# kpham-augment/LongLive

Measured on AMD Instinct MI355X. Metric: generated frames/sec (832x480) LongLive-1.3B, frame-sink + short-window attention, 4 denoise steps + clean-context pass, higher is better.
Workload: dtype bf16

## Files before the change

### include/longlive_hip.h

```cpp
#ifndef LONGLIVE_HIP_H
#define LONGLIVE_HIP_H

#include <stdint.h>

#ifdef __cplusplus
extern "C" {
#endif

typedef uint16_t ll_bf16;
typedef void* ll_stream;

enum ll_status {
  LL_OK = 0,
  LL_ERR_INVALID_ARG = -1,
  LL_ERR_LAUNCH = -2,
  LL_ERR_UNSUPPORTED = -3
};

enum ll_epilogue {
  LL_EPI_BIAS = 0,
  LL_EPI_BIAS_GELU = 1,
  LL_EPI_BIAS_GATE_RES = 2,
  LL_EPI_BIAS_RES = 3
};

#define LL_ABI_VERSION 111
int ll_version(void);
const char* ll_last_error(void);
int ll_set_tuning(const char* key, int value);
int ll_gemm_plan(int M, int N, int K, int int8, char* out, int cap);
int ll_gemm_plan_epi(int M, int N, int K, int int8, int epilogue, int plain, char* out, int cap);
int ll_flash_attn_plan(int Lq, int H, int B, int seg0_len, int seg1_len, int seg_adjacent, char* out, int cap);
int ll_conv_plan(int T, int H, int W, int Cin, int Cout, int KT, int KH, int upsample, int with_res, int rms, char* out, int cap);


int ll_ln_modulate(const ll_bf16* x, ll_bf16* out, const ll_bf16* e, const ll_bf16* mod, int nmod, int shift_idx,
                   int scale_idx, int B, int L, int C, int F, float eps, ll_stream stream);

int ll_modulation_table(const ll_bf16* e, const ll_bf16* mods, ll_bf16* out, int num_layers, int BF, int nmod, int C,
                        ll_stream stream);

int ll_modulation_table_f32(const ll_bf16* e, const ll_bf16* mods, float* out, int num_layers, int BF, int nmod, int C,
                            unsigned one_plus_mask, ll_stream stream);

int ll_ln_modulate_tab(const ll_bf16* x, ll_bf16* out, int8_t* q, float* qscale, const float* tab, int nmod, int shift_idx,
                       int scale_idx, int B, int L, int C, int F, float eps, ll_stream stream);

int ll_layernorm_affine(const ll_bf16* x, const ll_bf16* w, const ll_bf16* b, ll_bf16* out, int rows, int C,
                        float eps, ll_stream stream);

int ll_ln_modulate_q8(const ll_bf16* x, int8_t* q, float* qscale, const ll_bf16* e, const ll_bf16* mod, int nmod,
                      int shift_idx, int scale_idx, int B, int L, int C, int F, float eps, ll_stream stream);
int ll_layernorm_affine_q8(const ll_bf16* x, const ll_bf16* w, const ll_bf16* b, int8_t* q, float* qscale, int rows,
                           int C, float eps, ll_stream stream);

int ll_rmsnorm(const ll_bf16* x, const ll_bf16* w, ll_bf16* out, int rows, int C, int ldx, int ldo, float eps,
               ll_stream stream);

int ll_qk_norm_rope_kv_store(const ll_bf16* qkv, const ll_bf16* wq, const ll_bf16* wk, const float* rope_f,
                             const float* rope_hw, ll_bf16* q_out, ll_bf16* cache_k, ll_bf16* cache_v, int B, int L,
                             int C, int head_dim, int frame_len, int start_frame, int S, int write_start,
                             int roped_offset, int write_len, float eps, ll_stream stream);

int ll_kv_roll(ll_bf16* cache_k, ll_bf16* cache_v, int B, int S, int C, int dst, int src, int n, ll_stream stream);


int ll_gemm_bf16(const ll_bf16* x, const ll_bf16* w, const ll_bf16* bias, ll_bf16* out, int M, int N, int K, int ldx,
                 int ldo, int epilogue, const ll_bf16* res, const ll_bf16* e, const ll_bf16* mod, int nmod,
                 int gate_idx, int rows_per_batch, int frame_len, ll_stream stream);

int ll_gemm_ksplit_plan(int M, int N, int K);
long long ll_gemm_ksplit_workspace_bytes(int M, int N, int K);
int ll_gemm_bf16_ksplit(const ll_bf16* x, const ll_bf16* w, const ll_bf16* bias, ll_bf16* out, int M, int N, int K, int ldx,
                        int ldo, int epilogue, const ll_bf16* res, void* workspace, long long workspace_bytes, ll_stream stream);
int ll_gemm_bf16_ksplit_t5norm(const ll_bf16* x, const ll_bf16* w, const ll_bf16* bias, ll_bf16* out, int M, int N, int K, int ldx,
                               int ldo, const ll_bf16* res, const ll_bf16* norm_w, float eps, ll_bf16* h_out, void* workspace,
                               long long workspace_bytes, ll_stream stream);

int ll_gemm_w8a8(const int8_t* xq, const float* sx, const int8_t* wq, const float* sw, const ll_bf16* bias, ll_bf16* out,
                 int M, int N, int K, int ldo, int epilogue, const ll_bf16* res, const ll_bf16* e, const ll_bf16* mod,
                 int nmod, int gate_idx, int rows_per_batch, int frame_len, ll_stream stream);

int ll_gemm_bf16_qkv(const ll_bf16* x, const ll_bf16* w, const ll_bf16* bias, ll_bf16* out, int M, int N, int K, int ldx, int ldo,
                     ll_bf16* cache_v, int B, int L, int S, int write_start, int roped_offset, int write_len, ll_stream stream);
int ll_gemm_w8a8_qkv(const int8_t* xq, const float* sx, const int8_t* wq, const float* sw, const ll_bf16* bias, ll_bf16* out,
                     int M, int N, int K, int ldo, ll_bf16* cache_v, int B, int L, int S, int write_start, int roped_offset,
                     int write_len, ll_stream stream);

int ll_quantize_rows(const ll_bf16* x, int8_t* q, float* scale, int rows, int K, int ldx, ll_stream stream);

int ll_quantize_mx(const ll_bf16* x, uint8_t* q, uint8_t* qs, int rows, int K, int ldx, ll_stream stream);
int ll_gemm_mx(const uint8_t* xq, const uint8_t* sx, const uint8_t* wq, const uint8_t* sw, const ll_bf16* bias, ll_bf16* out,
               uint8_t* q_out, uint8_t* s_out, int M, int N, int K, int ldo, int epilogue, const ll_bf16* res, const ll_bf16* e,
               const ll_bf16* mod, int nmod, int gate_idx, int rows_per_batch, int frame_len, ll_stream stream);
int ll_gemm_mx_qkv(const uint8_t* xq, const uint8_t* sx, const uint8_t* wq, const uint8_t* sw, const ll_bf16* bias, ll_bf16* out,
                   int M, int N, int K, int ldo, ll_bf16* cache_v, int B, int L, int S, int write_start, int roped_offset,
                   int write_len, ll_stream stream);
int ll_ln_modulate_mx(const ll_bf16* x, uint8_t* q, uint8_t* qs, const ll_bf16* e, const ll_bf16* mod, int nmod, int shift_idx,
                      int scale_idx, int B, int L, int C, int F, float eps, ll_stream stream);
int ll_ln_modulate_tab_mx(const ll_bf16* x, uint8_t* q, uint8_t* qs, const float* tab, int nmod, int shift_idx, int scale_idx,
                          int B, int L, int C, int F, float eps, ll_stream stream);
int ll_layernorm_affine_mx(const ll_bf16* x, const ll_bf16* w, const ll_bf16* b, uint8_t* q, uint8_t* qs, int rows, int C,
                           float eps, ll_stream stream);
int ll_gemm_plan_mx(int M, int N, int K, char* out, int cap);

int ll_quantize_mx6(const ll_bf16* x, uint8_t* q, uint8_t* qs, int rows, int K, int ldx, ll_stream stream);
int ll_gemm_mx6(const uint8_t* xq, const uint8_t* sx, const uint8_t* wq, const uint8_t* sw, const ll_bf16* bias, ll_bf16* out,
                uint8_t* q_out, uint8_t* s_out, int M, int N, int K, int ldo, int epilogue, const ll_bf16* res, const ll_bf16* e,
                const ll_bf16* mod, int nmod, int gate_idx, int rows_per_batch, int frame_len, ll_stream stream);
int ll_gemm_mx6_qkv(const uint8_t* xq, const uint8_t* sx, const uint8_t* wq, const uint8_t* sw, const ll_bf16* bias, ll_bf16* out,
                    int M, int N, int K, int ldo, ll_bf16* cache_v, int B, int L, int S, int write_start, int roped_offset,
                    int write_len, ll_stream stream);
int ll_ln_modulate_mx6(const ll_bf16* x, uint8_t* q, uint8_t* qs, const ll_bf16* e, const ll_bf16* mod, int nmod, int shift_idx,
                       int scale_idx, int B, int L, int C, int F, float eps, ll_stream stream);
int ll_ln_modulate_tab_mx6(const ll_bf16* x, uint8_t* q, uint8_t* qs, const float* tab, int nmod, int shift_idx, int scale_idx,
                           int B, int L, int C, int F, float eps, ll_stream stream);
int ll_layernorm_affine_mx6(const ll_bf16* x, const ll_bf16* w, const ll_bf16* b, uint8_t* q, uint8_t* qs, int rows, int C,
                            float eps, ll_stream stream);
int ll_gemm_plan_mx6(int M, int N, int K, char* out, int cap);

int ll_quantize_mx4(const ll_bf16* x, uint8_t* q, uint8_t* qs, int rows, int K, int ldx, ll_stream stream);
int ll_gemm_mx4w6(const uint8_t* xq, const uint8_t* sx, const uint8_t* wq, const uint8_t* sw, const ll_bf16* bias, ll_bf16* out,
                  uint8_t* q_out, uint8_t* s_out, int M, int N, int K, int ldo, int epilogue, const ll_bf16* res, const ll_bf16* e,
                  const ll_bf16* mod, int nmod, int gate_idx, int rows_per_batch, int frame_len, ll_stream stream);
int ll_gemm_mx4w6_qkv(const uint8_t* xq, const uint8_t* sx, const uint8_t* wq, const uint8_t* sw, const ll_bf16* bias, ll_bf16* out,
                      int M, int N, int K, int ldo, ll_bf16* cache_v, int B, int L, int S, int write_start, int roped_offset,
                      int write_len, ll_stream stream);
int ll_gemm_plan_mx4w6(int M, int N, int K, char* out, int cap);

int ll_gemm_mx4(const uint8_t* xq, const uint8_t* sx, const uint8_t* wq, const uint8_t* sw, const ll_bf16* bias, ll_bf16* out,
                uint8_t* q_out, uint8_t* s_out, int M, int N, int K, int ldo, int epilogue, const ll_bf16* res, const ll_bf16* e,
                const ll_bf16* mod, int nmod, int gate_idx, int rows_per_batch, int frame_len, ll_stream stream);
int ll_gemm_mx4_qkv(const uint8_t* xq, const uint8_t* sx, const uint8_t* wq, const uint8_t* sw, const ll_bf16* bias, ll_bf16* out,
                    int M, int N, int K, int ldo, ll_bf16* cache_v, int B, int L, int S, int write_start, int roped_offset,
                    int write_len, ll_stream stream);
int ll_ln_modulate_mx4(const ll_bf16* x, uint8_t* q, uint8_t* qs, const ll_bf16* e, const ll_bf16* mod, int nmod, int shift_idx,
                       int scale_idx, int B, int L, int C, int F, float eps, ll_stream stream);
int ll_ln_modulate_tab_mx4(const ll_bf16* x, uint8_t* q, uint8_t* qs, const float* tab, int nmod, int shift_idx, int scale_idx,
                           int B, int L, int C, int F, float eps, ll_stream stream);
int ll_layernorm_affine_mx4(const ll_bf16* x, const ll_bf16* w, const ll_bf16* b, uint8_t* q, uint8_t* qs, int rows, int C,
                            float eps, ll_stream stream);
int ll_gemm_plan_mx4(int M, int N, int K, char* out, int cap);

int ll_quantize_rows_f8(const ll_bf16* x, uint8_t* q, float* scale, int rows, int K, int ldx, ll_stream stream);
int ll_gemm_f8(const uint8_t* xq, const float* sx, const uint8_t* wq, const float* sw, const ll_bf16* bias, ll_bf16* out,
               int M, int N, int K, int ldo, int epilogue, const ll_bf16* res, const ll_bf16* e, const ll_bf16* mod,
               int nmod, int gate_idx, int rows_per_batch, int frame_len, ll_stream stream);
int ll_gemm_f8_qkv(const uint8_t* xq, const float* sx, const uint8_t* wq, const float* sw, const ll_bf16* bias, ll_bf16* out,
                   int M, int N, int K, int ldo, ll_bf16* cache_v, int B, int L, int S, int write_start, int roped_offset,
                   int write_len, ll_stream stream);
int ll_ln_modulate_f8(const ll_bf16* x, uint8_t* q, float* qscale, const ll_bf16* e, const ll_bf16* mod, int nmod, int shift_idx,
                      int scale_idx, int B, int L, int C, int F, float eps, ll_stream stream);
int ll_ln_modulate_tab_f8(const ll_bf16* x, uint8_t* q, float* qscale, const float* tab, int nmod, int shift_idx, int scale_idx,
                          int B, int L, int C, int F, float eps, ll_stream stream);
int ll_layernorm_affine_f8(const ll_bf16* x, const ll_bf16* w, const ll_bf16* b, uint8_t* q, float* qscale, int rows, int C,
                           float eps, ll_stream stream);
int ll_gemm_plan_f8(int M, int N, int K, char* out, int cap);

int ll_kv_shadow_mx(const ll_bf16* k, const ll_bf16* v, uint8_t* kq, uint8_t* ks, uint8_t* vq, uint8_t* vs, int B, int S, int S32, int H,
                    int head_dim, int lo, int hi, ll_stream stream);
int ll_flash_attn_mx(const ll_bf16* q, const uint8_t* kq, const uint8_t* ks, const uint8_t* vq, const uint8_t* vs, ll_bf16* out, int B,
                     int Lq, int H, int head_dim, int ldq, int ldo, int S, int S32, int seg0_start, int seg0_len, int seg1_start,
                     int seg1_len, float scale, ll_stream stream);
int ll_flash_attn_mx_plan(int Lq, int H, int B, int seg0_start, int seg0_len, int seg1_start, int seg1_len, char* out, int cap);

int ll_linear_small(const ll_bf16* x, const ll_bf16* w, const ll_bf16* bias, ll_bf16* out, int M, int N, int K,
                    int act_in, int act_out, ll_stream stream);

int ll_flash_attn(const ll_bf16* q, const ll_bf16* k, const ll_bf16* v, ll_bf16* out, int B, int Lq, int H, int ldq,
                  int ldo, int ldk, long long k_batch_stride, int seg0_start, int seg0_len, int seg1_start,
                  int seg1_len, float scale, ll_stream stream);

int ll_gemm_ssq_planes(int M, int N, int K);
int ll_gemm_bf16_ssq(const ll_bf16* x, const ll_bf16* w, const ll_bf16* bias, ll_bf16* out, float* ssq, int M, int N, int K, int ldx,
                     int ldo, ll_stream stream);
int ll_flash_attn_qnorm_ok(int H, int nkeys);
int ll_flash_attn_qnorm(const ll_bf16* q, const float* ssq, const ll_bf16* norm_w, float eps, const ll_bf16* k, const ll_bf16* v,
                        ll_bf16* out, int B, int Lq, int H, int ldq, int ldo, int ldk, long long k_batch_stride, int key_start,
                        int nkeys, float scale, ll_stream stream);

enum ll_qfmt { LL_QFMT_MX = 1, LL_QFMT_MX6 = 2, LL_QFMT_MX4 = 3 };
int ll_flash_attn_q_ok(int fmt, int H, int seg0_start, int seg0_len, int seg1_start, int seg1_len);
int ll_flash_attn_q_plan(int fmt, int Lq, int H, int B, int seg0_start, int seg0_len, int seg1_start, int seg1_len, char* out, int cap);
int ll_flash_attn_q(int fmt, const ll_bf16* q, const ll_bf16* k, const ll_bf16* v, uint8_t* codes, uint8_t* scales, int B, int Lq, int H,
                    int ldq, int ldc, int lds, int ldk, long long k_batch_stride, int seg0_start, int seg0_len, int seg1_start,
                    int seg1_len, float scale, ll_stream stream);
int ll_flash_attn_mx_q(int fmt, const ll_bf16* q, const uint8_t* kq, const uint8_t* ks, const uint8_t* vq, const uint8_t* vs,
                       uint8_t* codes, uint8_t* scales, int B, int Lq, int H, int head_dim, int ldq, int ldc, int lds, int S, int S32,
                       int seg0_start, int seg0_len, int seg1_start, int seg1_len, float scale, ll_stream stream);


int ll_patchify(const ll_bf16* x, ll_bf16* patches, int B, int F, int Cin, int H, int W, ll_stream stream);

int ll_sinusoid(const float* t, ll_bf16* out, int n, int dim, ll_stream stream);

int ll_unpatchify_x0(const ll_bf16* head, const ll_bf16* xt, const float* sigma, ll_bf16* flow, ll_bf16* x0, int B,
                     int F, int Cout, int H, int W, ll_stream stream);

int ll_add_noise(const ll_bf16* x0, const ll_bf16* noise, const float* sigma, ll_bf16* out, int N, long long inner,
                 ll_stream stream);

int ll_sigma_lookup(const float* t, const float* timesteps, const float* sigmas, float* out, int n, int n_table,
                    ll_stream stream);

int ll_synth_hash(float* out, long long lo, long long n, unsigned long long stream_const, int kind, ll_stream stream);


int ll_conv_cl(const ll_bf16* x, const ll_bf16* zero16, const ll_bf16* w, const ll_bf16* bias, const ll_bf16* res,
               ll_bf16* out, int T, int H, int W, int Cin, int Cout, int Kpad, int KT, int KH, int upsample, int ldo,
               ll_stream stream);
int ll_conv_cl_rms_ok(int H, int W, int Cin, int Cout, int KT, int KH, int upsample);
int ll_conv_cl_rms(const ll_bf16* x, const ll_bf16* zero16, const ll_bf16* w, const ll_bf16* bias, const ll_bf16* res, ll_bf16* out,
                   const ll_bf16* rms_gamma, ll_bf16* out_rms, int rms_silu, int T, int H, int W, int Cin, int Cout, int Kpad, int KT,
                   int KH, int upsample, int ldo, ll_stream stream);

int ll_rms_silu_cl(const ll_bf16* x, const ll_bf16* gamma, ll_bf16* out, long long pixels, int C, int do_silu,
                   ll_stream stream);

int ll_softmax_rows(const ll_bf16* s, ll_bf16* p, int rows, int N, int ld, float scale, ll_stream stream);

int ll_vae_unscale_cl(const ll_bf16* z, const ll_bf16* mean, const ll_bf16* inv_std, ll_bf16* out, int T, int C, int h,
                      int w, ll_stream stream);

int ll_cl_to_tchw_clamp(const ll_bf16* x, float* out, int T, int H, int W, int ldc, ll_stream stream);


int ll_cl_to_frames_u8(const ll_bf16* x, uint8_t* out, long long stride_t, int T, int H, int W, int ldc, ll_stream stream);

int ll_jpeg_sizes(int T, int H, int W, long long* out_stride, long long* scratch_bytes);
int ll_jpeg_encode_u8(const uint8_t* frames, long long stride_t, int T, int H, int W, int quality, uint8_t* out, long long out_stride,
                      int32_t* sizes, void* scratch, long long scratch_bytes, ll_stream stream);
int ll_jpeg_coefficients_u8(const uint8_t* frames, long long stride_t, int T, int H, int W, int quality, int16_t* coef, ll_stream stream);

int ll_jpeg_decode_sizes(int T, int H, int W, int ncomp, int hs, int vs, long long* coef_bytes, long long* scratch_bytes);
int ll_jpeg_decode_coefficients(const uint8_t* data, long long nbytes, const int32_t* segs, int nseg, const uint8_t* huff,
                                const uint8_t* sel, int T, int H, int W, int ncomp, int hs, int vs, int16_t* coef, int32_t* status,
                                ll_stream stream);
int ll_jpeg_decode_pixels(const int16_t* coef, const uint16_t* qt, int T, int H, int W, int ncomp, int hs, int vs, uint8_t* out,
                          long long stride_t, void* scratch, long long scratch_bytes, ll_stream stream);
int ll_jpeg_decode_u8(const uint8_t* data, long long nbytes, const int32_t* segs, int nseg, const uint8_t* huff, const uint8_t* sel,
                      const uint16_t* qt, int T, int H, int W, int ncomp, int hs, int vs, int16_t* coef, int32_t* status, uint8_t* out,
                      long long stride_t, void* scratch, long long scratch_bytes, ll_stream stream);
int ll_jpeg_decode_split_sizes(int nseg, int nsub, long long* work_bytes);
int ll_jpeg_decode_coefficients_split(const uint8_t* data, long long nbytes, const int32_t* segs, int nseg, const uint8_t* huff,
                                      const uint8_t* sel, int T, int H, int W, int ncomp, int hs, int vs, int16_t* coef, int32_t* status,
                                      const int32_t* subs, int nsub, int rounds, int32_t* info, void* work, long long work_bytes,
                                      ll_stream stream);
int ll_jpeg_decode_u8_split(const uint8_t* data, long long nbytes, const int32_t* segs, int nseg, const uint8_t* huff, const uint8_t* sel,
                            const uint16_t* qt, int T, int H, int W, int ncomp, int hs, int vs, int16_t* coef, int32_t* status, uint8_t* out,
                            long long stride_t, void* scratch, long long scratch_bytes, const int32_t* subs, int nsub, int rounds,
                            int32_t* info, void* work, long long work_bytes, ll_stream stream);
int ll_resize_u8(const uint8_t* src, long long src_stride_t, int Hs, int Ws, int y0, int x0, int Hc, int Wc, uint8_t* dst,
                 long long dst_stride_t, int Hd, int Wd, int T, const int32_t* ystart, const int32_t* ycount, const float* yweight, int ky,
                 const int32_t* xstart, const int32_t* xcount, const float* xweight, int kx, ll_stream stream);


int ll_conv_cl_down(const ll_bf16* x, const ll_bf16* zero16, const ll_bf16* w, const ll_bf16* bias, ll_bf16* out, int T, int H, int W,
                    int Cin, int Cout, int Kpad, int ldo, ll_stream stream);
int ll_conv_cl_tdown(const ll_bf16* x, const ll_bf16* zero16, const ll_bf16* w, const ll_bf16* bias, ll_bf16* out, int T, int H, int W,
                     int Cin, int Cout, int Kpad, int ldo, ll_stream stream);
int ll_conv_down_plan(int kind, int T, int H, int W, int Cin, int Cout, char* out, int cap);

int ll_pixels_to_cl(const void* px, int is_f32, long long stride_c, long long stride_t, ll_bf16* out, int T, int H, int W, int Cpad,
                    ll_stream stream);

int ll_pixels_u8_to_cl(const uint8_t* px, long long stride_t, ll_bf16* out, int T, int H, int W, int Cpad, ll_stream stream);

int ll_vae_scale_tchw(const ll_bf16* mu, const ll_bf16* mean, const ll_bf16* inv_std, float* out, int T, int z_dim, int h, int w, int ld,
                      ll_stream stream);


int ll_t5_rmsnorm(const ll_bf16* x, const ll_bf16* w, ll_bf16* out, int rows, int C, float eps, ll_stream stream);

int ll_t5_gated_gelu(const ll_bf16* h, ll_bf16* out, long long M, int F, ll_stream stream);

int ll_gather_rows(const ll_bf16* table, const long long* ids, ll_bf16* out, int n, int C, long long vocab, ll_stream stream);

int ll_t5_attention(const ll_bf16* q, const ll_bf16* k, const ll_bf16* vt, const ll_bf16* bias_tab, ll_bf16* out, int L,
                    int H, int ldqk, int ldo, int seq_len, ll_stream stream);

#ifdef __cplusplus
}
#endif
#endif
```

### longlive_amd/_lib.py

```python
from __future__ import annotations

import ctypes as C
import os

_HERE = os.path.dirname(os.path.abspath(__file__))
LIB_PATH = os.path.join(_HERE, "liblonglive_hip.so")

ABI_VERSION = 111

_p, _i, _f, _ll = C.c_void_p, C.c_int, C.c_float, C.c_longlong

SIGNATURES = {
    "ll_version": [],
    "ll_last_error": [],
    "ll_set_tuning": [C.c_char_p, _i],
    "ll_gemm_plan": [_i, _i, _i, _i, C.c_char_p, _i],
    "ll_gemm_plan_epi": [_i, _i, _i, _i, _i, _i, C.c_char_p, _i],
    "ll_flash_attn_plan": [_i, _i, _i, _i, _i, _i, C.c_char_p, _i],
    "ll_ln_modulate": [_p, _p, _p, _p, _i, _i, _i, _i, _i, _i, _i, _f, _p],
    "ll_modulation_table": [_p, _p, _p, _i, _i, _i, _i, _p],
    "ll_modulation_table_f32": [_p, _p, _p, _i, _i, _i, _i, C.c_uint, _p],
    "ll_ln_modulate_tab": [_p, _p, _p, _p, _p, _i, _i, _i, _i, _i, _i, _i, _f, _p],
    "ll_layernorm_affine": [_p, _p, _p, _p, _i, _i, _f, _p],
    "ll_ln_modulate_q8": [_p, _p, _p, _p, _p, _i, _i, _i, _i, _i, _i, _i, _f, _p],
    "ll_layernorm_affine_q8": [_p, _p, _p, _p, _p, _i, _i, _f, _p],
    "ll_rmsnorm": [_p, _p, _p, _i, _i, _i, _i, _f, _p],
    "ll_qk_norm_rope_kv_store": [_p, _p, _p, _p, _p, _p, _p, _p, _i, _i, _i, _i, _i, _i, _i, _i, _i, _i, _f, _p],
    "ll_kv_roll": [_p, _p, _i, _i, _i, _i, _i, _i, _p],
    "ll_gemm_bf16": [_p, _p, _p, _p, _i, _i, _i, _i, _i, _i, _p, _p, _p, _i, _i, _i, _i, _p],
    "ll_gemm_ksplit_plan": [_i, _i, _i],
    "ll_gemm_ksplit_workspace_bytes": [_i, _i, _i],
    "ll_gemm_bf16_ksplit": [_p, _p, _p, _p, _i, _i, _i, _i, _i, _i, _p, _p, _ll, _p],
    "ll_gemm_bf16_ksplit_t5norm": [_p, _p, _p, _p, _i, _i, _i, _i, _i, _p, _p, _f, _p, _p, _ll, _p],
    "ll_gemm_w8a8": [_p, _p, _p, _p, _p, _p, _i, _i, _i, _i, _i, _p, _p, _p, _i, _i, _i, _i, _p],
    "ll_gemm_bf16_qkv": [_p, _p, _p, _p, _i, _i, _i, _i, _i, _p, _i, _i, _i, _i, _i, _i, _p],
    "ll_gemm_w8a8_qkv": [_p, _p, _p, _p, _p, _p, _i, _i, _i, _i, _p, _i, _i, _i, _i, _i, _i, _p],
    "ll_quantize_rows": [_p, _p, _p, _i, _i, _i, _p],
    "ll_linear_small": [_p, _p, _p, _p, _i, _i, _i, _i, _i, _p],
    "ll_flash_attn": [_p, _p, _p, _p, _i, _i, _i, _i, _i, _i, _ll, _i, _i, _i, _i, _f, _p],
    "ll_patchify": [_p, _p, _i, _i, _i, _i, _i, _p],
    "ll_sinusoid": [_p, _p, _i, _i, _p],
    "ll_unpatchify_x0": [_p, _p, _p, _p, _p, _i, _i, _i, _i, _i, _p],
    "ll_add_noise": [_p, _p, _p, _p, _i, _ll, _p],
    "ll_sigma_lookup": [_p, _p, _p, _p, _i, _i, _p],
    "ll_synth_hash": [_p, _ll, _ll, C.c_ulonglong, _i, _p],
    "ll_gemm_ssq_planes": [_i, _i, _i],
    "ll_gemm_bf16_ssq": [_p, _p, _p, _p, _p, _i, _i, _i, _i, _i, _p],
    "ll_flash_attn_qnorm_ok": [_i, _i],
    "ll_flash_attn_qnorm": [_p, _p, _p, _f, _p, _p, _p, _i, _i, _i, _i, _i, _i, _ll, _i, _i, _f, _p],
    "ll_flash_attn_q_ok": [_i] * 6,
    "ll_flash_attn_q_plan": [_i] * 8 + [C.c_char_p, _i],
    "ll_flash_attn_q": [_i] + [_p] * 5 + [_i] * 7 + [_ll] + [_i] * 4 + [_f, _p],
    "ll_flash_attn_mx_q": [_i] + [_p] * 7 + [_i] * 13 + [_f, _p],
    "ll_conv_plan": [_i] * 10 + [C.c_char_p, _i],
    "ll_conv_cl": [_p] * 6 + [_i] * 10 + [_p],
    "ll_conv_cl_rms_ok": [_i] * 7,
    "ll_conv_cl_rms": [_p] * 8 + [_i] * 11 + [_p],
    "ll_rms_silu_cl": [_p, _p, _p, _ll, _i, _i, _p],
    "ll_softmax_rows": [_p, _p, _i, _i, _i, _f, _p],
    "ll_vae_unscale_cl": [_p, _p, _p, _p, _i, _i, _i, _i, _p],
    "ll_cl_to_tchw_clamp": [_p, _p, _i, _i, _i, _i, _p],
    "ll_cl_to_frames_u8": [_p, _p, _ll, _i, _i, _i, _i, _p],
    "ll_jpeg_sizes": [_i, _i, _i, C.POINTER(_ll), C.POINTER(_ll)],
    "ll_jpeg_encode_u8": [_p, _ll, _i, _i, _i, _i, _p, _ll, _p, _p, _ll, _p],
    "ll_jpeg_coefficients_u8": [_p, _ll, _i, _i, _i, _i, _p, _p],
    "ll_jpeg_decode_sizes": [_i] * 6 + [C.POINTER(_ll), C.POINTER(_ll)],
    "ll_jpeg_decode_coefficients": [_p, _ll, _p, _i, _p, _p] + [_i] * 6 + [_p, _p, _p],
    "ll_jpeg_decode_pixels": [_p, _p] + [_i] * 6 + [_p, _ll, _p, _ll, _p],
    "ll_jpeg_decode_u8": [_p, _ll, _p, _i, _p, _p, _p] + [_i] * 6 + [_p, _p, _p, _ll, _p, _ll, _p],
    "ll_jpeg_decode_split_sizes": [_i, _i, C.POINTER(_ll)],
    "ll_jpeg_decode_coefficients_split": [_p, _ll, _p, _i, _p, _p] + [_i] * 6 + [_p, _p] + [_p, _i, _i, _p, _p, _ll, _p],
    "ll_jpeg_decode_u8_split": [_p, _ll, _p, _i, _p, _p, _p] + [_i] * 6 + [_p, _p, _p, _ll, _p, _ll] + [_p, _i, _i, _p, _p, _ll, _p],
    "ll_resize_u8": [_p, _ll] + [_i] * 6 + [_p, _ll, _i, _i, _i, _p, _p, _p, _i, _p, _p, _p, _i, _p],
    "ll_conv_cl_down": [_p] * 5 + [_i] * 7 + [_p],
    "ll_conv_cl_tdown": [_p] * 5 + [_i] * 7 + [_p],
    "ll_conv_down_plan": [_i] * 6 + [C.c_char_p, _i],
    "ll_pixels_to_cl": [_p, _i, _ll, _ll, _p, _i, _i, _i, _i, _p],
    "ll_pixels_u8_to_cl": [_p, _ll, _p, _i, _i, _i, _i, _p],
    "ll_vae_scale_tchw": [_p, _p, _p, _p, _i, _i, _i, _i, _i, _p],
    "ll_t5_rmsnorm": [_p, _p, _p, _i, _i, _f, _p],
    "ll_t5_gated_gelu": [_p, _p, _ll, _i, _p],
    "ll_gather_rows": [_p, _p, _p, _i, _i, _ll, _p],
    "ll_t5_attention": [_p, _p, _p, _p, _p, _i, _i, _i, _i, _i, _p],
    "ll_quantize_mx": [_p, _p, _p, _i, _i, _i, _p],
    "ll_gemm_mx": [_p, _p, _p, _p, _p, _p, _p, _p, _i, _i, _i, _i, _i, _p, _p, _p, _i, _i, _i, _i, _p],
    "ll_gemm_mx_qkv": [_p, _p, _p, _p, _p, _p, _i, _i, _i, _i, _p, _i, _i, _i, _i, _i, _i, _p],
    "ll_ln_modulate_mx": [_p, _p, _p, _p, _p, _i, _i, _i, _i, _i, _i, _i, _f, _p],
    "ll_ln_modulate_tab_mx": [_p, _p, _p, _p, _i, _i, _i, _i, _i, _i, _i, _f, _p],
    "ll_layernorm_affine_mx": [_p, _p, _p, _p, _p, _i, _i, _f, _p],
    "ll_gemm_plan_mx": [_i, _i, _i, C.c_char_p, _i],
    "ll_kv_shadow_mx": [_p] * 6 + [_i] * 7 + [_p],
    "ll_flash_attn_mx": [_p] * 6 + [_i] * 12 + [_f, _p],
    "ll_flash_attn_mx_plan": [_i] * 7 + [C.c_char_p, _i],
    "ll_quantize_rows_f8": [_p, _p, _p, _i, _i, _i, _p],
    "ll_gemm_f8": [_p, _p, _p, _p, _p, _p, _i, _i, _i, _i, _i, _p, _p, _p, _i, _i, _i, _i, _p],
    "ll_gemm_f8_qkv": [_p, _p, _p, _p, _p, _p, _i, _i, _i, _i, _p, _i, _i, _i, _i, _i, _i, _p],
    "ll_ln_modulate_f8": [_p, _p, _p, _p, _p, _i, _i, _i, _i, _i, _i, _i, _f, _p],
    "ll_ln_modulate_tab_f8": [_p, _p, _p, _p, _i, _i, _i, _i, _i, _i, _i, _f, _p],
    "ll_layernorm_affine_f8": [_p, _p, _p, _p, _p, _i, _i, _f, _p],
    "ll_gemm_plan_f8": [_i, _i, _i, C.c_char_p, _i],
    "ll_quantize_mx6": [_p, _p, _p, _i, _i, _i, _p],
    "ll_gemm_mx6": [_p] * 8 + [_i] * 5 + [_p] * 3 + [_i] * 4 + [_p],
    "ll_gemm_mx6_qkv": [_p] * 6 + [_i] * 4 + [_p] + [_i] * 6 + [_p],
    "ll_ln_modulate_mx6": [_p] * 5 + [_i] * 7 + [_f, _p],
    "ll_ln_modulate_tab_mx6": [_p] * 4 + [_i] * 7 + [_f, _p],
    "ll_layernorm_affine_mx6": [_p] * 5 + [_i, _i, _f, _p],
    "ll_gemm_plan_mx6": [_i, _i, _i, C.c_char_p, _i],
    "ll_quantize_mx4": [_p, _p, _p, _i, _i, _i, _p],
    "ll_gemm_mx4w6": [_p] * 8 + [_i] * 5 + [_p] * 3 + [_i] * 4 + [_p],
    "ll_gemm_mx4w6_qkv": [_p] * 6 + [_i] * 4 + [_p] + [_i] * 6 + [_p],
    "ll_gemm_plan_mx4w6": [_i, _i, _i, C.c_char_p, _i],
    "ll_gemm_mx4": [_p] * 8 + [_i] * 5 + [_p] * 3 + [_i] * 4 + [_p],
    "ll_gemm_mx4_qkv": [_p] * 6 + [_i] * 4 + [_p] + [_i] * 6 + [_p],
    "ll_ln_modulate_mx4": [_p] * 5 + [_i] * 7 + [_f, _p],
    "ll_ln_modulate_tab_mx4": [_p] * 4 + [_i] * 7 + [_f, _p],
    "ll_layernorm_affine_mx4": [_p] * 5 + [_i, _i, _f, _p],
    "ll_gemm_plan_mx4": [_i, _i, _i, C.c_char_p, _i],
}
_RESTYPES = {"ll_last_error": C.c_char_p, "ll_gemm_ksplit_workspace_bytes": C.c_longlong}

_lib = None


def load() -> C.CDLL:
    global _lib
    if _lib is not None:
        return _lib
    path = os.environ.get("LONGLIVE_HIP_LIB", LIB_PATH)
    if not os.path.exists(path):
        raise RuntimeError(
            f"{path} not found: the HIP extension is not built (make -C longlive_amd/csrc). "
            "longlive_amd has no CPU fallback by design.")
    lib = C.CDLL(path)
    for name, argtypes in SIGNATURES.items():
        try:
            fn = getattr(lib, name)
        except AttributeError as exc:
            raise RuntimeError(f"{LIB_PATH} does not export {name}") from exc
        fn.argtypes = argtypes
        fn.restype = _RESTYPES.get(name, C.c_int)
    if lib.ll_version() != ABI_VERSION:
        raise RuntimeError(f"{path} has ABI version {lib.ll_version()}, this binding needs {ABI_VERSION}: rebuild it "
                           "(make -C longlive_amd/csrc); a stale library would misread every argument list")
    _lib = lib
    for kv in filter(None, os.environ.get("LL_TUNING", "").split(",")):
        k, v = kv.split("=")
        if lib.ll_set_tuning(k.encode(), int(v)) != 0:
            raise RuntimeError(f"LL_TUNING: {lib.ll_last_error().decode()}")
    return lib


def check(rc: int, what: str = "") -> None:
    if rc != 0:
        msg = load().ll_last_error()
        raise RuntimeError(f"longlive_hip {what} failed (status {rc}): {msg.decode() if msg else ''}")
```

### longlive_amd/csrc/gemm.hip

```cpp
#include <stdio.h>
#include <string.h>
#include <atomic>

#include "attention_common.h"
#include "gemm_asm.h"
#include "gemm_common.h"
#include "mx.h"

#ifdef LL_GEMM_DIAG
constexpr bool GEMM_DIAG = true;
#else
constexpr bool GEMM_DIAG = false;
#endif

#define V2_BM 256
#define V2_STAGE ((V2_BM + BN) * ROWB)

template <int EPI, int Q>
__global__ __launch_bounds__(512, 2) void gemm_kernel_v2(const char* __restrict__ X, const char* __restrict__ Wt,
                                                         bf16* __restrict__ Y, int M, int N, int nk, size_t xrow_bytes,
                                                         size_t wrow_bytes, int ldo, int ntm, int ntn, int gm, int lds_epi, EpiArgs ea) {
  extern __shared__ __attribute__((aligned(16))) char smem[];
  const int tid = threadIdx.x, lane = tid & 63;
  const int wave = __builtin_amdgcn_readfirstlane(tid >> 6);
// ... 346 lines not shown
  else snprintf(walk, sizeof walk, ", N fastest");
  snprintf(out, (size_t)cap, "%s<%s> tile %dx%d, %d workgroups%s", p.name, kind, p.bm, p.bn, p.ntm * p.ntn, walk);
}

extern "C" int ll_gemm_plan(int M, int N, int K, int int8, char* out, int cap) {
  LL_REQUIRE(out != nullptr && cap > 0, "ll_gemm_plan: needs an output buffer");
  gemm_plan_text(M, N, int8 ? "i8" : "bf16", out, cap);
  (void)K;
  return LL_OK;
}

extern "C" int ll_gemm_plan_f8(int M, int N, int K, char* out, int cap) {
  LL_REQUIRE(out != nullptr && cap > 0, "ll_gemm_plan_f8: needs an output buffer");
  gemm_plan_text(M, N, "f8", out, cap);
  (void)K;
  return LL_OK;
}

extern "C" int ll_gemm_plan_epi(int M, int N, int K, int int8, int epilogue, int plain, char* out, int cap);

extern "C" int ll_t5_rmsnorm(const ll_bf16* x, const ll_bf16* w, ll_bf16* out, int rows, int C, float eps, ll_stream stream);

static bool gemm_asm_wanted(int epilogue) {
  return (g_gemm_asm & 1) && !((g_gemm_asm & 4) && epilogue == LL_EPI_BIAS_GELU) && !((g_gemm_asm & 8) && epilogue != LL_EPI_BIAS_GELU);
}

typedef void (*gemm_kernel_t)(const char*, const char*, bf16*, int, int, int, size_t, size_t, int, int, int, int, int, EpiArgs);
template <int E, int Q>
static gemm_kernel_t gemm_instance(int variant) {
  switch (variant) {
    case 3: return gemm_kernel_v5<E, Q, 2, 4, 8, 4, 2, false>;
    case 5: return gemm_kernel_v5<E, Q, 2, 4, 8, 3, 1, true>;
    case 6: return gemm_kernel_v5<E, Q, 4, 2, 4, 7, 1, true>;
    default: return gemm_kernel_v2<E, Q>;
  }
}

template <int Q>
static int launch_gemm(const void* x, const void* w, bf16* out, int M, int N, int K, size_t xrow_bytes, size_t wrow_bytes,
                       int ldo, int epilogue, const EpiArgs& ea, hipStream_t s) {
  if (Q == GQ_BF16 && gemm_asm_wanted(epilogue) && wrow_bytes == (size_t)K * 2) {
    const int r = gemm_asm_launch((const bf16*)x, (const bf16*)w, out, M, N, K, (int)(xrow_bytes / 2), ldo, epilogue, ea, g_gemm_group_m, s);
    if (r) return r < 0 ? r : 0;
  }
  if (Q == GQ_I8 && (g_gemm_asm & 16) && gemm_asm_wanted(epilogue) && xrow_bytes == (size_t)K && wrow_bytes == (size_t)K) {
    const int r = gemm_asm_launch_i8((const int8_t*)x, (const int8_t*)w, out, M, N, K, ldo, epilogue, ea, g_gemm_group_m, s);
    if (r) return r < 0 ? r : 0;
  }
  const int nk = (Q == GQ_BF16 ? 2 * K : K) / ROWB;
  const GemmPlan p = gemm_plan(M, N);
  const int mode = g_gemm_lds_epi & 3;
  const int lds_epi = (mode == 2 || (mode == 1 && epilogue != LL_EPI_BIAS_GELU) ? 1 : 0) | (GEMM_DIAG ? g_gemm_lds_epi & 0x300 : 0);
  const gemm_kernel_t k = epilogue == LL_EPI_BIAS            ? gemm_instance<LL_EPI_BIAS, Q>(p.variant)
                          : epilogue == LL_EPI_BIAS_GELU     ? gemm_instance<LL_EPI_BIAS_GELU, Q>(p.variant)
                          : epilogue == LL_EPI_BIAS_GATE_RES ? gemm_instance<LL_EPI_BIAS_GATE_RES, Q>(p.variant)
                                                             : gemm_instance<LL_EPI_BIAS_RES, Q>(p.variant);
  (void)ll_lds_attr((const void*)k, p.lds);
  hipLaunchKernelGGL(k, dim3(p.ntm * p.ntn), dim3(512), (size_t)p.lds, s, (const char*)x, (const char*)w, out, M, N, nk, xrow_bytes,
                     wrow_bytes, ldo, p.ntm, p.ntn, g_gemm_group_m, lds_epi, ea);
  return LL_OK;
}

struct FamBF16 {
  static constexpr int Q = GQ_BF16;
  static int check(const char* fn, const void*, const void*, const void*, const void*, const void*, int, int K, int ldx, int) {
    LL_REQUIRE(K > 0 && K % 64 == 0, "%s: K=%d must be a positive multiple of 64", fn, K);
    LL_REQUIRE(ldx >= K && ldx % 8 == 0, "%s: ldx=%d must be >= K and a multiple of 8", fn, ldx);
    return LL_OK;
  }
  static size_t xrow(int, int ldx) { return (size_t)ldx * 2; }
  static size_t wrow(int K) { return (size_t)K * 2; }
};
struct FamW8A8 {
  static constexpr int Q = GQ_I8;
  static int check(const char* fn, const void*, const void* sx, const void*, const void* sw, const void*, int, int K, int, int) {
    LL_REQUIRE(K > 0 && K % 128 == 0, "%s: K=%d must be a positive multiple of 128", fn, K);
    LL_REQUIRE(sx && sw, "%s: activation and weight scales are required", fn);
    return LL_OK;
  }
  static size_t xrow(int K, int) { return (size_t)K; }
  static size_t wrow(int K) { return (size_t)K; }
};
struct FamF8 {
  static constexpr int Q = GQ_F8;
  static int check(const char* fn, const void* xq, const void* sx, const void* wq, const void* sw, const void* out, int M, int K, int,
                   int ldo) {
    LL_REQUIRE(xq && sx && wq && sw, "%s: codes and scales of both operands are required", fn);
    LL_REQUIRE(out != nullptr, "%s: out is required", fn);
    LL_REQUIRE(K > 0 && K % 128 == 0, "%s: K=%d must be a positive multiple of 128", fn, K);
    LL_REQUIRE(M >= 0, "%s: M=%d", fn, M);
    LL_REQUIRE(ldo % 8 == 0, "%s: ldo=%d must be a multiple of 8", fn, ldo);
    return LL_OK;
  }
  static size_t xrow(int K, int) { return (size_t)K; }
  static size_t wrow(int K) { return (size_t)K; }
};

template <class F>
static int gemm_call(const char* fn, const void* x, const float* sx, const void* w, const float* sw, const ll_bf16* bias, ll_bf16* out,
                     int M, int N, int K, int ldx, int ldo, int epilogue, const ll_bf16* res, const ll_bf16* e, const ll_bf16* mod,
                     int nmod, int gate_idx, int rows_per_batch, int frame_len, ll_stream stream) {
  if (int rc = F::check(fn, x, sx, w, sw, out, M, K, ldx, ldo)) return rc;
  if (int rc = check_epilogue(fn, M, N, ldo, epilogue, bias, res, e, mod, nmod, gate_idx, rows_per_batch, frame_len)) return rc;
  if (M == 0) return LL_OK;
  EpiArgs ea{(const bf16*)bias, (const bf16*)res, (const bf16*)e, (const bf16*)mod, sx, sw, nmod, gate_idx,
             rows_per_batch, frame_len, frame_len > 0 && rows_per_batch > 0 ? rows_per_batch / frame_len : 0};
  if (int lrc = launch_gemm<F::Q>(x, w, (bf16*)out, M, N, K, F::xrow(K, ldx), F::wrow(K), ldo, epilogue, ea, (hipStream_t)stream)) return lrc;
  return ll_check_launch(fn);
}

template <class F>
static int gemm_call_qkv(const char* fn, const void* x, const float* sx, const void* w, const float* sw, const ll_bf16* bias,
                         ll_bf16* out, int M, int N, int K, int ldx, int ldo, ll_bf16* cache_v, int B, int L, int S, int write_start,
                         int roped_offset, int write_len, ll_stream stream) {
  if (int rc = F::check(fn, x, sx, w, sw, out, M, K, ldx, ldo)) return rc;
  if (int rc = check_epilogue(fn, M, N, ldo, LL_EPI_BIAS, bias, nullptr, nullptr, nullptr, 0, 0, 0, 0)) return rc;
  if (int rc = check_v_insert(fn, M, N, B, L, S, write_start, roped_offset, write_len, cache_v)) return rc;
  if (M == 0) return LL_OK;
  EpiArgs ea{(const bf16*)bias, nullptr, nullptr, nullptr, sx, sw, 0, 0, 0, 0, 0};
  set_v_insert(ea, cache_v, N, L, S, write_start, roped_offset, write_len);
  if (int lrc = launch_gemm<F::Q>(x, w, (bf16*)out, M, N, K, F::xrow(K, ldx), F::wrow(K), ldo, LL_EPI_BIAS, ea, (hipStream_t)stream)) return lrc;
  return ll_check_launch(fn);
}

extern "C" int ll_gemm_bf16(const ll_bf16* x, const ll_bf16* w, const ll_bf16* bias, ll_bf16* out, int M, int N, int K,
                            int ldx, int ldo, int epilogue, const ll_bf16* res, const ll_bf16* e, const ll_bf16* mod,
                            int nmod, int gate_idx, int rows_per_batch, int frame_len, ll_stream stream) {
  return gemm_call<FamBF16>("ll_gemm_bf16", x, nullptr, w, nullptr, bias, out, M, N, K, ldx, ldo, epilogue, res, e, mod, nmod, gate_idx,
                            rows_per_batch, frame_len, stream);
}

extern "C" int ll_gemm_ssq_planes(int M, int N, int K) {
  if (!gemm_asm_wanted(LL_EPI_BIAS)) return 0;
  const GemmAsmPick p = gemm_asm_pick(GQ_BF16, M, N, K, K, LL_EPI_BIAS, true, false, false, 0, 0);
  return p.k && p.k->wn == 128 && N / 128 <= 16 ? N / 128 : 0;
}
extern "C" int ll_gemm_bf16_ssq(const ll_bf16* x, const ll_bf16* w, const ll_bf16* bias, ll_bf16* out, float* ssq, int M, int N, int K,
                                int ldx, int ldo, ll_stream stream) {
  LL_REQUIRE(K > 0 && K % 64 == 0, "ll_gemm_bf16_ssq: K=%d must be a positive multiple of 64", K);
  LL_REQUIRE(ldx >= K && ldx % 8 == 0, "ll_gemm_bf16_ssq: ldx=%d must be >= K and a multiple of 8", ldx);
  int rc = check_epilogue("ll_gemm_bf16_ssq", M, N, ldo, LL_EPI_BIAS, bias, nullptr, nullptr, nullptr, 0, 0, 0, 0);
  if (rc) return rc;
  LL_REQUIRE(ssq != nullptr && ((size_t)ssq & 3) == 0, "ll_gemm_bf16_ssq: ssq is required");
  LL_REQUIRE(ll_gemm_ssq_planes(M, N, K) > 0 && ldx == K, "ll_gemm_bf16_ssq: %d x %d x %d is not covered by the generated kernel under the current "
             "tuning (ask ll_gemm_ssq_planes first and run ll_gemm_bf16 + ll_rmsnorm instead)", M, N, K);
  if (M == 0) return LL_OK;
  const int r = gemm_asm_ssq_launch((const bf16*)x, (const bf16*)w, (const bf16*)bias, (bf16*)out, ssq, M, N, K, ldx, ldo, g_gemm_group_m,
                                    (hipStream_t)stream);
  if (r < 0) return r;
  LL_REQUIRE(r == 1, "ll_gemm_bf16_ssq: the generated kernel refused a shape its plan accepted");
  return ll_check_launch("ll_gemm_bf16_ssq");
}

extern "C" int ll_gemm_ksplit_plan(int M, int N, int K) {
  if (!gemm_asm_wanted(LL_EPI_BIAS)) return 0;
  return gemm_ksplit_splits(M, N, K, device_cus());
}
extern "C" long long ll_gemm_ksplit_workspace_bytes(int M, int N, int K) {
  const int S = ll_gemm_ksplit_plan(M, N, K);
  return S ? (long long)S * M * N * 4 : 0;
}
extern "C" int ll_gemm_bf16_ksplit(const ll_bf16* x, const ll_bf16* w, const ll_bf16* bias, ll_bf16* out, int M, int N, int K,
                                   int ldx, int ldo, int epilogue, const ll_bf16* res, void* workspace,
                                   long long workspace_bytes, ll_stream stream) {
  LL_REQUIRE(K > 0 && K % 64 == 0, "ll_gemm_bf16_ksplit: K=%d must be a positive multiple of 64", K);
  LL_REQUIRE(ldx >= K && ldx % 8 == 0, "ll_gemm_bf16_ksplit: ldx=%d must be >= K and a multiple of 8", ldx);
  LL_REQUIRE(epilogue == LL_EPI_BIAS || epilogue == LL_EPI_BIAS_RES, "ll_gemm_bf16_ksplit: epilogue %d (bias or bias + residual only)", epilogue);
  int rc = check_epilogue("ll_gemm_bf16_ksplit", M, N, ldo, epilogue, bias, res, nullptr, nullptr, 0, 0, 0, 0);
  if (rc) return rc;
  LL_REQUIRE(workspace_bytes >= 0 && (workspace != nullptr || workspace_bytes == 0), "ll_gemm_bf16_ksplit: workspace_bytes without a workspace");
  if (M == 0) return LL_OK;
  const int S = ll_gemm_ksplit_plan(M, N, K);
  if (S >= 2 && workspace != nullptr) {
    LL_REQUIRE(workspace_bytes >= (long long)S * M * N * 4 && ((size_t)workspace & 15) == 0,
               "ll_gemm_bf16_ksplit: workspace of %lld bytes, need %lld (16-byte aligned)", workspace_bytes, (long long)S * M * N * 4);
    const int r = gemm_asm_ksplit_launch((const bf16*)x, (const bf16*)w, (const bf16*)bias, (bf16*)out, M, N, K, ldx, ldo, epilogue,
                                         (const bf16*)res, (float*)workspace, S, g_gemm_group_m, (hipStream_t)stream, nullptr, 0.f, nullptr);
    if (r) return r < 0 ? r : ll_check_launch("ll_gemm_bf16_ksplit");
  }
  EpiArgs ea{(const bf16*)bias, (const bf16*)res, nullptr, nullptr, nullptr, nullptr, 0, 0, 0, 0, 0};
  if (int lrc = launch_gemm<GQ_BF16>(x, w, (bf16*)out, M, N, K, (size_t)ldx * 2, (size_t)K * 2, ldo, epilogue, ea, (hipStream_t)stream)) return lrc;
  return ll_check_launch("ll_gemm_bf16_ksplit");
}

extern "C" int ll_gemm_bf16_ksplit_t5norm(const ll_bf16* x, const ll_bf16* w, const ll_bf16* bias, ll_bf16* out, int M, int N, int K,
                                          int ldx, int ldo, const ll_bf16* res, const ll_bf16* norm_w, float eps, ll_bf16* h_out,
                                          void* workspace, long long workspace_bytes, ll_stream stream) {
  LL_REQUIRE(K > 0 && K % 64 == 0, "ll_gemm_bf16_ksplit_t5norm: K=%d must be a positive multiple of 64", K);
  LL_REQUIRE(ldx >= K && ldx % 8 == 0, "ll_gemm_bf16_ksplit_t5norm: ldx=%d must be >= K and a multiple of 8", ldx);
  LL_REQUIRE(norm_w != nullptr && h_out != nullptr, "ll_gemm_bf16_ksplit_t5norm: needs the norm weight and an output for the normalised rows");
  LL_REQUIRE(ldo == N, "ll_gemm_bf16_ksplit_t5norm: ldo=%d must equal N=%d (the norm runs over whole rows)", ldo, N);
  int rc = check_epilogue("ll_gemm_bf16_ksplit_t5norm", M, N, ldo, LL_EPI_BIAS_RES, bias, res, nullptr, nullptr, 0, 0, 0, 0);
  if (rc) return rc;
  LL_REQUIRE(workspace_bytes >= 0 && (workspace != nullptr || workspace_bytes == 0), "ll_gemm_bf16_ksplit_t5norm: workspace_bytes without a workspace");
  if (M == 0) return LL_OK;
  const int S = ll_gemm_ksplit_plan(M, N, K);
  if (S >= 2 && workspace != nullptr && N <= 4096) {
    LL_REQUIRE(workspace_bytes >= (long long)S * M * N * 4 && ((size_t)workspace & 15) == 0,
               "ll_gemm_bf16_ksplit_t5norm: workspace of %lld bytes, need %lld (16-byte aligned)", workspace_bytes, (long long)S * M * N * 4);
    const int r = gemm_asm_ksplit_launch((const bf16*)x, (const bf16*)w, (const bf16*)bias, (bf16*)out, M, N, K, ldx, ldo, LL_EPI_BIAS_RES,
                                         (const bf16*)res, (float*)workspace, S, g_gemm_group_m, (hipStream_t)stream, (const bf16*)norm_w, eps,
                                         (bf16*)h_out);
    if (r) return r < 0 ? r : ll_check_launch("ll_gemm_bf16_ksplit_t5norm");
  }
  rc = ll_gemm_bf16_ksplit(x, w, bias, out, M, N, K, ldx, ldo, LL_EPI_BIAS_RES, res, workspace, workspace_bytes, stream);
  if (rc) return rc;
  return ll_t5_rmsnorm(out, norm_w, h_out, M, N, eps, stream);
}

extern "C" int ll_gemm_plan_epi(int M, int N, int K, int int8, int epilogue, int plain, char* out, int cap) {
  LL_REQUIRE(out != nullptr && cap > 0, "ll_gemm_plan_epi: needs an output buffer");
  if (gemm_asm_wanted(epilogue) && (!int8 || (g_gemm_asm & 16))) {
    const GemmAsmPick p = gemm_asm_pick(int8 ? GQ_I8 : GQ_BF16, M, N, K, K, epilogue, plain != 0, plain == 2, plain == 2 && (2 * (N / 3)) % 192 == 0,
                                        1, int8 ? 0 : device_cus());
    if (p.k) { gemm_asm_plan(p, out, cap); ll_plan_append_knobs(out, cap); return LL_OK; }
  }
  return ll_gemm_plan(M, N, K, int8, out, cap);
}

extern "C" int ll_gemm_w8a8(const int8_t* xq, const float* sx, const int8_t* wq, const float* sw, const ll_bf16* bias,
                            ll_bf16* out, int M, int N, int K, int ldo, int epilogue, const ll_bf16* res,
                            const ll_bf16* e, const ll_bf16* mod, int nmod, int gate_idx, int rows_per_batch,
                            int frame_len, ll_stream stream) {
  return gemm_call<FamW8A8>("ll_gemm_w8a8", xq, sx, wq, sw, bias, out, M, N, K, K, ldo, epilogue, res, e, mod, nmod, gate_idx,
                            rows_per_batch, frame_len, stream);
}

extern "C" int ll_gemm_f8(const uint8_t* xq, const float* sx, const uint8_t* wq, const float* sw, const ll_bf16* bias, ll_bf16* out,
                          int M, int N, int K, int ldo, int epilogue, const ll_bf16* res, const ll_bf16* e, const ll_bf16* mod,
                          int nmod, int gate_idx, int rows_per_batch, int frame_len, ll_stream stream) {
  return gemm_call<FamF8>("ll_gemm_f8", xq, sx, wq, sw, bias, out, M, N, K, K, ldo, epilogue, res, e, mod, nmod, gate_idx,
                          rows_per_batch, frame_len, stream);
}

extern "C" int ll_gemm_bf16_qkv(const ll_bf16* x, const ll_bf16* w, const ll_bf16* bias, ll_bf16* out, int M, int N, int K, int ldx,
                                int ldo, ll_bf16* cache_v, int B, int L, int S, int write_start, int roped_offset, int write_len,
                                ll_stream stream) {
  return gemm_call_qkv<FamBF16>("ll_gemm_bf16_qkv", x, nullptr, w, nullptr, bias, out, M, N, K, ldx, ldo, cache_v, B, L, S, write_start,
                                roped_offset, write_len, stream);
}

extern "C" int ll_gemm_w8a8_qkv(const int8_t* xq, const float* sx, const int8_t* wq, const float* sw, const ll_bf16* bias,
                                ll_bf16* out, int M, int N, int K, int ldo, ll_bf16* cache_v, int B, int L, int S, int write_start,
                                int roped_offset, int write_len, ll_stream stream) {
  return gemm_call_qkv<FamW8A8>("ll_gemm_w8a8_qkv", xq, sx, wq, sw, bias, out, M, N, K, K, ldo, cache_v, B, L, S, write_start,
                                roped_offset, write_len, stream);
}

extern "C" int ll_gemm_f8_qkv(const uint8_t* xq, const float* sx, const uint8_t* wq, const float* sw, const ll_bf16* bias,
                              ll_bf16* out, int M, int N, int K, int ldo, ll_bf16* cache_v, int B, int L, int S, int write_start,
                              int roped_offset, int write_len, ll_stream stream) {
  return gemm_call_qkv<FamF8>("ll_gemm_f8_qkv", xq, sx, wq, sw, bias, out, M, N, K, K, ldo, cache_v, B, L, S, write_start, roped_offset,
                              write_len, stream);
}

template <bool F8, class TQ>
static int quantize_rows_launch(const char* fn, void (*reg4)(const bf16*, TQ*, float*, int, int, int),
                                void (*reg18)(const bf16*, TQ*, float*, int, int, int), void (*two_pass)(const bf16*, TQ*, float*, int, int, int),
                                const ll_bf16* x, TQ* q, float* scale, int rows, int K, int ldx, ll_stream stream) {
  if (F8) LL_REQUIRE(x != nullptr && q != nullptr && scale != nullptr, "%s: x, codes and scales are required", fn);
  LL_REQUIRE(K > 0 && K % 8 == 0, "%s: K=%d must be a positive multiple of 8", fn, K);
  LL_REQUIRE(ldx >= K && ldx % 8 == 0, "%s: ldx=%d must be >= K and a multiple of 8", fn, ldx);
  if (F8) LL_REQUIRE(rows >= 0, "%s: rows=%d", fn, rows);
  if (rows == 0) return LL_OK;
  hipLaunchKernelGGL(K <= 2048 ? reg4 : K <= 9216 ? reg18 : two_pass, dim3((rows + 3) / 4), dim3(256), 0, (hipStream_t)stream,
                     (const bf16*)x, q, scale, rows, K, ldx);
  return ll_check_launch(fn);
}

extern "C" int ll_quantize_rows(const ll_bf16* x, int8_t* q, float* scale, int rows, int K, int ldx, ll_stream stream) {
  return quantize_rows_launch<false>("ll_quantize_rows", quantize_rows_reg_kernel<4>, quantize_rows_reg_kernel<18>, quantize_rows_kernel,
                                     x, q, scale, rows, K, ldx, stream);
}

extern "C" int ll_quantize_rows_f8(const ll_bf16* x, uint8_t* q, float* scale, int rows, int K, int ldx, ll_stream stream) {
  return quantize_rows_launch<true>("ll_quantize_rows_f8", quantize_rows_f8_reg_kernel<4>, quantize_rows_f8_reg_kernel<18>,
                                    quantize_rows_f8_kernel, x, q, scale, rows, K, ldx, stream);
}

extern "C" int ll_linear_small(const ll_bf16* x, const ll_bf16* w, const ll_bf16* bias, ll_bf16* out, int M, int N,
                               int K, int act_in, int act_out, ll_stream stream) {
  LL_REQUIRE(M >= 0 && M <= 8, "ll_linear_small: M=%d must be <= 8", M);
  LL_REQUIRE(K % 8 == 0, "ll_linear_small: K=%d must be a multiple of 8", K);
  if (M == 0 || N == 0) return LL_OK;
  hipLaunchKernelGGL(linear_small_kernel, dim3((N + 3) / 4), dim3(256), 0, (hipStream_t)stream, (const bf16*)x,
                     (const bf16*)w, (const bf16*)bias, (bf16*)out, M, N, K, act_in, act_out);
  return ll_check_launch("ll_linear_small");
}
```

### longlive_amd/csrc/gemm_asm.h

```cpp
#pragma once
#include "gemm_common.h"

extern int g_gemm_asm_persistent;
extern const int g_gemm_asm_mfma16_default;
extern int g_gemm_asm_mfma16;

struct GemmAsmKernel {
  const void* fn;
  const char* name;
  int wn, epilogue;
  bool persistent, i8, m16;
  int mfma16_bit;
};

struct GemmAsmPick {
  const GemmAsmKernel* k;
  int ntm, ntn, grid, lds;
};
GemmAsmPick gemm_asm_pick(int kind, int M, int N, int K, int ldx, int epilogue, bool plain, bool has_v, bool v_ok, int frame_len, int cus);
const char* gemm_asm_plan(const GemmAsmPick& p, char* out, int cap);

int gemm_asm_launch(const bf16* x, const bf16* w, bf16* out, int M, int N, int K, int ldx, int ldo, int epilogue, const EpiArgs& ea,
                    int gm, hipStream_t s);
int gemm_asm_launch_i8(const int8_t* x, const int8_t* w, bf16* out, int M, int N, int K, int ldo, int epilogue, const EpiArgs& ea,
                       int gm, hipStream_t s);
int gemm_asm_ssq_launch(const bf16* x, const bf16* w, const bf16* bias, bf16* out, float* ssq, int M, int N, int K, int ldx, int ldo, int gm,
                        hipStream_t s);
int gemm_ksplit_splits(int M, int N, int K, int cus);
int gemm_asm_ksplit_launch(const bf16* x, const bf16* w, const bf16* bias, bf16* out, int M, int N, int K, int ldx, int ldo,
                           int epilogue, const bf16* res, float* workspace, int splits, int gm, hipStream_t s, const bf16* norm_w,
                           float eps, bf16* h_out);
```

### longlive_amd/csrc/gemm_asm.hip

```cpp
#include "gemm_asm.h"

#define GA_EACH "gemm_asm_each.inl"
#include "gemm_asm_kernels.def"
static const GemmAsmKernel g_ga_kernels[] = {
#define GA_TABLE
#include "gemm_asm_kernels.def"
#undef GA_TABLE
};
enum { GA_EPI_PARTIAL = 4, GA_EPI_SSQ = 5 };

int g_gemm_asm_persistent = 1;
extern const int g_gemm_asm_mfma16_default = 511;
int g_gemm_asm_mfma16 = g_gemm_asm_mfma16_default;

static const GemmAsmKernel* ga_kernel(bool i8, int wn, int epilogue, bool persistent) {
  const GemmAsmKernel* k32 = nullptr;
  for (const GemmAsmKernel& k : g_ga_kernels)
    if (k.i8 == i8 && k.wn == wn && k.epilogue == epilogue && k.persistent == persistent) {
      if (!k.m16) k32 = &k;
      else if (g_gemm_asm_mfma16 & k.mfma16_bit) return &k;
    }
  return k32;
}

static int ga_lds(int wn) { return 3 * wn * 128 + 4 * 2 * 8192; }

static int ga_width(bool i8, int M, int N, int K, int ldx, int epilogue, bool plain, bool has_v, bool v_ok, int frame_len) {
  const int kstep = i8 ? 128 : 64;
  if (!plain || M <= 0 || K % kstep != 0 || K < 4 * kstep) return 0;
  if (i8 ? (long long)256 * K >= 0x7fffffffLL
         : (ldx % 8) != 0 || (long long)256 * ldx * 2 >= 0x7fffffffLL || (long long)256 * K * 2 >= 0x7fffffffLL) return 0;
  if (epilogue == LL_EPI_BIAS_GATE_RES && frame_len <= 0) return 0;
  if (has_v) return (v_ok && epilogue == LL_EPI_BIAS && N % 192 == 0) ? 192 : 0;
  if (epilogue == LL_EPI_BIAS_GELU) return N % 224 == 0 ? 224 : 0;
  if (epilogue == LL_EPI_BIAS && N > 2048 && N % 192 == 0) return 192;
  if (i8) return N % 128 == 0 && N <= 2048 ? 128 : 0;
  if (epilogue == LL_EPI_BIAS && M <= 1024 && N >= 16384 && N % 256 == 0) return 256;
  if (N % 128 == 0 && (N <= 2048 || M <= 1024) &&
      (epilogue == LL_EPI_BIAS || epilogue == LL_EPI_BIAS_GATE_RES || epilogue == LL_EPI_BIAS_RES)) return 128;
  return 0;
}

GemmAsmPick gemm_asm_pick(int kind, int M, int N, int K, int ldx, int epilogue, bool plain, bool has_v, bool v_ok, int frame_len, int cus) {
  const bool i8 = kind == GQ_I8;
  GemmAsmPick p{};
  const int wn = ga_width(i8, M, N, K, ldx, epilogue, plain, has_v, v_ok, frame_len);
  if (!wn) return p;
  const int epi = wn == 224 ? LL_EPI_BIAS_GELU : wn != 128 || epilogue == LL_EPI_BIAS ? LL_EPI_BIAS
                  : epilogue == LL_EPI_BIAS_GATE_RES ? LL_EPI_BIAS_GATE_RES : LL_EPI_BIAS_RES;
  p.ntm = (M + 255) / 256, p.ntn = N / wn, p.lds = ga_lds(wn);
  const int pcus = cus & ~7;
  if (!i8 && g_gemm_asm_persistent && pcus >= 8 && p.ntm * p.ntn > pcus) p.k = ga_kernel(i8, wn, epi, true);
  p.grid = p.k ? pcus : p.ntm * p.ntn;
  if (!p.k) p.k = ga_kernel(i8, wn, epi, false);
  return p;
}

const char* gemm_asm_plan(const GemmAsmPick& p, char* out, int cap) {
  const int wn = p.k->wn, tiles = p.ntm * p.ntn;
  if (p.k->persistent)
    snprintf(out, (size_t)cap, "%s<bf16> tile 256x%d (4 waves x 64 rows, one wave per SIMD, generated schedule), %d persistent workgroups "
             "walk %d tiles, next tile staged under the epilogue", p.k->name, wn, p.grid, tiles);
  else
    snprintf(out, (size_t)cap, "%s<%s> tile 256x%d (4 waves x 64 rows, one wave per SIMD, generated schedule), %d workgroups", p.k->name,
             p.k->i8 ? "i8" : "bf16", wn, tiles);
  return out;
}

struct GemmAsmArgs {
  const void *x, *w;
  const bf16* bias;
  bf16* out;
  const bf16 *res, *gate;
  int M, N, K, ldx, ldo, frame_len, gate_stride, ntm, ntn, gm;
  bf16* v_out;
  int v_col0, v_C, v_shift, v_lo, v_hi;
  const float *sx, *sw;
  float* ssq;
};

static int ga_launch(const GemmAsmKernel& k, int grid, hipStream_t s, GemmAsmArgs& a, const char* what) {
  const int lds = ga_lds(k.wn);
  if (int rc = ll_lds_attr(k.fn, lds)) return rc;
  void* args[] = {&a.x, &a.w, &a.bias, &a.out, &a.res, &a.gate, &a.M, &a.N, &a.K, &a.ldx, &a.ldo, &a.frame_len, &a.gate_stride, &a.ntm, &a.ntn,
                  &a.gm, &a.v_out, &a.v_col0, &a.v_C, &a.v_shift, &a.v_lo, &a.v_hi, k.i8 ? (void*)&a.sx : (void*)&a.ssq, &a.sw};
  if (hipLaunchKernel(k.fn, dim3(grid), dim3(256), args, (size_t)lds, s) != hipSuccess) return ll_check_launch(what);
  return 1;
}

static int ga_gemm(int kind, const void* x, const void* w, bf16* out, int M, int N, int K, int ldx, int ldo, int epilogue, const EpiArgs& ea,
                   int gm, hipStream_t s) {
  const bool has_v = ea.v_out != nullptr, i8 = kind == GQ_I8;
  const GemmAsmPick p = gemm_asm_pick(kind, M, N, K, ldx, epilogue, ea.mod == nullptr && (i8 || ea.sx == nullptr), has_v,
                                      has_v && ea.v_L == M && ea.v_col0 % 192 == 0 && ea.v_C > 0, ea.frame_len, i8 ? 0 : device_cus());
  if (!p.k) return 0;
  GemmAsmArgs a{x, w, ea.bias, out, ea.res, epilogue == LL_EPI_BIAS_GATE_RES ? ea.e + (size_t)ea.gate_idx * N : nullptr, M, N, K, ldx, ldo,
                ea.frame_len, ea.nmod * N * 2, p.ntm, p.ntn, gm, ea.v_out, ea.v_col0, ea.v_C, ea.v_write_start - ea.v_roped_offset,
                ea.v_roped_offset, ea.v_roped_offset + ea.v_write_len, ea.sx, ea.sw, nullptr};
  return ga_launch(*p.k, p.grid, s, a, "gemm_asm");
}
int gemm_asm_launch(const bf16* x, const bf16* w, bf16* out, int M, int N, int K, int ldx, int ldo, int epilogue, const EpiArgs& ea,
                    int gm, hipStream_t s) {
  return ga_gemm(GQ_BF16, x, w, out, M, N, K, ldx, ldo, epilogue, ea, gm, s);
}
int gemm_asm_launch_i8(const int8_t* x, const int8_t* w, bf16* out, int M, int N, int K, int ldo, int epilogue, const EpiArgs& ea,
                       int gm, hipStream_t s) {
  if (ea.sx == nullptr || ea.sw == nullptr) return 0;
  return ga_gemm(GQ_I8, x, w, out, M, N, K, K, ldo, epilogue, ea, gm, s);
}

int gemm_asm_ssq_launch(const bf16* x, const bf16* w, const bf16* bias, bf16* out, float* ssq, int M, int N, int K, int ldx, int ldo, int gm,
                        hipStream_t s) {
  const GemmAsmPick p = gemm_asm_pick(GQ_BF16, M, N, K, ldx, LL_EPI_BIAS, true, false, false, 0, 0);
  if (!p.k || p.k->wn != 128) return 0;
  const GemmAsmKernel* k = ga_kernel(false, 128, GA_EPI_SSQ, false);
  GemmAsmArgs a{x, w, bias, out, nullptr, nullptr, M, N, K, ldx, ldo, 0, 0, p.ntm, p.ntn, gm, nullptr, 0, 0, 0, 0, 0, nullptr, nullptr, ssq};
  return ga_launch(*k, p.grid, s, a, k->name);
}

template <int EPI>
__global__ __launch_bounds__(256) void gemm_ksplit_reduce_kernel(const float* __restrict__ part, int splits, int M, int N,
                                                                 const bf16* __restrict__ bias, const bf16* __restrict__ res,
                                                                 bf16* __restrict__ out, int ldo) {
  const int n8 = N / 8;
  const long long idx = (long long)blockIdx.x * 256 + threadIdx.x;
  if (idx >= (long long)M * n8) return;
  const int m = (int)(idx / n8), n = (int)(idx - (long long)m * n8) * 8;
  float acc[8];
#pragma unroll
  for (int j = 0; j < 8; ++j) acc[j] = 0.f;
  for (int s = 0; s < splits; ++s) {
    const float4* p = reinterpret_cast<const float4*>(part + ((size_t)s * M + m) * N + n);
    float4 a = p[0], b = p[1];
    acc[0] += a.x; acc[1] += a.y; acc[2] += a.z; acc[3] += a.w; acc[4] += b.x; acc[5] += b.y; acc[6] += b.z; acc[7] += b.w;
  }
  bf16x8 bv = *reinterpret_cast<const bf16x8*>(bias + n), o;
  bf16x8 rv;
  if (EPI == LL_EPI_BIAS_RES) rv = *reinterpret_cast<const bf16x8*>(res + (size_t)m * ldo + n);
#pragma unroll
  for (int j = 0; j < 8; ++j) {
    bf16 v = (bf16)(acc[j] + (float)bv[j]);
    o[j] = EPI == LL_EPI_BIAS_RES ? (bf16)((float)rv[j] + (float)v) : v;
  }
  *reinterpret_cast<bf16x8*>(out + (size_t)m * ldo + n) = o;
}

__global__ __launch_bounds__(256) void gemm_ksplit_reduce_norm_kernel(const float* __restrict__ part, int splits, int M, int N,
                                                                      const bf16* __restrict__ bias, const bf16* __restrict__ res,
                                                                      bf16* __restrict__ out, int ldo, const bf16* __restrict__ nw,
                                                                      float eps, bf16* __restrict__ h_out) {
  __shared__ float sh[4];
  const int m = blockIdx.x;
  bf16x8 xn[2];
  float ss = 0.f;
#pragma unroll
  for (int i = 0; i < 2; ++i) {
    const int n = threadIdx.x * 8 + 2048 * i;
    if (n < N) {
      float acc[8];
#pragma unroll
      for (int j = 0; j < 8; ++j) acc[j] = 0.f;
      for (int s = 0; s < splits; ++s) {
        const float4* p = reinterpret_cast<const float4*>(part + ((size_t)s * M + m) * N + n);
        float4 a = p[0], b = p[1];
        acc[0] += a.x; acc[1] += a.y; acc[2] += a.z; acc[3] += a.w; acc[4] += b.x; acc[5] += b.y; acc[6] += b.z; acc[7] += b.w;
      }
      bf16x8 bv = *reinterpret_cast<const bf16x8*>(bias + n), rv = *reinterpret_cast<const bf16x8*>(res + (size_t)m * ldo + n), o;
#pragma unroll
      for (int j = 0; j < 8; ++j) {
        bf16 v = (bf16)(acc[j] + (float)bv[j]);
        o[j] = (bf16)((float)rv[j] + (float)v);
        ss += (float)o[j] * (float)o[j];
      }
      xn[i] = o;
      *reinterpret_cast<bf16x8*>(out + (size_t)m * ldo + n) = o;
    }
  }
  ss = t5_block_sum(ss, sh);
  const float r = rsqrtf(ss / (float)N + eps);
#pragma unroll
  for (int i = 0; i < 2; ++i) {
    const int n = threadIdx.x * 8 + 2048 * i;
    if (n < N) {
      bf16x8 g = *reinterpret_cast<const bf16x8*>(nw + n), o;
#pragma unroll
      for (int j = 0; j < 8; ++j) o[j] = (bf16)((float)g[j] * rbf((float)xn[i][j] * r));
      *reinterpret_cast<bf16x8*>(h_out + (size_t)m * N + n) = o;
    }
  }
}

int gemm_ksplit_splits(int M, int N, int K, int cus) {
  if (M <= 0 || N <= 0 || N % 128 != 0 || K % 64 != 0 || K < 1024 || cus <= 0) return 0;
  const long long tiles = (long long)((M + 255) / 256) * (N / 128);
  if (tiles * 2 > cus) return 0;
  const int nk = K / 64;
  int S = (int)((long long)cus * 64 / N);
  if (S > 4) S = 4;
  if (S > nk / 8) S = nk / 8;
  while (S >= 2 && (S - 1) * ((nk + S - 1) / S) >= nk) --S;
  if (S < 2 || tiles * S > 2 * cus) return 0;
  return S;
}
int gemm_asm_ksplit_launch(const bf16* x, const bf16* w, const bf16* bias, bf16* out, int M, int N, int K, int ldx, int ldo,
                           int epilogue, const bf16* res, float* workspace, int splits, int gm, hipStream_t s, const bf16* norm_w,
                           float eps, bf16* h_out) {
  if (splits < 2 || (epilogue != LL_EPI_BIAS && epilogue != LL_EPI_BIAS_RES) || (ldx % 8) != 0) return 0;
  if ((long long)256 * ldx * 2 >= 0x7fffffffLL || (long long)256 * K * 2 >= 0x7fffffffLL) return 0;
  const GemmAsmKernel* k = ga_kernel(false, 128, GA_EPI_PARTIAL, false);
  const int ntm = (M + 255) / 256, ntn = N / 128, per = (K / 64 + splits - 1) / splits;
  GemmAsmArgs a{x, w, nullptr, (bf16*)workspace, nullptr, nullptr, M, N, K, ldx,  N, 0, 0, ntm, ntn, gm, nullptr,  per, 0, 0, 0, 0,
                nullptr, nullptr, nullptr};
  if (int rc = ga_launch(*k, ntm * ntn * splits, s, a, k->name); rc != 1) return rc;
  const long long threads = (long long)M * (N / 8);
  dim3 grid((unsigned)((threads + 255) / 256)), block(256);
  if (norm_w != nullptr)
    hipLaunchKernelGGL(gemm_ksplit_reduce_norm_kernel, dim3(M), block, 0, s, (const float*)workspace, splits, M, N, bias, res,
                       out, ldo, norm_w, eps, h_out);
  else if (epilogue == LL_EPI_BIAS_RES)
    hipLaunchKernelGGL((gemm_ksplit_reduce_kernel<LL_EPI_BIAS_RES>), grid, block, 0, s, (const float*)workspace, splits, M, N, bias, res, out, ldo);
  else
    hipLaunchKernelGGL((gemm_ksplit_reduce_kernel<LL_EPI_BIAS>), grid, block, 0, s, (const float*)workspace, splits, M, N, bias, res, out, ldo);
  return 1;
}
```

### longlive_amd/csrc/gen/gemm_asm_gen.py

```python
#!/usr/bin/env python3
from __future__ import annotations

import os
import sys

sys.path.insert(0, os.path.dirname(os.path.abspath(__file__)))
import attn_asm_gen as _A
from attn_asm_gen import Gen, finalize, lint, sreg, vreg, areg, to_inc, f32bits, spread

EPI_BIAS, EPI_GELU, EPI_GATE_RES, EPI_RES = 0, 1, 2, 3
EPI_PARTIAL = 4
EPI_BIAS_SSQ = 5

S_X, S_W, S_Y, S_BIAS, S_RES, S_GATE = 8, 10, 12, 14, 16, 18
S_LDX, S_LDW, S_LDO = 20, 21, 22
S_ROWS, S_COLS, S_NK = 23, 24, 25
S_FLEN, S_GSTRIDE, S_M0 = 26, 27, 28
S_ROWLO = 29
S_SX, S_SW = 64, 66
S_SSQ = 64
S_XRS, S_WRS = 32, 36
S_WAVE, S_I, S_T0, S_T1, S_T2 = 40, 41, 44, 45, 46
S_WM0, S_XK, S_WK, S_XKMAX, S_WKMAX = 47, 48, 49, 43, 62
S_MSK = 50
V_TID = 0

NSLOT, XU = 3, 2
S_XM0 = 30

S_XB, S_WB, S_YB, S_BIASB, S_RESB, S_GATEB = 84, 86, 88, 90, 92, 94
S_LDO0, S_MM, S_NN = 68, 69, 70
S_TILE, S_GRID, S_NTILES, S_NTM, S_NTN, S_GM = 71, 72, 73, 74, 75, 76
S_VHI, S_VOUT, S_VCOL0, S_VC2, S_VSHIFT, S_VLO = 77, 78, 80, 81, 82, 83
S_XN, S_WN, S_PF, S_ROWSN = 64, 66, 31, 42
S_MT, S_NT = 54, 55


def KN(k):
    return _A.knob_env("ASM_G_", k, 0)


class Cfg:
    def __init__(self, WN, epi, i8=False, mfma=32):
        assert WN % 32 == 0 and 64 <= WN <= 256
        assert not (i8 and epi in (EPI_PARTIAL, EPI_BIAS_SSQ))
        assert mfma in (32, 16) and not (mfma == 16 and (i8 or epi == EPI_PARTIAL))
        self.WN, self.NB, self.MB, self.epi, self.i8 = WN, WN // 32, 2, epi, i8
        self.mfma = mfma
        self.m16 = mfma == 16
        self.sc = 2 if self.m16 else 1
        self.bl = 2 if self.m16 else 4
        self.nacc = self.MB * self.NB * 16
        self.slotb = WN * 128
        self.npw = WN // 32
        self.xbase = NSLOT * self.slotb
        self.xunit = 64 * 128
        self.lds_bytes = self.xbase + 4 * XU * self.xunit
        assert self.lds_bytes <= 160 * 1024
        self.FW = 0
        self.FX = 2 * self.NB * 2 * 4
        nxt = max(self.FX + 2 * self.MB * 4 * 4, 144)
        self.V_WOFF = nxt
        self.V_XROFF = nxt + 12
        self.V_DW = nxt + 16
        self.V_DX = nxt + 24
        self.V_LANE, self.V_R, self.V_H, self.V_ROW = nxt + 32, nxt + 33, nxt + 34, nxt + 35
        self.V_T = 0
        assert nxt + 37 <= 256, nxt
        self.V_EA = nxt + 37
        top = self.V_EA + (7 if self.m16 else 5)
        if i8:
            self.V_SX = top + 2
            top += 6
        assert top % 2 == 0, top
        self.nl = {EPI_GATE_RES: 6, EPI_RES: 2}.get(epi, 0)
        self.V_E0 = top
        top += 16 if self.nl else 0
        self.V_SS = top
        top += (8 if self.m16 else 4) if epi == EPI_BIAS_SSQ else 0
        self.V_EB = top
        self.early_nb = 0 if epi == EPI_PARTIAL else max(0, min(self.NB, (256 - top) // 8))

    def acc(self, mb, nb):
        return (mb * self.NB + nb) * 16

    def fw(self, p, nb, ks):
        return self.FW + ((p * self.NB + nb) * 2 + ks) * 4

    def fx(self, b, mb, ks4):
        return self.FX + ((b * self.MB + mb) * 4 + ks4) * 4

    def acc16(self, mb16, nb16):
        return (mb16 * 2 * self.NB + nb16) * 4

    def fw16(self, p, nb16):
        return self.FW + (p * 2 * self.NB + nb16) * 4

    def fx16(self, b, mb16, hs):
        return self.FX + ((b * 4 + mb16) * 2 + hs) * 4


def mfmas(c: Cfg, h):
    p, b, hf = h & 1, (h >> 1) & 1, h & 1
    out = []
    if c.m16:
        for nb16 in range(2 * c.NB):
            for mb16 in range(4):
                a = areg(c.acc16(mb16, nb16), 4)
                out.append(f"v_mfma_f32_16x16x32_bf16 {a}, {vreg(c.fw16(p, nb16), 4)}, {vreg(c.fx16(b, mb16, hf), 4)}, {a}")
        return out
    for ks in range(2):
        for nb in range(c.NB):
            for mb in range(c.MB):
                a = areg(c.acc(mb, nb), 16)
                op = "v_mfma_i32_32x32x32_i8" if c.i8 else "v_mfma_f32_32x32x16_bf16"
                out.append(f"{op} {a}, {vreg(c.fw(p, nb, ks), 4)}, {vreg(c.fx(b, mb, 2 * hf + ks), 4)}, {a}")
    return out


def w_frag_reads(c: Cfg, h):
    slot, hs = (h >> 1) % NSLOT, h & 1
    out = []
    if c.m16:
        for nb16 in range(2 * c.NB):
            off = slot * c.slotb + nb16 * 2048
            b64, imm = off >> 16, off & 0xFFFF
            out.append(f"ds_read_b128 {vreg(c.fw16(h & 1, nb16), 4)}, {vreg(c.V_WOFF + 4 * b64 + 2 * hs)} offset:{imm}")
        return out
    for ks in range(2):
        for nb in range(c.NB):
            off = slot * c.slotb + nb * 4096
            b64, imm = off >> 16, off & 0xFFFF
            out.append(f"ds_read_b128 {vreg(c.fw(h & 1, nb, ks), 4)}, {vreg(c.V_WOFF + 4 * b64 + 2 * hs + ks)} offset:{imm}")
    return out


def x_frag_reads(c: Cfg, s):
    out = []
    if c.m16:
        for hs in range(2):
            for mb16 in range(4):
                out.append(f"ds_read_b128 {vreg(c.fx16(s & 1, mb16, hs), 4)}, {vreg(c.V_XROFF + 2 * hs)} offset:{(s % XU) * c.xunit + mb16 * 2048}")
        return out
    for ks4 in range(4):
        for mb in range(c.MB):
            out.append(f"ds_read_b128 {vreg(c.fx(s & 1, mb, ks4), 4)}, {vreg(c.V_XROFF + ks4)} offset:{(s % XU) * c.xunit + mb * 4096}")
    return out


def x_dma(c: Cfg, s):
    out = []
    for i in range(8):
        out.append(f"s_add_u32 m0, {sreg(S_XM0)}, {(s % XU) * c.xunit + 1024 * i}")
        out.append(f"buffer_load_dwordx4 {vreg(c.V_DX + i)}, {sreg(S_XRS, 4)}, {sreg(S_XK)} offen lds")
    out.append(f"s_add_u32 {sreg(S_XK)}, {sreg(S_XK)}, 128")
    out.append(f"s_min_u32 {sreg(S_XK)}, {sreg(S_XK)}, {sreg(S_XKMAX)}")
    return out


def w_dma(c: Cfg, s):
    out = []
    for i in range(c.npw):
        out.append(f"s_add_u32 m0, {sreg(S_WM0)}, {(s % NSLOT) * c.slotb + 1024 * i}")
        out.append(f"buffer_load_dwordx4 {vreg(c.V_DW + i)}, {sreg(S_WRS, 4)}, {sreg(S_WK)} offen lds")
    out.append(f"s_add_u32 {sreg(S_WK)}, {sreg(S_WK)}, 128")
    out.append(f"s_min_u32 {sreg(S_WK)}, {sreg(S_WK)}, {sreg(S_WKMAX)}")
    return out


def drop_loads(ops):
    return [o for o in ops if not o.startswith("buffer_load")]


def udiv(g: Gen, q, num, den, T):
    I = g.I
    I(f"v_cvt_f32_u32 {vreg(T)}, {sreg(num)}")
    I(f"v_cvt_f32_u32 {vreg(T + 1)}, {sreg(den)}")
    I(f"v_rcp_f32 {vreg(T + 1)}, {vreg(T + 1)}")
    I("s_nop 0")
    I(f"v_mul_f32 {vreg(T)}, {vreg(T)}, {vreg(T + 1)}")
    I(f"v_cvt_u32_f32 {vreg(T)}, {vreg(T)}")
    I("s_nop 0")
    I(f"v_readfirstlane_b32 {sreg(q)}, {vreg(T)}")
    I("s_nop 0")
    I(f"s_mul_i32 {sreg(S_T2)}, {sreg(q)}, {sreg(den)}")
    I(f"s_cmp_gt_u32 {sreg(S_T2)}, {sreg(num)}")
    I(f"s_cselect_b32 {sreg(S_T2)}, 1, 0")
    I(f"s_sub_u32 {sreg(q)}, {sreg(q)}, {sreg(S_T2)}")
    I(f"s_mul_i32 {sreg(S_T2)}, {sreg(q)}, {sreg(den)}")
    I(f"s_sub_u32 {sreg(S_T2)}, {sreg(num)}, {sreg(S_T2)}")
    I(f"s_cmp_ge_u32 {sreg(S_T2)}, {sreg(den)}")
    I(f"s_cselect_b32 {sreg(S_T2)}, 1, 0")
    I(f"s_add_u32 {sreg(q)}, {sreg(q)}, {sreg(S_T2)}")


def gen_tile_map(g: Gen, tile, T):
    I = g.I
    q, r, x, hi, q1, a, b, c_ = 54, 55, 56, 57, 58, 59, 60, 61
    I(f"s_lshr_b32 {sreg(q)}, {sreg(S_NTILES)}, 3")
    I(f"s_and_b32 {sreg(r)}, {sreg(S_NTILES)}, 7")
    I(f"s_and_b32 {sreg(x)}, {sreg(tile)}, 7")
    I(f"s_lshr_b32 {sreg(hi)}, {sreg(tile)}, 3")
    I(f"s_add_u32 {sreg(q1)}, {sreg(q)}, 1")
    I(f"s_mul_i32 {sreg(a)}, {sreg(x)}, {sreg(q1)}")
    I(f"s_mul_i32 {sreg(b)}, {sreg(r)}, {sreg(q1)}")
    I(f"s_sub_u32 {sreg(c_)}, {sreg(x)}, {sreg(r)}")
    I(f"s_mul_i32 {sreg(c_)}, {sreg(c_)}, {sreg(q)}")
    I(f"s_add_u32 {sreg(b)}, {sreg(b)}, {sreg(c_)}")
    I(f"s_cmp_lt_u32 {sreg(x)}, {sreg(r)}")
    I(f"s_cselect_b32 {sreg(a)}, {sreg(a)}, {sreg(b)}")
    I(f"s_add_u32 {sreg(S_T0)}, {sreg(a)}, {sreg(hi)}")
    I(f"s_mul_i32 {sreg(S_T1)}, {sreg(S_GM)}, {sreg(S_NTN)}")
    udiv(g, 56, S_T0, S_T1, T)
    I(f"s_mul_i32 {sreg(57)}, {sreg(56)}, {sreg(S_T1)}")
    I(f"s_sub_u32 {sreg(S_T0)}, {sreg(S_T0)}, {sreg(57)}")
    I(f"s_mul_i32 {sreg(58)}, {sreg(56)}, {sreg(S_GM)}")
    I(f"s_sub_u32 {sreg(S_T1)}, {sreg(S_NTM)}, {sreg(58)}")
    I(f"s_min_u32 {sreg(S_T1)}, {sreg(S_T1)}, {sreg(S_GM)}")
    udiv(g, S_NT, S_T0, S_T1, T)
    I(f"s_mul_i32 {sreg(57)}, {sreg(S_NT)}, {sreg(S_T1)}")
    I(f"s_sub_u32 {sreg(57)}, {sreg(S_T0)}, {sreg(57)}")
    I(f"s_add_u32 {sreg(S_MT)}, {sreg(58)}, {sreg(57)}")


def add64(g: Gen, dst, base, lo, hi=None):
    g.I(f"s_add_u32 {sreg(dst)}, {sreg(base)}, {sreg(lo)}")
    g.I(f"s_addc_u32 {sreg(dst + 1)}, {sreg(base + 1)}, {sreg(hi) if hi is not None else 0}")


def gen_tile_bases(g: Gen, c, xdst, wdst, rows_dst, skip_label, full: bool, prefix: str):
    I = g.I
    m0r, n0 = 56, 57
    I(f"s_lshl_b32 {sreg(m0r)}, {sreg(S_MT)}, 8")
    I(f"s_mul_i32 {sreg(n0)}, {sreg(S_NT)}, {c.WN}")
    I(f"s_mul_i32 {sreg(S_T0)}, {sreg(m0r)}, {sreg(S_LDX)}")
    I(f"s_mul_hi_u32 {sreg(S_T1)}, {sreg(m0r)}, {sreg(S_LDX)}")
    add64(g, xdst, S_XB, S_T0, S_T1)
    I(f"s_mul_i32 {sreg(S_T0)}, {sreg(n0)}, {sreg(S_LDW)}")
    I(f"s_mul_hi_u32 {sreg(S_T1)}, {sreg(n0)}, {sreg(S_LDW)}")
    add64(g, wdst, S_WB, S_T0, S_T1)
    I(f"s_sub_u32 {sreg(rows_dst)}, {sreg(S_MM)}, {sreg(m0r)}")
    if full:
        I(f"s_sub_u32 {sreg(S_COLS)}, {sreg(S_NN)}, {sreg(n0)}")
        I(f"s_mov_b32 {sreg(S_M0)}, {sreg(m0r)}")
        I(f"s_mov_b32 {sreg(S_ROWLO)}, 0")
        I(f"s_mov_b32 {sreg(S_LDO)}, {sreg(S_LDO0)}")
        I(f"s_lshl_b32 {sreg(58)}, {sreg(n0)}, 1")
        add64(g, S_BIAS, S_BIASB, 58)
        add64(g, S_GATE, S_GATEB, 58)
        I(f"s_mul_i32 {sreg(S_T0)}, {sreg(m0r)}, {sreg(S_LDO0)}")
        I(f"s_mul_hi_u32 {sreg(S_T1)}, {sreg(m0r)}, {sreg(S_LDO0)}")
        I(f"s_add_u32 {sreg(S_T0)}, {sreg(S_T0)}, {sreg(58)}")
        I(f"s_addc_u32 {sreg(S_T1)}, {sreg(S_T1)}, 0")
        add64(g, S_Y, S_YB, S_T0, S_T1)
        add64(g, S_RES, S_RESB, S_T0, S_T1)
    g.uid += 1
    lab = f"{prefix}_NOTV_{g.uid}"
    I(f"s_cmp_eq_u64 {sreg(S_VOUT, 2)}, 0")
    I(f"s_cbranch_scc1 {lab}")
    I(f"s_cmp_lt_u32 {sreg(n0)}, {sreg(S_VCOL0)}")
    I(f"s_cbranch_scc1 {lab}")
    I(f"s_min_i32 {sreg(59)}, {sreg(S_MM)}, {sreg(S_VHI)}")
    I(f"s_sub_i32 {sreg(59)}, {sreg(59)}, {sreg(m0r)}")
    I(f"s_sub_i32 {sreg(60)}, {sreg(S_VLO)}, {sreg(m0r)}")
    I(f"s_max_i32 {sreg(60)}, {sreg(60)}, 0")
    I(f"s_cmp_le_i32 {sreg(59)}, {sreg(60)}")
    I(f"s_cbranch_scc1 {skip_label}")
    I(f"s_mov_b32 {sreg(rows_dst)}, {sreg(59)}")
    if full:
        I(f"s_mov_b32 {sreg(S_ROWLO)}, {sreg(60)}")
        I(f"s_mov_b32 {sreg(S_LDO)}, {sreg(S_VC2)}")
        I(f"s_add_i32 {sreg(S_T2)}, {sreg(m0r)}, {sreg(S_VSHIFT)}")
        I(f"s_mul_i32 {sreg(S_T0)}, {sreg(S_T2)}, {sreg(S_VC2)}")
        I(f"s_mul_hi_i32 {sreg(S_T1)}, {sreg(S_T2)}, {sreg(S_VC2)}")
        I(f"s_sub_u32 {sreg(58)}, {sreg(n0)}, {sreg(S_VCOL0)}")
        I(f"s_lshl_b32 {sreg(58)}, {sreg(58)}, 1")
        I(f"s_add_u32 {sreg(S_T0)}, {sreg(S_T0)}, {sreg(58)}")
        I(f"s_addc_u32 {sreg(S_T1)}, {sreg(S_T1)}, 0")
        add64(g, S_Y, S_VOUT, S_T0, S_T1)
    g.L(lab)


def generate(WN: int, epi: int, prefix: str, i8: bool = False, persistent: bool = False, mfma: int = 32) -> str:
    c = Cfg(WN, epi, i8, mfma)
    assert not (persistent and (i8 or epi in (EPI_PARTIAL, EPI_BIAS_SSQ)))
    g = Gen()
    I = g.I
    T = 128
    npw = c.npw
    def ident():
        I(f"v_and_b32 {vreg(c.V_LANE)}, 63, {vreg(V_TID)}")
        I(f"v_lshrrev_b32 {vreg(T)}, 6, {vreg(V_TID)}")
        I("s_nop 0")
        I(f"v_readfirstlane_b32 {sreg(S_WAVE)}, {vreg(T)}")
        I(f"v_and_b32 {vreg(c.V_R)}, 31, {vreg(c.V_LANE)}")
        I(f"v_lshrrev_b32 {vreg(c.V_H)}, 5, {vreg(c.V_LANE)}")
    if persistent:
        ident()
        I(f"s_mov_b32 {sreg(S_PF)}, 0")
        g.L(f"{prefix}_TILE")
        gen_tile_map(g, S_TILE, T)
        gen_tile_bases(g, c, S_X, S_W, S_ROWS, f"{prefix}_NEXT", True, prefix)
    if not persistent:
        ident()
    for rs, base, rows, ld in ((S_XRS, S_X, S_ROWS, S_LDX), (S_WRS, S_W, S_COLS, S_LDW)):
        I(f"s_mov_b32 {sreg(rs)}, {sreg(base)}")
        I(f"s_and_b32 {sreg(rs + 1)}, {sreg(base + 1)}, 0xffff")
        I(f"s_min_u32 {sreg(S_T0)}, {sreg(rows)}, 256")
        I(f"s_mul_i32 {sreg(rs + 2)}, {sreg(S_T0)}, {sreg(ld)}")
        I(f"s_mov_b32 {sreg(rs + 3)}, 0x00020000")
    I(f"s_mov_b32 {sreg(S_XK)}, 0")
    I(f"s_mov_b32 {sreg(S_WK)}, 0")
    I(f"s_lshl_b32 {sreg(S_WKMAX)}, {sreg(S_NK)}, 7")
    I(f"s_sub_u32 {sreg(S_WKMAX)}, {sreg(S_WKMAX)}, 128")
    I(f"s_mov_b32 {sreg(S_XKMAX)}, {sreg(S_WKMAX)}")
    I(f"s_mul_i32 {sreg(S_WM0)}, {sreg(S_WAVE)}, {1024 * npw}")
    I(f"s_mul_i32 {sreg(S_XM0)}, {sreg(S_WAVE)}, {XU * c.xunit}")
    I(f"s_add_u32 {sreg(S_XM0)}, {sreg(S_XM0)}, {c.xbase}")
    I(f"v_lshrrev_b32 {vreg(T)}, 3, {vreg(c.V_LANE)}")
    I(f"v_and_b32 {vreg(T + 1)}, 7, {vreg(c.V_LANE)}")
    for dst, cnt, ld in ((c.V_DW, npw, S_LDW), (c.V_DX, 8, S_LDX)):
        I(f"s_mul_i32 {sreg(S_T0)}, {sreg(S_WAVE)}, {8 * cnt}")
        for i in range(cnt):
            I(f"v_add_u32 {vreg(T + 2)}, {sreg(S_T0)}, {vreg(T)}")
            I(f"v_add_u32 {vreg(T + 2)}, {8 * i}, {vreg(T + 2)}")
            I(f"v_lshrrev_b32 {vreg(T + 3)}, 1, {vreg(T + 2)}")
            I(f"v_and_b32 {vreg(T + 3)}, 7, {vreg(T + 3)}")
            I(f"v_xor_b32 {vreg(T + 3)}, {vreg(T + 3)}, {vreg(T + 1)}")
            I(f"v_lshlrev_b32 {vreg(T + 3)}, 4, {vreg(T + 3)}")
            I(f"v_mul_lo_u32 {vreg(dst + i)}, {vreg(T + 2)}, {sreg(ld)}")
            I(f"v_add_u32 {vreg(dst + i)}, {vreg(dst + i)}, {vreg(T + 3)}")
    I(f"s_lshl_b32 {sreg(S_T0)}, {sreg(S_WAVE)}, 6")
    for mb in range(c.MB):
        I(f"v_add_u32 {vreg(c.V_ROW + mb)}, {sreg(S_T0)}, {vreg(c.V_R)}")
        if mb:
            I(f"v_add_u32 {vreg(c.V_ROW + mb)}, {32 * mb}, {vreg(c.V_ROW + mb)}")
    if c.m16:
        I(f"v_and_b32 {vreg(T + 1)}, 15, {vreg(c.V_LANE)}")
        I(f"v_lshrrev_b32 {vreg(T + 3)}, 4, {vreg(c.V_LANE)}")
        I(f"v_lshrrev_b32 {vreg(T)}, 1, {vreg(T + 1)}")
        I(f"v_lshlrev_b32 {vreg(T + 1)}, 7, {vreg(T + 1)}")
    else:
        I(f"v_lshrrev_b32 {vreg(T)}, 1, {vreg(c.V_R)}")
        I(f"v_and_b32 {vreg(T)}, 7, {vreg(T)}")
        I(f"v_lshlrev_b32 {vreg(T + 1)}, 7, {vreg(c.V_R)}")
    for hs in range(2):
        if c.m16:
            I(f"v_add_u32 {vreg(T + 2)}, {4 * hs}, {vreg(T + 3)}")
            I(f"v_xor_b32 {vreg(T + 2)}, {vreg(T + 2)}, {vreg(T)}")
            I(f"v_lshl_add_u32 {vreg(c.V_WOFF + 2 * hs)}, {vreg(T + 2)}, 4, {vreg(T + 1)}")
            I(f"v_add_u32 {vreg(c.V_WOFF + 4 + 2 * hs)}, 0x10000, {vreg(c.V_WOFF + 2 * hs)}")
            I(f"v_add_u32 {vreg(c.V_WOFF + 8 + 2 * hs)}, 0x20000, {vreg(c.V_WOFF + 2 * hs)}")
            I(f"v_add_u32 {vreg(c.V_XROFF + 2 * hs)}, {sreg(S_XM0)}, {vreg(c.V_WOFF + 2 * hs)}")
            continue
        for ks in range(2):
            I(f"v_add_u32 {vreg(T + 2)}, {4 * hs + 2 * ks}, {vreg(c.V_H)}")
            I(f"v_xor_b32 {vreg(T + 2)}, {vreg(T + 2)}, {vreg(T)}")
            I(f"v_lshl_add_u32 {vreg(c.V_WOFF + 2 * hs + ks)}, {vreg(T + 2)}, 4, {vreg(T + 1)}")
            I(f"v_add_u32 {vreg(c.V_WOFF + 4 + 2 * hs + ks)}, 0x10000, {vreg(c.V_WOFF + 2 * hs + ks)}")
            I(f"v_add_u32 {vreg(c.V_WOFF + 8 + 2 * hs + ks)}, 0x20000, {vreg(c.V_WOFF + 2 * hs + ks)}")
            I(f"v_add_u32 {vreg(c.V_XROFF + 2 * hs + ks)}, {sreg(S_XM0)}, {vreg(c.V_WOFF + 2 * hs + ks)}")
    I(f"s_cmp_ge_u32 {sreg(S_T0)}, {sreg(S_ROWS)}")
    I(f"s_cbranch_scc1 {prefix}_IDLE")
    n_early = gen_epilogue_setup(g, c)
    if persistent:
        I(f"s_cmp_eq_u32 {sreg(S_PF)}, 1")
        I(f"s_cbranch_scc1 {prefix}_STAGED")
    for j in range(NSLOT):
        for op in w_dma(c, j):
            I(op)
        if j < XU:
            for op in x_dma(c, j):
                I(op)
    for r in range(c.nacc):
        I(f"v_accvgpr_write_b32 {areg(r)}, 0")
    I(f"s_waitcnt vmcnt({2 * npw + 8})")
    if persistent:
        I(f"s_branch {prefix}_READY")
        g.L(f"{prefix}_STAGED")
        I(f"s_mov_b32 {sreg(S_WK)}, {128 * NSLOT}")
        I(f"s_min_u32 {sreg(S_WK)}, {sreg(S_WK)}, {sreg(S_WKMAX)}")
        I(f"s_mov_b32 {sreg(S_XK)}, {128 * XU}")
        I(f"s_min_u32 {sreg(S_XK)}, {sreg(S_XK)}, {sreg(S_XKMAX)}")
        for r in range(c.nacc):
            I(f"v_accvgpr_write_b32 {areg(r)}, 0")
        I(f"s_waitcnt vmcnt({n_early})")
        g.L(f"{prefix}_READY")
    I("s_barrier")
    for op in x_frag_reads(c, 0) + w_frag_reads(c, 0):
        I(op)
    I("s_waitcnt lgkmcnt(0)")
    I(f"s_mov_b32 {sreg(S_I)}, 0")
    period = 2 * NSLOT * XU // (2 if NSLOT % 2 == 0 else 1)
    sc = c.sc
    assert (period // 2) % NSLOT == 0 and (period // 2) % XU == 0
    g.L(f"{prefix}_LOOP")
    for h in range(period):
        s = h >> 1
        mm = mfmas(c, h)
        n = len(mm)
        wr = [] if KN("NO_WREAD") else w_frag_reads(c, h + 1)
        if h & 1 == 0:
            fillers = [(0.6 * sc + k * (n - 6 * sc) / len(wr), op) for k, op in enumerate(wr)] if wr else []
            xd = x_dma(c, s + 2)
            fillers += spread(drop_loads(xd) if KN("NO_X") else xd, 1.3 * sc, n - 1.5 * sc)
            g.phase([] if KN("NO_MFMA") else mm, fillers)
            I(f"s_waitcnt vmcnt({npw + 8})")
            I("s_barrier")
        else:
            xr = [] if KN("NO_WREAD") else x_frag_reads(c, s + 1)
            fillers = [((0.3 + k * 0.5) * sc, op) for k, op in enumerate(xr)]
            fillers += [(4.6 * sc + k * (n - 10 * sc) / len(wr), op) for k, op in enumerate(wr)] if wr else []
            wd = w_dma(c, s + 3)
            fillers += spread(drop_loads(wd) if KN("NO_W") else wd, 1.3 * sc, n - 1.5 * sc)
            g.phase([] if KN("NO_MFMA") else mm, fillers)
            I(f"s_add_u32 {sreg(S_I)}, {sreg(S_I)}, 1")
            I(f"s_cmp_ge_u32 {sreg(S_I)}, {sreg(S_NK)}")
            I(f"s_cbranch_scc1 {prefix}_EPI")
    I(f"s_branch {prefix}_LOOP")
    g.L(f"{prefix}_EPI")
    I("s_nop 15")
    I("s_nop 15")
    if KN("NO_EPI") and not persistent:
        I("s_waitcnt vmcnt(0)")
        I("s_endpgm")
    if persistent:
        gen_prefetch(g, c, prefix, "A")
    tail_stores = 0 if KN("NO_EPI") else gen_epilogue(g, c)
    if persistent:
        g.L(f"{prefix}_NEXT")
        I(f"s_add_u32 {sreg(S_TILE)}, {sreg(S_TILE)}, {sreg(S_GRID)}")
        I(f"s_cmp_lt_u32 {sreg(S_TILE)}, {sreg(S_NTILES)}")
        I(f"s_cbranch_scc1 {prefix}_TILE")
    I(f"s_waitcnt vmcnt({0 if persistent else min(63, tail_stores)})")
    I("s_endpgm")
    g.L(f"{prefix}_IDLE")
    if persistent:
        I(f"s_cmp_eq_u32 {sreg(S_PF)}, 1")
        I(f"s_cbranch_scc1 {prefix}_IDLE_STAGED")
    for j in range(NSLOT):
        for op in w_dma(c, j):
            I(op)
    I(f"s_waitcnt vmcnt({2 * npw})")
    if persistent:
        I(f"s_branch {prefix}_IDLE_READY")
        g.L(f"{prefix}_IDLE_STAGED")
        I(f"s_mov_b32 {sreg(S_WK)}, {128 * NSLOT}")
        I(f"s_min_u32 {sreg(S_WK)}, {sreg(S_WK)}, {sreg(S_WKMAX)}")
        I("s_waitcnt vmcnt(0)")
        g.L(f"{prefix}_IDLE_READY")
    I("s_barrier")
    I(f"s_mov_b32 {sreg(S_I)}, 0")
    g.L(f"{prefix}_IDLE_LOOP")
    for st in range(NSLOT):
        I(f"s_waitcnt vmcnt({npw})")
        I("s_barrier")
        for op in w_dma(c, st + 3):
            I(op)
        I(f"s_add_u32 {sreg(S_I)}, {sreg(S_I)}, 1")
        I(f"s_cmp_ge_u32 {sreg(S_I)}, {sreg(S_NK)}")
        I(f"s_cbranch_scc1 {prefix}_IDLE_END")
    I(f"s_branch {prefix}_IDLE_LOOP")
    g.L(f"{prefix}_IDLE_END")
    if persistent:
        gen_prefetch(g, c, prefix, "I")
        I(f"s_branch {prefix}_NEXT")
    else:
        I("s_waitcnt vmcnt(0)")
        I("s_endpgm")
    return finalize(g.out)


def gen_prefetch(g: Gen, c: Cfg, prefix: str, tag: str):
    I = g.I
    T = 128
    npw = c.npw
    I("s_barrier")
    I(f"s_mov_b32 {sreg(S_PF)}, 0")
    I(f"s_add_u32 {sreg(S_I)}, {sreg(S_TILE)}, {sreg(S_GRID)}")
    I(f"s_cmp_ge_u32 {sreg(S_I)}, {sreg(S_NTILES)}")
    I(f"s_cbranch_scc1 {prefix}_PF_DONE_{tag}")
    gen_tile_map(g, S_I, T)
    gen_tile_bases(g, c, S_XN, S_WN, S_ROWSN, f"{prefix}_PF_DONE_{tag}", False, prefix)
    I(f"s_mov_b32 {sreg(S_PF)}, 1")
    for rs, base, rows, ld in ((S_WRS, S_WN, None, S_LDW), (S_XRS, S_XN, S_ROWSN, S_LDX)):
        I(f"s_mov_b32 {sreg(rs)}, {sreg(base)}")
        I(f"s_and_b32 {sreg(rs + 1)}, {sreg(base + 1)}, 0xffff")
        if rows is None:
            I(f"s_mul_i32 {sreg(rs + 2)}, {sreg(ld)}, {c.WN}")
        else:
            I(f"s_min_u32 {sreg(S_T0)}, {sreg(rows)}, 256")
            I(f"s_mul_i32 {sreg(rs + 2)}, {sreg(S_T0)}, {sreg(ld)}")
        I(f"s_mov_b32 {sreg(rs + 3)}, 0x00020000")
    I(f"s_mov_b32 {sreg(S_XK)}, 0")
    I(f"s_mov_b32 {sreg(S_WK)}, 0")
    I(f"s_lshl_b32 {sreg(S_T0)}, {sreg(S_WAVE)}, 6")
    I(f"s_cmp_ge_u32 {sreg(S_T0)}, {sreg(S_ROWSN)}")
    I(f"s_cbranch_scc1 {prefix}_PF_WONLY_{tag}")
    for j in range(NSLOT):
        for op in w_dma(c, j):
            I(op)
        if j < XU:
            for op in x_dma(c, j):
                I(op)
    I(f"s_branch {prefix}_PF_DONE_{tag}")
    g.L(f"{prefix}_PF_WONLY_{tag}")
    for j in range(NSLOT):
        for op in w_dma(c, j):
            I(op)
    g.L(f"{prefix}_PF_DONE_{tag}")



def gen_epilogue_setup(g: Gen, c: Cfg):
    I = g.I
    T = c.V_T
    epi = c.epi
    EA = c.V_EA
    for mb in range(c.MB):
        I(f"v_mul_lo_u32 {vreg(EA + mb)}, {vreg(c.V_ROW + mb)}, {sreg(S_LDO)}")
        I(f"v_lshl_add_u32 {vreg(EA + mb)}, {vreg(c.V_H)}, 4, {vreg(EA + mb)}")
    R16, Q16 = T + 60, T + 61
    if c.m16:
        I(f"v_and_b32 {vreg(R16)}, 0xffffffef, {vreg(c.V_ROW)}")
        I(f"v_lshrrev_b32 {vreg(Q16)}, 4, {vreg(c.V_LANE)}")
        I(f"v_lshlrev_b32 {vreg(EA + 2)}, 3, {vreg(Q16)}")
    else:
        I(f"v_lshlrev_b32 {vreg(EA + 2)}, 3, {vreg(c.V_H)}")
    if epi == EPI_GATE_RES:
        I(f"s_sub_u32 {sreg(S_T1)}, {sreg(S_ROWS)}, 1")
        for mb in range(4 if c.m16 else c.MB):
            m, q, t = T + 66, EA + 3 + mb, T + 48
            if c.m16:
                I(f"v_add_u32 {vreg(m)}, {16 * mb}, {vreg(R16)}")
                I(f"v_min_u32 {vreg(m)}, {sreg(S_T1)}, {vreg(m)}")
            else:
                I(f"v_min_u32 {vreg(m)}, {sreg(S_T1)}, {vreg(c.V_ROW + mb)}")
            I(f"v_add_u32 {vreg(m)}, {sreg(S_M0)}, {vreg(m)}")
            I(f"v_cvt_f32_u32 {vreg(t)}, {vreg(m)}")
            I(f"v_cvt_f32_u32 {vreg(t + 1)}, {sreg(S_FLEN)}")
            I(f"v_rcp_f32 {vreg(t + 1)}, {vreg(t + 1)}")
            I("s_nop 0")
            I(f"v_mul_f32 {vreg(t)}, {vreg(t)}, {vreg(t + 1)}")
            I(f"v_cvt_u32_f32 {vreg(q)}, {vreg(t)}")
            I(f"v_mul_lo_u32 {vreg(t)}, {vreg(q)}, {sreg(S_FLEN)}")
            I(f"v_cmp_gt_u32_e64 {sreg(S_MSK, 2)}, {vreg(t)}, {vreg(m)}")
            I(f"v_cndmask_b32_e64 {vreg(t + 2)}, 0, 1, {sreg(S_MSK, 2)}")
            I(f"v_sub_u32 {vreg(q)}, {vreg(q)}, {vreg(t + 2)}")
            I(f"v_mul_lo_u32 {vreg(t)}, {vreg(q)}, {sreg(S_FLEN)}")
            I(f"v_add_u32 {vreg(t)}, {sreg(S_FLEN)}, {vreg(t)}")
            I(f"v_cmp_le_u32_e64 {sreg(S_MSK, 2)}, {vreg(t)}, {vreg(m)}")
            I(f"v_cndmask_b32_e64 {vreg(t + 2)}, 0, 1, {sreg(S_MSK, 2)}")
            I(f"v_add_u32 {vreg(q)}, {vreg(q)}, {vreg(t + 2)}")
            I(f"v_mul_lo_u32 {vreg(q)}, {vreg(q)}, {sreg(S_GSTRIDE)}")
            I(f"v_lshl_add_u32 {vreg(q)}, {vreg(Q16 if c.m16 else c.V_H)}, 3, {vreg(q)}")
    for mb in range(c.MB):
        I(f"v_cmp_lt_u32_e64 {sreg(S_MSK + 2 * mb, 2)}, {vreg(c.V_ROW + mb)}, {sreg(S_ROWS)}")
        I(f"v_cmp_ge_u32_e64 vcc, {vreg(c.V_ROW + mb)}, {sreg(S_ROWLO)}")
        I(f"s_and_b64 {sreg(S_MSK + 2 * mb, 2)}, {sreg(S_MSK + 2 * mb, 2)}, vcc")
    if c.i8:
        I(f"v_lshlrev_b32 {vreg(EA + 5)}, 4, {vreg(c.V_H)}")
        I(f"s_sub_u32 {sreg(S_T1)}, {sreg(S_ROWS)}, 1")
        for mb in range(c.MB):
            I(f"v_min_u32 {vreg(T + 48)}, {sreg(S_T1)}, {vreg(c.V_ROW + mb)}")
            I(f"v_lshlrev_b32 {vreg(T + 48)}, 2, {vreg(T + 48)}")
            I(f"global_load_dword {vreg(c.V_SX + 2 * mb)}, {vreg(T + 48)}, {sreg(S_SX, 2)}")
    n0 = sum(1 for l in g.out if l.startswith("global_load"))
    for nb in range(c.early_nb):
        for g4 in range(c.bl):
            I(f"global_load_dwordx2 {vreg(c.V_EB + 8 * nb + 2 * g4, 2)}, {vreg(EA + 2)}, {sreg(S_BIAS, 2)} offset:{64 * nb + (64 // c.bl) * g4}")
    if c.nl:
        epi_block_loads(g, c, 0, c.V_E0)
    return sum(1 for l in g.out if l.startswith("global_load")) - n0 + (c.MB if c.i8 else 0)


def epi_block_loads(g: Gen, c: Cfg, j: int, P: int):
    I = g.I
    nb, mb = j // c.MB, j % c.MB
    EA = c.V_EA
    if c.epi == EPI_GATE_RES:
        for g4 in range(4):
            if c.m16:
                I(f"global_load_dwordx2 {vreg(P + 2 * g4, 2)}, {vreg(EA + 3 + 2 * mb + (g4 & 1))}, {sreg(S_GATE, 2)} offset:{64 * nb + 32 * (g4 >> 1)}")
                continue
            I(f"global_load_dwordx2 {vreg(P + 2 * g4, 2)}, {vreg(EA + 3 + mb)}, {sreg(S_GATE, 2)} offset:{64 * nb + 16 * g4}")
    if c.epi in (EPI_GATE_RES, EPI_RES):
        I(f"s_mov_b64 exec, {sreg(S_MSK + 2 * mb, 2)}")
        for k in (0, 2):
            I(f"global_load_dwordx4 {vreg(P + 8 + 2 * k, 4)}, {vreg(EA + mb)}, {sreg(S_RES, 2)} offset:{64 * nb + 16 * k}")
        I("s_mov_b64 exec, -1")


def gen_epilogue(g: Gen, c: Cfg):
    I = g.I
    T = c.V_T
    epi = c.epi
    EA = c.V_EA
    K0, K1, CEXP = 0.7978845608028654, 0.044715, -2.0 * 1.4426950408889634
    cons = {}
    def const_pair(name, val, s0):
        I(f"s_mov_b32 {sreg(s0)}, {hex(f32bits(val))}")
        I(f"s_mov_b32 {sreg(s0 + 1)}, {hex(f32bits(val))}")
        cons[name] = s0
    if epi == EPI_GELU:
        const_pair("k1", K1, 54); const_pair("k0", K0, 56); const_pair("ce", CEXP, 58); const_pair("one", 1.0, 60)
    if epi == EPI_BIAS_SSQ:
        for k in range((4 if c.m16 else 2) * c.MB):
            I(f"v_mov_b32 {vreg(c.V_SS + k)}, 0")
    if epi == EPI_PARTIAL:
        for nb in range(c.NB):
            for mb in range(c.MB):
                a0 = c.acc(mb, nb)
                for r in range(16):
                    I(f"v_accvgpr_read_b32 {vreg(T + r)}, {areg(a0 + r)}")
                I(f"s_mov_b64 exec, {sreg(S_MSK + 2 * mb, 2)}")
                for g4 in range(4):
                    I(f"global_store_dwordx4 {vreg(EA + mb)}, {vreg(T + 4 * g4, 4)}, {sreg(S_Y, 2)} offset:{128 * nb + 32 * g4}")
                I("s_mov_b64 exec, -1")
        return 4 * c.NB * c.MB
    BB, PB = T + 72, T + 72 + 8 * c.NB
    assert PB + 32 <= min(c.V_WOFF + 32, 256), (PB, c.V_WOFF)
    n_late = c.bl * (c.NB - c.early_nb)
    q = []
    SWB = PB + 32
    assert not c.i8 or SWB + 32 <= c.V_LANE, (SWB, c.V_LANE)

    def wait_for(tags):
        idx = [i for i, t in enumerate(q) if t in tags]
        return None if not idx else min(63, len(q) - 1 - idx[-1])

    def sw_loads(nb):
        for g4 in range(4):
            I(f"global_load_dwordx4 {vreg(SWB + 16 * (nb & 1) + 4 * g4, 4)}, {vreg(EA + 5)}, {sreg(S_SW, 2)} offset:{128 * nb + 32 * g4}")
        q.extend([("sw", nb)] * 4)

    for nb in range(c.early_nb, c.NB):
        for g4 in range(c.bl):
            I(f"global_load_dwordx2 {vreg(BB + 8 * nb + 2 * g4, 2)}, {vreg(EA + 2)}, {sreg(S_BIAS, 2)} offset:{64 * nb + (64 // c.bl) * g4}")
        q.extend([("bias", nb)] * c.bl)
    if c.i8:
        sw_loads(0)
        for mb in range(c.MB):
            I(f"v_mov_b32 {vreg(c.V_SX + 2 * mb + 1)}, {vreg(c.V_SX + 2 * mb)}")
    blocks = [(nb, mb) for nb in range(c.NB) for mb in range(c.MB)]
    nl = c.nl

    for j, (nb, mb) in enumerate(blocks):
        P = c.V_E0 if j == 0 else PB + 16 * (j & 1)
        if c.i8 and mb == 0 and nb + 1 < c.NB:
            sw_loads(nb + 1)
        if nl and j + 1 < len(blocks):
            epi_block_loads(g, c, j + 1, PB + 16 * ((j + 1) & 1))
            q.extend([("blk", j + 1)] * nl)
        nxt_loads = nl if (nl and j + 1 < len(blocks)) else 0
        if c.i8:
            need = [("blk", j)] + ([("bias", nb), ("sw", nb)] if mb == 0 else [])
            n = wait_for(need)
            if n is not None:
                I(f"s_waitcnt vmcnt({n})")
        elif nl and j == 0:
            I(f"s_waitcnt vmcnt({(n_late if c.early_nb else 0) + nxt_loads})")
        elif nl:
            I(f"s_waitcnt vmcnt({2 + nxt_loads})")
        elif c.early_nb == 0 and j == 0:
            I("s_waitcnt vmcnt(0)")
        if not nl and mb == 0 and nb == c.early_nb and 0 < c.early_nb < c.NB:
            I(f"s_waitcnt vmcnt({min(63, 2 * j)})")
        if mb == 0:
            for g4 in range(4):
                for d in range(2):
                    src = (c.V_EB if nb < c.early_nb else BB) + 8 * nb + 2 * (g4 >> 1 if c.m16 else g4) + d
                    I(f"v_lshlrev_b32 {vreg(T + 24 + 4 * g4 + 2 * d)}, 16, {vreg(src)}")
                    I(f"v_and_b32 {vreg(T + 24 + 4 * g4 + 2 * d + 1)}, 0xffff0000, {vreg(src)}")
        a0 = c.acc(mb, nb)
        for r in range(16):
            src = c.acc16(2 * mb + ((r >> 2) & 1), 2 * nb + (r >> 3)) + (r & 3) if c.m16 else a0 + r
            I(f"v_accvgpr_read_b32 {vreg(T + r)}, {areg(src)}")
        if c.i8:
            for r in range(16):
                I(f"v_cvt_f32_i32 {vreg(T + r)}, {vreg(T + r)}")
            for r in range(0, 16, 2):
                I(f"v_pk_mul_f32 {vreg(T + 56, 2)}, {vreg(SWB + 16 * (nb & 1) + r, 2)}, {vreg(c.V_SX + 2 * mb, 2)}")
                I(f"v_pk_mul_f32 {vreg(T + r, 2)}, {vreg(T + r, 2)}, {vreg(T + 56, 2)}")
        for r in range(0, 16, 2):
            I(f"v_pk_add_f32 {vreg(T + r, 2)}, {vreg(T + r, 2)}, {vreg(T + 24 + r, 2)}")
        for r in range(0, 16, 2):
            I(f"v_cvt_pk_bf16_f32 {vreg(T + 16 + r // 2)}, {vreg(T + r)}, {vreg(T + r + 1)}")
        if epi in (EPI_GELU, EPI_GATE_RES, EPI_BIAS_SSQ):
            for r in range(0, 16, 2):
                I(f"v_lshlrev_b32 {vreg(T + r)}, 16, {vreg(T + 16 + r // 2)}")
                I(f"v_and_b32 {vreg(T + r + 1)}, 0xffff0000, {vreg(T + 16 + r // 2)}")
        if epi == EPI_BIAS_SSQ:
            for r in range(0, 16, 2):
                ss = c.V_SS + 2 * (2 * mb + ((r >> 2) & 1) if c.m16 else mb)
                I(f"v_pk_fma_f32 {vreg(ss, 2)}, {vreg(T + r, 2)}, {vreg(T + r, 2)}, {vreg(ss, 2)}")
        if epi == EPI_GATE_RES:
            for r in range(0, 16, 2):
                src = P + r // 2
                I(f"v_lshlrev_b32 {vreg(T + 56)}, 16, {vreg(src)}")
                I(f"v_and_b32 {vreg(T + 57)}, 0xffff0000, {vreg(src)}")
                I(f"v_pk_mul_f32 {vreg(T + r, 2)}, {vreg(T + r, 2)}, {vreg(T + 56, 2)}")
            for r in range(0, 16, 2):
                I(f"v_cvt_pk_bf16_f32 {vreg(T + 16 + r // 2)}, {vreg(T + r)}, {vreg(T + r + 1)}")
        if epi == EPI_GELU:
            for r in range(0, 16, 2):
                x, t = vreg(T + r, 2), vreg(T + 44 + (r % 4), 2)
                I(f"v_pk_mul_f32 {t}, {sreg(cons['k1'], 2)}, {x}")
                I(f"v_pk_mul_f32 {t}, {t}, {x}")
                I(f"v_pk_mul_f32 {t}, {t}, {x}")
                I(f"v_pk_add_f32 {t}, {x}, {t}")
                I(f"v_pk_mul_f32 {t}, {sreg(cons['k0'], 2)}, {t}")
                I(f"v_pk_mul_f32 {t}, {sreg(cons['ce'], 2)}, {t}")
                I(f"v_exp_f32 {vreg(T + 44 + (r % 4))}, {vreg(T + 44 + (r % 4))}")
                I(f"v_exp_f32 {vreg(T + 45 + (r % 4))}, {vreg(T + 45 + (r % 4))}")
                I("s_nop 0")
                I(f"v_pk_add_f32 {t}, {sreg(cons['one'], 2)}, {t}")
                I(f"v_rcp_f32 {vreg(T + 44 + (r % 4))}, {vreg(T + 44 + (r % 4))}")
                I(f"v_rcp_f32 {vreg(T + 45 + (r % 4))}, {vreg(T + 45 + (r % 4))}")
                I("s_nop 0")
                I(f"v_pk_mul_f32 {x}, {x}, {t}")
            for r in range(0, 16, 2):
                I(f"v_cvt_pk_bf16_f32 {vreg(T + 16 + r // 2)}, {vreg(T + r)}, {vreg(T + r + 1)}")
        for k in (0, 2):
            ax, ay, bx, by = T + 16 + 2 * k, T + 17 + 2 * k, T + 18 + 2 * k, T + 19 + 2 * k
            I("s_nop 1")
            swap = "v_permlane16_swap_b32" if c.m16 else "v_permlane32_swap_b32"
            I(f"{swap} {vreg(ax)}, {vreg(bx)}")
            I(f"{swap} {vreg(ay)}, {vreg(by)}")
        off_y = 64 * nb
        if epi in (EPI_GATE_RES, EPI_RES):
            for k in (0, 2):
                for d in range(4):
                    vsrc, rsrc = T + 16 + 2 * k + d, P + 8 + 2 * k + d
                    I(f"v_lshlrev_b32 {vreg(T)}, 16, {vreg(vsrc)}")
                    I(f"v_and_b32 {vreg(T + 1)}, 0xffff0000, {vreg(vsrc)}")
                    I(f"v_lshlrev_b32 {vreg(T + 2)}, 16, {vreg(rsrc)}")
                    I(f"v_and_b32 {vreg(T + 3)}, 0xffff0000, {vreg(rsrc)}")
                    I(f"v_pk_add_f32 {vreg(T, 2)}, {vreg(T + 2, 2)}, {vreg(T, 2)}")
                    I(f"v_cvt_pk_bf16_f32 {vreg(vsrc)}, {vreg(T)}, {vreg(T + 1)}")
        I(f"s_mov_b64 exec, {sreg(S_MSK + 2 * mb, 2)}")
        for k in (0, 2):
            I(f"global_store_dwordx4 {vreg(EA + mb)}, {vreg(T + 16 + 2 * k, 4)}, {sreg(S_Y, 2)} offset:{off_y + 16 * k}")
        I("s_mov_b64 exec, -1")
        q.extend([("st", j)] * 2)
    if epi == EPI_BIAS_SSQ and c.m16:
        R16, Q16 = T + 8, T + 9
        I(f"v_and_b32 {vreg(R16)}, 0xffffffef, {vreg(c.V_ROW)}")
        I(f"v_lshrrev_b32 {vreg(Q16)}, 4, {vreg(c.V_LANE)}")
        for step in ("v_permlane32_swap_b32", "v_permlane16_swap_b32"):
            for mb in range(4):
                ss = c.V_SS + 2 * mb
                I(f"v_add_f32 {vreg(ss)}, {vreg(ss)}, {vreg(ss + 1)}")
                I(f"v_mov_b32 {vreg(ss + 1)}, {vreg(ss)}")
            I("s_nop 1")
            for mb in range(4):
                ss = c.V_SS + 2 * mb
                I(f"{step} {vreg(ss)}, {vreg(ss + 1)}")
        for mb in range(4):
            ss = c.V_SS + 2 * mb
            I(f"v_add_f32 {vreg(ss)}, {vreg(ss)}, {vreg(ss + 1)}")
            I(f"v_add_u32 {vreg(T + mb)}, {16 * mb}, {vreg(R16)}")
            I(f"v_cmp_lt_u32_e64 vcc, {vreg(T + mb)}, {sreg(S_ROWS)}")
            I(f"v_cmp_eq_u32_e64 {sreg(S_MT, 2)}, {vreg(Q16)}, 0")
            I(f"s_and_b64 vcc, vcc, {sreg(S_MT, 2)}")
            I(f"v_lshlrev_b32 {vreg(T + mb)}, 2, {vreg(T + mb)}")
            I("s_mov_b64 exec, vcc")
            I(f"global_store_dword {vreg(T + mb)}, {vreg(ss)}, {sreg(S_SSQ, 2)}")
            I("s_mov_b64 exec, -1")
            q.append(("st", "ssq"))
    elif epi == EPI_BIAS_SSQ:
        for mb in range(c.MB):
            ss = c.V_SS + 2 * mb
            I(f"v_add_f32 {vreg(ss)}, {vreg(ss)}, {vreg(ss + 1)}")
            I(f"v_mov_b32 {vreg(ss + 1)}, {vreg(ss)}")
        I("s_nop 1")
        for mb in range(c.MB):
            ss = c.V_SS + 2 * mb
            I(f"v_permlane32_swap_b32 {vreg(ss)}, {vreg(ss + 1)}")
        for mb in range(c.MB):
            ss = c.V_SS + 2 * mb
            I(f"v_add_f32 {vreg(ss)}, {vreg(ss)}, {vreg(ss + 1)}")
            I(f"v_lshlrev_b32 {vreg(T + mb)}, 2, {vreg(c.V_ROW + mb)}")
            I(f"v_cmp_eq_u32_e64 vcc, {vreg(c.V_H)}, 0")
            I(f"s_and_b64 vcc, vcc, {sreg(S_MSK + 2 * mb, 2)}")
            I("s_mov_b64 exec, vcc")
            I(f"global_store_dword {vreg(T + mb)}, {vreg(ss)}, {sreg(S_SSQ, 2)}")
            I("s_mov_b64 exec, -1")
            q.append(("st", "ssq"))
    n = 0
    while n < len(q) and q[len(q) - 1 - n][0] == "st":
        n += 1
    return n


if __name__ == "__main__":
    if "--diag" in sys.argv:
        sys.argv.remove("--diag")
    WN, epi = int(sys.argv[1]), int(sys.argv[2])
    form = sys.argv[5] if len(sys.argv) > 5 else ""
    i8, pers, mfma = form == "i8", form in ("p", "pm16"), 16 if form in ("m16", "pm16") else 32
    txt = generate(WN, epi, f"GA{WN}E{epi}" + ("I8" if i8 else "") + ("P" if pers else "") + ("M16" if mfma == 16 else ""), i8, pers, mfma)
    probs = lint(txt)
    for p in probs[:20]:
        print("LINT:", p, file=sys.stderr)
    if len(sys.argv) > 3:
        open(sys.argv[3], "w").write(to_inc(txt))
    if len(sys.argv) > 4:
        open(sys.argv[4], "w").write(txt)
    n = sum(1 for l in txt.splitlines() if l and not l.endswith(":"))
    print(f"gemm WN={WN} epi={epi}: {n} instructions, {len(probs)} lint findings", file=sys.stderr)
    sys.exit(1 if probs else 0)
```

### longlive_amd/model.py

```python
from __future__ import annotations

import math
from typing import Callable, Dict, List, NamedTuple, Optional, Tuple

import torch
import torch.nn as nn

from . import ops
from .kv_cache import KVPlan, plan_update, shadow_refresh_ranges
from .synth import WanConfig

bf16 = torch.bfloat16


class _Lin(nn.Module):
    def __init__(self, out_f: int, in_f: int, device, dtype):
        super().__init__()
        self.weight = nn.Parameter(torch.zeros(out_f, in_f, device=device, dtype=dtype), requires_grad=False)
        self.bias = nn.Parameter(torch.zeros(out_f, device=device, dtype=dtype), requires_grad=False)


class _Norm(nn.Module):
    def __init__(self, dim: int, device, dtype, bias: bool = False):
        super().__init__()
        self.weight = nn.Parameter(torch.ones(dim, device=device, dtype=dtype), requires_grad=False)
        if bias:
            self.bias = nn.Parameter(torch.zeros(dim, device=device, dtype=dtype), requires_grad=False)


class _Attn(nn.Module):
    def __init__(self, dim, device, dtype):
        super().__init__()
        self.q, self.k, self.v, self.o = (_Lin(dim, dim, device, dtype) for _ in range(4))
        self.norm_q, self.norm_k = _Norm(dim, device, dtype), _Norm(dim, device, dtype)
        self.max_attention_size = 32760


class _Block(nn.Module):
    def __init__(self, cfg: WanConfig, device, dtype):
        super().__init__()
        d = cfg.dim
        self.self_attn = _Attn(d, device, dtype)
        self.cross_attn = _Attn(d, device, dtype)
        del self.cross_attn.max_attention_size
        self.norm3 = _Norm(d, device, dtype, bias=True)
        self.ffn = nn.ModuleList([_Lin(cfg.ffn_dim, d, device, dtype), nn.Identity(), _Lin(d, cfg.ffn_dim, device, dtype)])
        self.modulation = nn.Parameter(torch.zeros(1, 6, d, device=device, dtype=dtype), requires_grad=False)


class _Head(nn.Module):
    def __init__(self, cfg: WanConfig, device, dtype):
        super().__init__()
        self.head = _Lin(math.prod(cfg.patch_size) * cfg.out_dim, cfg.dim, device, dtype)
        self.modulation = nn.Parameter(torch.zeros(1, 2, cfg.dim, device=device, dtype=dtype), requires_grad=False)


class _Conv(nn.Module):
    def __init__(self, cfg: WanConfig, device, dtype):
        super().__init__()
        self.weight = nn.Parameter(torch.zeros(cfg.dim, cfg.in_dim, *cfg.patch_size, device=device, dtype=dtype),
                                   requires_grad=False)
        self.bias = nn.Parameter(torch.zeros(cfg.dim, device=device, dtype=dtype), requires_grad=False)


class _QuantMode(NamedTuple):
    quantize_w: Optional[Callable]
    quantize_x: Optional[Callable]
    ln_modulate: Callable
    ln_modulate_tab: Callable
    layernorm_affine: Callable
    gemm: Callable
    gemm_qkv: Callable
    mx_out: bool
    granule: int
    afmt: Optional[ops.QFormat] = None


def _op(name: str) -> Callable:
    return lambda *a, **kw: getattr(ops, name)(*a, **kw)


def _quant_mode(wq: str, xq: str, act: str, gemm: str, mx_out: bool, granule: int) -> _QuantMode:
    return _QuantMode(_op(wq), _op(xq), _op("ln_modulate_" + act), _op("ln_modulate_tab_" + act), _op("layernorm_affine_" + act),
                      _op("gemm_" + gemm), _op(f"gemm_{gemm}_qkv_v_insert"), mx_out, granule, getattr(ops, act.upper()) if act.startswith("mx") else None)


def _rowwise(gemm: str) -> Callable:
    return lambda x, w, *a, **kw: getattr(ops, gemm)(*x, *w, *a, **kw)


_QUANT_MODES = {
    None: _QuantMode(None, None, _op("ln_modulate"), _op("ln_modulate_tab"), _op("layernorm_affine"), _op("gemm"),
                     lambda x, w, b, cache_v, ws, ro, wl, B, L: ops.gemm_qkv_v_insert(x, w, b, cache_v, ws, ro, wl), False, 1),
    "int8": _quant_mode("quantize_rows", "quantize_rows", "q8", "w8a8", False, 128)._replace(
        ln_modulate_tab=lambda *a: ops.ln_modulate_tab(*a, q8=True), gemm=_rowwise("gemm_w8a8"),
        gemm_qkv=lambda x, w, b, cache_v, ws, ro, wl, B, L: ops.gemm_qkv_v_insert(None, w, b, cache_v, ws, ro, wl, xq=x)),
    "mxfp8": _quant_mode("quantize_mx", "quantize_mx", "mx", "mx", True, 128),
    "fp8_rowwise": _quant_mode("quantize_rows_f8", "quantize_rows_f8", "f8", "f8", False, 128)._replace(gemm=_rowwise("gemm_f8")),
    "mxfp6": _quant_mode("quantize_mx6", "quantize_mx6", "mx6", "mx6", True, 256),
    "mxfp4_a6": _quant_mode("quantize_mx4", "quantize_mx6", "mx6", "mx4w6", True, 256),
    "mxfp4_a4": _quant_mode("quantize_mx4", "quantize_mx4", "mx4", "mx4", True, 256),
}


_MX_SHADOW = "_ll_mx"


def mx_shadow_key(k: torch.Tensor, v: torch.Tensor) -> tuple:
    return (k.data_ptr(), v.data_ptr(), tuple(k.shape), k._version, v._version)


def _idx_versions(cache: dict):
    g, e = cache.get("global_end_index"), cache.get("local_end_index")
    return (g._version if torch.is_tensor(g) else ("int", g), e._version if torch.is_tensor(e) else ("int", e))


def _kv_state(cache: dict) -> Tuple[int, int]:
    st = cache.get("_ll_idx")
    if st is not None and len(st) == 4 and st[2:] != list(_idx_versions(cache)):
        st = None
    if st is None:
        g, e = cache["global_end_index"], cache["local_end_index"]
        st = [int(g.item()) if torch.is_tensor(g) else int(g), int(e.item()) if torch.is_tensor(e) else int(e),
              *_idx_versions(cache)]
        cache["_ll_idx"] = st
    return st[0], st[1]


def _kv_commit(cache: dict, G: int, E: int) -> None:
    for key, val in (("global_end_index", G), ("local_end_index", E)):
        cur = cache.get(key)
        if torch.is_tensor(cur):
            cur.fill_(val)
        else:
            cache[key] = val
    cache["_ll_idx"] = [G, E, *_idx_versions(cache)]


class CausalWanModelHIP(nn.Module):

    rope_frames = 1024

    def __init__(self, cfg: WanConfig, device="cuda", dtype=bf16):
        super().__init__()
        assert dtype == bf16, "the HIP path computes in bf16 (inference.py:134)"
        assert cfg.head_dim == 128, "kernels are specialised for head_dim 128 (Wan2.1-T2V-1.3B: 1536 / 12)"
        assert cfg.patch_size == (1, 2, 2)
        self.cfg = cfg
        d = cfg.dim
        self.patch_embedding = _Conv(cfg, device, dtype)
        self.text_embedding = nn.ModuleList([_Lin(d, cfg.text_dim, device, dtype), nn.Identity(), _Lin(d, d, device, dtype)])
        self.time_embedding = nn.ModuleList([_Lin(d, cfg.freq_dim, device, dtype), nn.Identity(), _Lin(d, d, device, dtype)])
        self.time_projection = nn.ModuleList([nn.Identity(), _Lin(6 * d, d, device, dtype)])
        self.blocks = nn.ModuleList([_Block(cfg, device, dtype) for _ in range(cfg.num_layers)])
        self.head = _Head(cfg, device, dtype)
        self.local_attn_size = cfg.local_attn_size
        self.sink_size = cfg.sink_size
        self.max_attention_size = 32760 if cfg.local_attn_size == -1 else cfg.local_attn_size * 1560
        for b in self.blocks:
            b.self_attn.max_attention_size = self.max_attention_size
        self.num_frame_per_block = 1
        self.block_mask = None
        self.quant: Optional[str] = None
        self.attn_quant: Optional[str] = None
        self.use_modulation_table = True
        self.fuse_v_insert = True
        self.use_modulation_f32 = True
        self.fuse_attn_quant = False
        self.fuse_cross_qnorm = True
        self._packed = None
        self._rope_f = None
        self._rope_hw: Dict[Tuple[int, int], torch.Tensor] = {}
        self._ctx_cache = None
        self._time_memo: Dict[tuple, tuple] = {}
        self._register_load_state_dict_pre_hook(self._invalidate_derived)

    def _apply(self, fn, *a, **k):
        self._packed = None
        self._rope_f = None
        self._rope_hw = {}
        self._ctx_cache = None
        self._time_memo = {}
        return super()._apply(fn, *a, **k)

    def _invalidate_derived(self, *unused_hook_args):
        self._packed = None
        self._ctx_cache = None
        self._time_memo = {}

    def invalidate_packed(self):
        self._invalidate_derived()

    def load_state_dict(self, state_dict, strict: bool = True, **kw):
        self._invalidate_derived()
        return super().load_state_dict(state_dict, strict=strict, **kw)

    @staticmethod
    def _prepare_blockwise_causal_attn_mask(*args, **kwargs):
        return None

    def _param_key(self):
        key = []
        for blk in self.blocks:
            sa = blk.self_attn
            ts = [sa.q.weight, sa.k.weight, sa.v.weight, sa.q.bias, sa.k.bias, sa.v.bias, blk.modulation]
            if self.quant is not None:
                ts += [sa.o.weight, blk.cross_attn.q.weight, blk.cross_attn.o.weight, blk.ffn[0].weight, blk.ffn[2].weight]
            key.extend((t.data_ptr(), t._version) for t in ts)
        return tuple(key)

    def _pack(self):
        if self._packed is not None:
            if self._packed_key == self._param_key():
                return self._packed
            self._invalidate_derived()
        P = []
        for blk in self.blocks:
            sa, ca = blk.self_attn, blk.cross_attn
            d = dict(
                wqkv=torch.cat([sa.q.weight, sa.k.weight, sa.v.weight], 0).contiguous(),
                bqkv=torch.cat([sa.q.bias, sa.k.bias, sa.v.bias], 0).contiguous(),
                mod=blk.modulation.detach().reshape(6, -1).contiguous(),
            )
            quantize = _QUANT_MODES[self.quant].quantize_w
            if quantize is not None:
                for name, w in (("qkv", d["wqkv"]), ("o", sa.o.weight), ("cq", ca.q.weight), ("co", ca.o.weight),
                                ("f1", blk.ffn[0].weight), ("f2", blk.ffn[2].weight)):
                    d["q_" + name], d["s_" + name] = quantize(w.detach().contiguous())
            P.append(d)
        self._packed = P
        self._mods = torch.stack([d["mod"] for d in P], 0).contiguous()
        self._packed_key = self._param_key()
        return P

    def set_quant(self, mode: Optional[str]):
        if mode not in _QUANT_MODES:
            raise ValueError(f"unknown quantisation mode {mode!r}")
        granule = _QUANT_MODES[mode].granule
        if granule >= 128 and (self.cfg.dim % 128 or self.cfg.ffn_dim % 128):
            raise ValueError(f"{mode} linears need dim and ffn_dim to be multiples of 128")
        if granule == 256 and (self.cfg.dim % 256 or self.cfg.ffn_dim % 256):
            raise ValueError(f"{mode} linears need dim and ffn_dim to be multiples of 256 (packed 256-k super-blocks)")
        self.quant = mode
        self._packed = None
        return self

    def set_attn_quant(self, mode: Optional[str]):
        if mode not in (None, "mxfp8"):
            raise ValueError(f"unknown attention quantisation mode {mode!r}")
        if mode is not None and self.cfg.head_dim != 128:
            raise ValueError("MX attention needs head_dim 128")
        self.attn_quant = mode
        return self

    @staticmethod
    def _mx_shadow(kvc: dict):
        k = kvc["k"]
        sh = kvc.get(_MX_SHADOW)
        if sh is None or sh["kq"].shape[0] != k.shape[0] or sh["S"] != k.shape[1] or sh["kq"].shape[2] != k.shape[2]:
            sh = ops.kv_shadow_mx_alloc(k)
            sh["key"] = None
            kvc[_MX_SHADOW] = sh
        return sh, sh["key"] != mx_shadow_key(k, kvc["v"])

    def _lin(self, x, pk, key, w, b, epilogue=0, **kw):
        m = _QUANT_MODES[self.quant]
        if m.quantize_w is not None:
            w = (pk["q_" + key], pk["s_" + key])
            if not isinstance(x, tuple):
                x = m.quantize_x(x)
        return m.gemm(x, w, b, epilogue, tag="gemm_" + key, **kw)

    def _rope_tables(self, hp: int, wp: int, device):
        d = self.cfg.head_dim
        half = d // 2
        c3 = half // 3
        nf = half - 2 * c3

        def angles(n, dim):
            return torch.outer(torch.arange(n, dtype=torch.float64),
                               1.0 / torch.pow(10000.0, torch.arange(0, dim, 2, dtype=torch.float64).div(dim)))

        if self._rope_f is None:
            a = angles(self.rope_frames, d - 4 * (d // 6))
            assert a.shape[1] == nf
            self._rope_f = torch.stack([a.cos(), a.sin()], -1).float().contiguous().to(device)
        key = (hp, wp)
        if key not in self._rope_hw:
            ah = angles(1024, 2 * (d // 6))[:hp]
            aw = angles(1024, 2 * (d // 6))[:wp]
            a = torch.cat([ah.view(hp, 1, c3).expand(hp, wp, c3), aw.view(1, wp, c3).expand(hp, wp, c3)], -1)
            a = a.reshape(hp * wp, 2 * c3)
            self._rope_hw[key] = torch.stack([a.cos(), a.sin()], -1).float().contiguous().to(device)
        return self._rope_f, self._rope_hw[key]

    def time_embed(self, t: torch.Tensor):
        c = self.cfg
        tf = t.reshape(-1).to(torch.float32).contiguous()
        emb = ops.sinusoid(tf, c.freq_dim)
        h = ops.linear_small(emb, self.time_embedding[0].weight, self.time_embedding[0].bias, act_out=1)
        e = ops.linear_small(h, self.time_embedding[2].weight, self.time_embedding[2].bias)
        e0 = ops.linear_small(e, self.time_projection[1].weight, self.time_projection[1].bias, act_in=1)
        return e, e0.view(*t.shape, 6, c.dim)

    def _time_param_key(self):
        ps = (self.time_embedding[0].weight, self.time_embedding[0].bias, self.time_embedding[2].weight, self.time_embedding[2].bias,
              self.time_projection[1].weight, self.time_projection[1].bias)
        return tuple((p.data_ptr(), p._version) for p in ps)

    def text_embed(self, context: torch.Tensor):
        key = (context.data_ptr(), (context._version, torch.cuda.current_stream(context.device).cuda_stream if context.is_cuda else 0))
        if self._ctx_cache is not None and self._ctx_cache[:2] == key:
            return self._ctx_cache[2]
        c = self.cfg
        ctx = context.to(bf16)
        if ctx.shape[1] < c.text_len:
            ctx = torch.cat([ctx, ctx.new_zeros(ctx.shape[0], c.text_len - ctx.shape[1], ctx.shape[2])], 1)
        ctx = ctx.contiguous()
        h = ops.gemm(ctx, self.text_embedding[0].weight, self.text_embedding[0].bias, ops.EPI_BIAS_GELU)
        out = ops.gemm(h, self.text_embedding[2].weight, self.text_embedding[2].bias)
        self._ctx_cache = (key[0], key[1], out, context)
        return out

    @torch.no_grad()
    def block_forward(self, i: int, xs: torch.Tensor, e0: torch.Tensor, ctx: Optional[torch.Tensor], kvc: dict,
                      cac: dict, F: int, grid_hw: Tuple[int, int], current_start: int,
                      sink_recache_after_switch: bool = False, q_buf: Optional[torch.Tensor] = None,
                      kv_insert_only: bool = False, pk: Optional[dict] = None, premod: bool = False,
                      cache_done_event=None, co_running: bool = False, tab32: Optional[torch.Tensor] = None) -> KVPlan:
        c = self.cfg
        B, L, C = xs.shape
        Hh, D = c.num_heads, c.head_dim
        hp, wp = grid_hw
        fs = hp * wp
        if L != F * fs:
            raise ValueError(f"block_forward: {L} tokens are not {F} frames of {hp}x{wp}")
        rope_f, rope_hw = self._rope_tables(hp, wp, xs.device)
        if q_buf is None:
            q_buf = torch.empty(B, L, Hh, D, dtype=bf16, device=xs.device)
        blk = self.blocks[i]
        if pk is None:
            pk = self._pack()[i]
        mod = None if premod else pk["mod"]
        sa, ca = blk.self_attn, blk.cross_attn
        m = _QUANT_MODES[self.quant]
        G, E = _kv_state(kvc)
        S = kvc["k"].shape[1]
        plan = plan_update(current_start, L, G, E, S, self.sink_size * fs, self.local_attn_size,
                           sa.max_attention_size, sink_recache_after_switch)
        amx = self.attn_quant == "mxfp8"
        ofmt = m.afmt if self.fuse_attn_quant else None
        if amx:
            shadow, stale = self._mx_shadow(kvc)
        else:
            kvc.pop(_MX_SHADOW, None)
        if plan.roll is not None:
            ops.kv_roll(kvc["k"], kvc["v"], *plan.roll)
        h1 = m.ln_modulate_tab(xs, tab32, 0, 1, F, c.eps) if tab32 is not None else m.ln_modulate(xs, e0, mod, 0, 1, F, c.eps)
        if self.fuse_v_insert:
            qkv = m.gemm_qkv(h1, pk["wqkv"] if m.quantize_w is None else (pk["q_qkv"], pk["s_qkv"]), pk["bqkv"], kvc["v"],
                             plan.write_start, plan.roped_offset, plan.write_len, B, L)
            v_dst = None
        else:
            qkv = self._lin(h1, pk, "qkv", pk["wqkv"], pk["bqkv"])
            v_dst = kvc["v"]
        ops.qk_norm_rope_kv_store(qkv, sa.norm_q.weight, sa.norm_k.weight, rope_f, rope_hw, q_buf.view(B, L, C),
                                  kvc["k"], v_dst, D, fs, current_start // fs, plan.write_start,
                                  plan.roped_offset, plan.write_len, c.eps)
        if amx:
            for lo, hi in shadow_refresh_ranges(plan, stale, S):
                ops.kv_shadow_mx(kvc["k"], kvc["v"], shadow, lo, hi, tag="kv_shadow_mx_co" if co_running else "kv_shadow_mx")
            shadow["key"] = mx_shadow_key(kvc["k"], kvc["v"])
        if kv_insert_only:
            if cache_done_event is not None:
                cache_done_event.record(torch.cuda.current_stream())
            return plan
        if amx:
            att = ops.flash_attn_mx(q_buf, shadow, plan.segments, tag="flash_attn_self_mx_co" if co_running else "flash_attn_self_mx",
                                    out_fmt=ofmt)
        else:
            att = ops.flash_attn(q_buf, kvc["k"], kvc["v"], plan.segments, tag="flash_attn_self_co" if co_running else "flash_attn_self",
                                 out_fmt=ofmt)
        if cache_done_event is not None:
            cache_done_event.record(torch.cuda.current_stream())
        self._lin(att if ofmt is not None else att.view(B, L, C), pk, "o", sa.o.weight, sa.o.bias, ops.EPI_BIAS_GATE_RES, out=xs, res=xs, e=e0,
                  mod=mod, gate_idx=2, rows_per_batch=L, frame_len=fs)
        xn = m.layernorm_affine(xs, blk.norm3.weight, blk.norm3.bias, c.eps)
        fuse_qn = (self.fuse_cross_qnorm and self.quant is None and ops.gemm_ssq_planes(B * L, C, C) == Hh and ops.flash_attn_qnorm_ok(Hh, c.text_len))
        if fuse_qn:
            qraw, ssq = ops.gemm_ssq(xn, ca.q.weight, ca.q.bias, tag="gemm_cq_ssq")
        else:
            qc = ops.rmsnorm(self._lin(xn, pk, "cq", ca.q.weight, ca.q.bias), ca.norm_q.weight, c.eps)
        if not cac["is_init"]:
            kc = ops.gemm(ctx, ca.k.weight, ca.k.bias)
            if cac["k"].shape != (B, c.text_len, Hh, D) or not cac["k"].is_contiguous():
                cac["k"] = torch.empty(B, c.text_len, Hh, D, dtype=bf16, device=xs.device)
                cac["v"] = torch.empty(B, c.text_len, Hh, D, dtype=bf16, device=xs.device)
            ops.rmsnorm(kc, ca.norm_k.weight, c.eps, out=cac["k"].view(B, c.text_len, C))
            ops.gemm(ctx, ca.v.weight, ca.v.bias, out=cac["v"].view(B, c.text_len, C))
            cac["is_init"] = True
        if fuse_qn:
            atc = ops.flash_attn_qnorm(qraw.view(B, L, Hh, D), ssq, ca.norm_q.weight, c.eps, cac["k"], cac["v"], c.text_len, tag="flash_attn_cross_qn")
        else:
            atc = ops.flash_attn(qc.view(B, L, Hh, D), cac["k"], cac["v"], [(0, c.text_len)], tag="flash_attn_cross", out_fmt=ofmt)
        self._lin(atc if isinstance(atc, tuple) else atc.view(B, L, C), pk, "co", ca.o.weight, ca.o.bias, ops.EPI_BIAS_RES, out=xs, res=xs)
        h2 = m.ln_modulate_tab(xs, tab32, 3, 4, F, c.eps) if tab32 is not None else m.ln_modulate(xs, e0, mod, 3, 4, F, c.eps)
        ff = self._lin(h2, pk, "f1", blk.ffn[0].weight, blk.ffn[0].bias, ops.EPI_BIAS_GELU,
                       **(dict(mx_out=True) if m.mx_out else {}))
        self._lin(ff, pk, "f2", blk.ffn[2].weight, blk.ffn[2].bias, ops.EPI_BIAS_GATE_RES, out=xs, res=xs, e=e0,
                  mod=mod, gate_idx=5, rows_per_batch=L, frame_len=fs)
        return plan

    @torch.no_grad()
    def forward_frames(self, x: torch.Tensor, t: torch.Tensor, context: torch.Tensor, kv_cache: List[dict],
                       crossattn_cache: List[dict], current_start: int = 0,
                       sink_recache_after_switch: bool = False, sigma: Optional[torch.Tensor] = None,
                       kv_only: bool = False, layer_wait=None, layer_record=None, t_uniform: Optional[float] = None):
        c = self.cfg
        B, F, Cin, H, W = x.shape
        hp, wp = H // 2, W // 2
        fs = hp * wp
        L = F * fs
        Hh, D, C = c.num_heads, c.head_dim, c.dim
        assert current_start % fs == 0, "current_start must sit on a frame boundary"
        x = x.to(bf16).contiguous()
        pe = self.patch_embedding
        xs = ops.gemm(ops.patchify(x), pe.weight.view(C, -1), pe.bias)
        need_ctx = any(not cc["is_init"] for cc in crossattn_cache)
        ctx = self.text_embed(context) if need_ctx else None

        q_buf = torch.empty(B, L, Hh, D, dtype=bf16, device=x.device)
        plans: List[KVPlan] = []
        last = len(self.blocks) - 1
        P = self._pack()
        premod = self.use_modulation_table
        tab_f32 = premod and self.use_modulation_f32 and x.is_cuda
        memo_key = None
        if t_uniform is not None and x.is_cuda and tuple(t.shape) == (B, F):
            memo_key = (float(t_uniform), B, F, premod, tab_f32, torch.cuda.current_stream(x.device).cuda_stream)
            hit = self._time_memo.get(memo_key)
            if hit is not None and hit[0] == self._time_param_key() and hit[1] is self._packed_key:
                e, e0, etab, etab32 = hit[2:]
            else:
                hit = None
        if memo_key is None or hit is None:
            e, e0 = self.time_embed(t)
            etab = ops.modulation_table(e0, self._mods) if premod else None
            etab32 = ops.modulation_table_f32(e0, self._mods, 0b010010) if tab_f32 else None
            if memo_key is not None:
                if len(self._time_memo) >= 64:
                    self._time_memo = {}
                self._time_memo[memo_key] = (self._time_param_key(), self._packed_key, e, e0, etab, etab32)
        cur_stream = torch.cuda.current_stream() if (layer_wait is not None or layer_record is not None) else None
        for i in range(len(self.blocks)):
            if layer_wait is not None:
                cur_stream.wait_event(layer_wait[i])
            plans.append(self.block_forward(i, xs, etab[i] if premod else e0, ctx, kv_cache[i], crossattn_cache[i], F, (hp, wp),
                                            current_start, sink_recache_after_switch, q_buf,
                                            kv_insert_only=kv_only and i == last, pk=P[i], premod=premod,
                                            cache_done_event=layer_record[i] if layer_record is not None else None,
                                            co_running=cur_stream is not None, tab32=etab32[i] if tab_f32 else None))
        for kvc, plan in zip(kv_cache, plans):
            _kv_commit(kvc, plan.G_new, plan.E_new)
        if kv_only:
            return (None, None) if sigma is not None else None
        eh = e.view(B, F, 1, C).expand(B, F, 2, C).contiguous()
        hd = ops.ln_modulate(xs, eh, self.head.modulation.view(2, C), 0, 1, F, c.eps)
        ho = ops.gemm(hd, self.head.head.weight, self.head.head.bias)
        if sigma is None:
            return ho
        return ops.unpatchify_x0(ho, x, sigma)

    def forward(self, x, t=None, context=None, seq_len=None, kv_cache=None, crossattn_cache=None,
                current_start: int = 0, cache_start=None, sink_recache_after_switch: bool = False, **unused):
        if kv_cache is None:
            raise NotImplementedError("only the KV-cache inference branch exists (the reference's training branch "
                                      "is itself a stub: causal_model.py:1102-1103)")
        xf = x.permute(0, 2, 1, 3, 4).contiguous()
        B, F = xf.shape[:2]
        zero = torch.zeros(B * F, dtype=torch.float32, device=xf.device)
        flow, _ = self.forward_frames(xf, t, context, kv_cache, crossattn_cache, current_start,
                                      sink_recache_after_switch, sigma=zero)
        return flow.permute(0, 2, 1, 3, 4)
```

### longlive_amd/ops.py

```python
from __future__ import annotations

import functools
import math
from dataclasses import dataclass
from typing import Optional, Tuple

import torch

from . import _lib

bf16 = torch.bfloat16

EPI_BIAS, EPI_BIAS_GELU, EPI_BIAS_GATE_RES, EPI_BIAS_RES = 0, 1, 2, 3


def _stream() -> int:
    return torch.cuda.current_stream().cuda_stream


class KernelTimer:

    def __init__(self, tags=None):
        self.tags = None if tags is None else set(tags)
        self.records = {}
# ... 105 lines not shown
    else:
        out = torch.empty_like(x)
        q = sc = None
    t0 = _t0(tag)
    _lib.check(lib.ll_ln_modulate_tab(x.data_ptr(), _ptr(out), _ptr(q), _ptr(sc), tab.data_ptr(), nmod, shift_idx, scale_idx,
                                      B, L, Cc, num_frames, eps, _stream()), "ll_ln_modulate_tab")
    _t1(tag, t0, (3.0 if q8 else 4.0) * B * L * Cc)
    return (q, sc) if q8 else out


def modulation_table(e, mods):
    _chk(e, "e"); _chk(mods, "mods")
    B, F, nmod, Cc = e.shape
    NL = mods.shape[0]
    assert mods.shape == (NL, nmod, Cc), (mods.shape, e.shape)
    out = torch.empty(NL, B, F, nmod, Cc, dtype=bf16, device=e.device)
    lib = _lib.load()
    _lib.check(lib.ll_modulation_table(e.data_ptr(), mods.data_ptr(), out.data_ptr(), NL, B * F, nmod, Cc, _stream()),
               "ll_modulation_table")
    return out


def layernorm_affine(x, w, b, eps: float, out=None):
    _chk(x, "x"); _chk(w, "w"); _chk(b, "b")
    Cc = x.shape[-1]
    assert w.numel() == Cc and b.numel() == Cc
    out = torch.empty_like(x) if out is None else _chk(out, "out")
    assert out.shape == x.shape
    lib = _lib.load()
    t0 = _t0("layernorm_affine")
    _lib.check(lib.ll_layernorm_affine(x.data_ptr(), w.data_ptr(), b.data_ptr(), out.data_ptr(), x.numel() // Cc, Cc,
                                       eps, _stream()), "ll_layernorm_affine")
    _t1("layernorm_affine", t0, 4.0 * x.numel())
    return out


def rmsnorm(x, w, eps: float, out=None, C: Optional[int] = None):
    assert x.dtype == bf16 and x.is_cuda and x.stride(-1) == 1
    Cc = x.shape[-1] if C is None else C
    x2 = x.flatten(0, -2) if x.dim() > 2 else x
    assert x2.dim() == 2 and x2.data_ptr() == x.data_ptr(), "rows of x must be evenly strided"
    rows, ldx = x2.shape[0], x2.stride(0)
    _chk(w, "w")
    assert w.numel() == Cc
    if out is None:
        out = torch.empty(rows, Cc, dtype=bf16, device=x.device)
    assert out.dtype == bf16 and out.is_cuda and out.stride(-1) == 1
    o2 = out.flatten(0, -2) if out.dim() > 2 else out
    assert o2.dim() == 2 and o2.data_ptr() == out.data_ptr() and o2.shape[0] == rows and o2.shape[1] >= Cc
    lib = _lib.load()
    t0 = _t0("rmsnorm")
    _lib.check(lib.ll_rmsnorm(x2.data_ptr(), w.data_ptr(), o2.data_ptr(), rows, Cc, ldx, o2.stride(0), eps, _stream()),
               "ll_rmsnorm")
    _t1("rmsnorm", t0, 4.0 * rows * Cc)
    return out


def qk_norm_rope_kv_store(qkv, wq, wk, rope_f, rope_hw, q_out, cache_k, cache_v, head_dim: int, frame_len: int,
                          start_frame: int, write_start: int, roped_offset: int, write_len: int, eps: float):
    _chk(qkv, "qkv"); _chk(wq, "wq"); _chk(wk, "wk"); _chk(q_out, "q_out"); _chk(cache_k, "cache_k")
    if cache_v is not None:
        _chk(cache_v, "cache_v")
    _chk(rope_f, "rope_f", torch.float32); _chk(rope_hw, "rope_hw", torch.float32)
    B, L, C3 = qkv.shape
    Cc = C3 // 3
    assert C3 == 3 * Cc and q_out.shape == (B, L, Cc)
    S = cache_k.shape[1]
    assert cache_k.shape[0] == B and cache_k.numel() == B * S * Cc and (cache_v is None or cache_v.shape == cache_k.shape)
    half = head_dim // 2
    nf = half - 2 * (half // 3)
    assert rope_f.shape == (1024, nf, 2), rope_f.shape
    assert rope_hw.shape == (frame_len, half - nf, 2), rope_hw.shape
    lib = _lib.load()
    t0 = _t0("qk_norm_rope_kv_store")
    _lib.check(lib.ll_qk_norm_rope_kv_store(qkv.data_ptr(), wq.data_ptr(), wk.data_ptr(), rope_f.data_ptr(),
                                            rope_hw.data_ptr(), q_out.data_ptr(), cache_k.data_ptr(),
                                            _ptr(cache_v), B, L, Cc, head_dim, frame_len, start_frame, S,
                                            write_start, roped_offset, write_len, eps, _stream()),
               "ll_qk_norm_rope_kv_store")
    nv = 1 if cache_v is not None else 0
    _t1("qk_norm_rope_kv_store", t0, 2.0 * ((2 + nv) * B * L * Cc + B * L * Cc + (1 + nv) * B * write_len * Cc))
    return q_out


def kv_roll(cache_k, cache_v, dst: int, src: int, n: int):
    _chk(cache_k, "cache_k"); _chk(cache_v, "cache_v")
    B, S = cache_k.shape[:2]
    Cc = cache_k.numel() // (B * S)
    assert cache_v.shape == cache_k.shape
    lib = _lib.load()
    t0 = _t0("kv_roll")
    _lib.check(lib.ll_kv_roll(cache_k.data_ptr(), cache_v.data_ptr(), B, S, Cc, dst, src, n, _stream()), "ll_kv_roll")
    _t1("kv_roll", t0, 2.0 * 2 * 2 * B * n * Cc)


def gemm(x, w, bias, epilogue: int = EPI_BIAS, out=None, res=None, e=None, mod=None, gate_idx: int = 0,
         rows_per_batch: int = 0, frame_len: int = 0, tag: str = "gemm"):
    _chk(x, "x"); _chk(w, "w"); _chk(bias, "bias")
    K = x.shape[-1]
    M = x.numel() // K
    N = w.shape[0]
    assert w.shape == (N, K) and bias.numel() == N, (w.shape, bias.shape, K)
    if out is None:
        out = torch.empty(*x.shape[:-1], N, dtype=bf16, device=x.device)
    _chk(out, "out")
    assert out.numel() == M * N
    nmod = 0
    if epilogue in (EPI_BIAS_GATE_RES, EPI_BIAS_RES):
        _chk(res, "res")
        assert res.numel() == M * N
    if epilogue == EPI_BIAS_GATE_RES:
        _chk(e, "e")
        nmod = e.shape[-2]
        assert e.shape[-1] == N and e.numel() == (M // frame_len) * nmod * N, (e.shape, M, frame_len)
        if mod is not None:
            _chk(mod, "mod")
            assert mod.numel() == nmod * N
    lib = _lib.load()
    t0 = _t0(tag)
    if M <= 1024 and M * N <= (1 << 22) and epilogue in (EPI_BIAS, EPI_BIAS_RES) and _ksplit_plan(lib, M, N, K):
        ws = ksplit_workspace(x.device, M, N, K)
        _lib.check(lib.ll_gemm_bf16_ksplit(x.data_ptr(), w.data_ptr(), bias.data_ptr(), out.data_ptr(), M, N, K, K, N, epilogue,
                                           _ptr(res), ws.data_ptr(), ws.numel(), _stream()), "ll_gemm_bf16_ksplit")
    else:
        _lib.check(lib.ll_gemm_bf16(x.data_ptr(), w.data_ptr(), bias.data_ptr(), out.data_ptr(), M, N, K, K, N, epilogue,
                                    _ptr(res), _ptr(e), _ptr(mod), nmod, gate_idx, rows_per_batch, frame_len, _stream()),
                   "ll_gemm_bf16")
    _t1(tag, t0, 2.0 * M * N * K)
    return out


def gemm_ssq_planes(M: int, N: int, K: int) -> int:
    return int(_lib.load().ll_gemm_ssq_planes(M, N, K))


def gemm_ssq(x, w, bias, out=None, tag: str = "gemm"):
    _chk(x, "x"); _chk(w, "w"); _chk(bias, "bias")
    K = x.shape[-1]
    M = x.numel() // K
    N = w.shape[0]
    assert w.shape == (N, K) and bias.numel() == N
    if out is None:
        out = torch.empty(*x.shape[:-1], N, dtype=bf16, device=x.device)
    _chk(out, "out")
    assert out.numel() == M * N
    planes = gemm_ssq_planes(M, N, K)
    if planes == 0:
        raise RuntimeError(f"gemm_ssq: {M} x {N} x {K} is not covered by the generated kernel (use gemm + rmsnorm)")
    ssq = torch.empty(planes, M, dtype=torch.float32, device=x.device)
    lib = _lib.load()
    t0 = _t0(tag)
    _lib.check(lib.ll_gemm_bf16_ssq(x.data_ptr(), w.data_ptr(), bias.data_ptr(), out.data_ptr(), ssq.data_ptr(), M, N, K, K, N, _stream()),
               "ll_gemm_bf16_ssq")
    _t1(tag, t0, 2.0 * M * N * K)
    return out, ssq


_ksplit_ws = {}


def _ksplit_plan(lib, M: int, N: int, K: int) -> int:
    return int(lib.ll_gemm_ksplit_plan(M, N, K))


def _dev_index(device) -> int:
    return torch.cuda.current_device() if device.index is None else device.index


def ksplit_workspace(device, M: int, N: int, K: int) -> torch.Tensor:
    need = int(_lib.load().ll_gemm_ksplit_workspace_bytes(M, N, K))
    key = (device.type, _dev_index(device), int(_stream() or 0))
    buf = _ksplit_ws.get(key)
    if buf is None or buf.numel() < need:
        buf = torch.empty(max(need, 16), dtype=torch.uint8, device=device)
        _ksplit_ws[key] = buf
    return buf


def gemm_qkv_v_insert(x, w, bias, cache_v, write_start: int, roped_offset: int, write_len: int, xq=None, tag: str = "gemm_qkv"):
    _chk(bias, "bias"); _chk(cache_v, "cache_v")
    int8 = xq is not None
    if int8:
        xi, sx = xq
        wq, sw = w
        _chk(xi, "xq", torch.int8); _chk(sx, "sx", torch.float32); _chk(wq, "wq", torch.int8); _chk(sw, "sw", torch.float32)
        B, L, K = xi.shape
        N = wq.shape[0]
        assert wq.shape == (N, K) and sx.numel() == B * L and sw.numel() == N
        dev = xi.device
    else:
        _chk(x, "x"); _chk(w, "w")
        B, L, K = x.shape
        N = w.shape[0]
        assert w.shape == (N, K)
        dev = x.device
    assert bias.numel() == N and N % 3 == 0
    S = cache_v.shape[1]
    assert cache_v.shape[0] == B and cache_v.numel() == B * S * (N // 3), (cache_v.shape, B, S, N)
    out = torch.empty(B, L, N, dtype=bf16, device=dev)
    lib = _lib.load()
    t0 = _t0(tag)
    if int8:
        _lib.check(lib.ll_gemm_w8a8_qkv(xi.data_ptr(), sx.data_ptr(), wq.data_ptr(), sw.data_ptr(), bias.data_ptr(), out.data_ptr(),
                                        B * L, N, K, N, cache_v.data_ptr(), B, L, S, write_start, roped_offset, write_len, _stream()),
                   "ll_gemm_w8a8_qkv")
    else:
        _lib.check(lib.ll_gemm_bf16_qkv(x.data_ptr(), w.data_ptr(), bias.data_ptr(), out.data_ptr(), B * L, N, K, K, N,
                                        cache_v.data_ptr(), B, L, S, write_start, roped_offset, write_len, _stream()),
                   "ll_gemm_bf16_qkv")
    _t1(tag, t0, 2.0 * B * L * N * K)
    return out


def quantize_rows(x, q=None, scale=None):
    _chk(x, "x")
    K = x.shape[-1]
    rows = x.numel() // K
    if q is None:
        q = torch.empty(x.shape, dtype=torch.int8, device=x.device)
    if scale is None:
        scale = torch.empty(rows, dtype=torch.float32, device=x.device)
    _chk(q, "q", torch.int8); _chk(scale, "scale", torch.float32)
    assert q.numel() == x.numel() and scale.numel() == rows
    lib = _lib.load()
    t0 = _t0("quantize_rows")
    _lib.check(lib.ll_quantize_rows(x.data_ptr(), q.data_ptr(), scale.data_ptr(), rows, K, K, _stream()), "ll_quantize_rows")
    _t1("quantize_rows", t0, 3.0 * x.numel())
    return q, scale


def linear_small(x, w, bias, act_in: int = 0, act_out: int = 0):
    _chk(x, "x"); _chk(w, "w"); _chk(bias, "bias")
    K = x.shape[-1]
    M = x.numel() // K
    N = w.shape[0]
    assert w.shape == (N, K) and bias.numel() == N
    out = torch.empty(*x.shape[:-1], N, dtype=bf16, device=x.device)
    lib = _lib.load()
    x2, o2 = x.view(M, K), out.view(M, N)
    for m0 in range(0, M, 8):
        m = min(8, M - m0)
        _lib.check(lib.ll_linear_small(x2[m0:].data_ptr(), w.data_ptr(), bias.data_ptr(), o2[m0:].data_ptr(), m, N, K,
                                       act_in, act_out, _stream()), "ll_linear_small")
    return out


def flash_attn(q, k, v, segments, out=None, scale: Optional[float] = None, tag: Optional[str] = None, out_fmt: Optional["QFormat"] = None):
    if out_fmt is not None:
        return _flash_attn_q(out_fmt, q, k, v, segments, scale, tag)
    _chk(q, "q"); _chk(k, "k"); _chk(v, "v")
    B, Lq, H, D = q.shape
    assert D == 128, "kernel is specialised for head_dim 128"
    Sk = k.shape[1]
    assert k.shape == (B, Sk, H, D) and v.shape == k.shape
    segs = [(int(a), int(b)) for a, b in segments if b > a]
    assert 1 <= len(segs) <= 2, segments
    for a, b_ in segs:
        assert 0 <= a < b_ <= Sk, (segments, Sk)
    (s0, e0) = segs[0]
    (s1, e1) = segs[1] if len(segs) == 2 else (0, 0)
    out = torch.empty_like(q) if out is None else _chk(out, "out")
    assert out.shape == q.shape
    if scale is None:
        scale = 1.0 / math.sqrt(D)
    lib = _lib.load()
    t0 = None
    if timer is not None:
        nkeys = (e0 - s0) + (e1 - s1)
        tag = tag or "flash_attn"
        t0 = timer.begin(tag)
    _lib.check(lib.ll_flash_attn(q.data_ptr(), k.data_ptr(), v.data_ptr(), out.data_ptr(), B, Lq, H, H * D, H * D,
                                 H * D, Sk * H * D, s0, e0 - s0, s1, e1 - s1, scale, _stream()),
               "ll_flash_attn")
    if timer is not None:
        timer.end(tag, t0, 4.0 * B * H * Lq * nkeys * D)
    return out


def flash_attn_qnorm_ok(H: int, nkeys: int) -> bool:
    return bool(_lib.load().ll_flash_attn_qnorm_ok(H, nkeys))


_QFMT_ID = {"mx": 1, "mx6": 2, "mx4": 3}


def _qfmt_id(fmt) -> int:
    assert fmt.name in _QFMT_ID, f"attention emits the block-scaled formats only (MX, MX6, MX4), not {fmt.name}"
    return _QFMT_ID[fmt.name]


def flash_attn_q_ok(fmt, H: int, segments) -> bool:
    s0, e0, s1, e1 = _segs2(segments, 1 << 30)
    return bool(_lib.load().ll_flash_attn_q_ok(_qfmt_id(fmt), H, s0, e0 - s0, s1, e1 - s1))


def flash_attn_q_plan(fmt, Lq: int, H: int, B: int, segments) -> str:
    import ctypes
    s0, e0, s1, e1 = _segs2(segments, 1 << 30)
    buf = ctypes.create_string_buffer(512)
    _lib.check(_lib.load().ll_flash_attn_q_plan(_qfmt_id(fmt), Lq, H, B, s0, e0 - s0, s1, e1 - s1, buf, 512), "ll_flash_attn_q_plan")
    return buf.value.decode()


def _flash_attn_q(fmt, q, k, v, segments, scale, tag):
    B, Lq, H, D = q.shape
    if not flash_attn_q_ok(fmt, H, segments):
# ... 926 lines not shown
```

Baseline: 92.94.

## Fold norm3 layernorm into cross-attn q GEMM via epilogue row statistics

```diff
diff --git a/include/longlive_hip.h b/include/longlive_hip.h
--- a/include/longlive_hip.h
+++ b/include/longlive_hip.h
@@ -175,6 +175,14 @@
 int ll_gemm_bf16_ssq(const ll_bf16* x, const ll_bf16* w, const ll_bf16* bias, ll_bf16* out, float* ssq, int M, int N, int K, int ldx,
                      int ldo, ll_stream stream);
 int ll_flash_attn_qnorm_ok(int H, int nkeys);
+
+int ll_gemm_fold_planes(int M, int C, int K, int frame_len);
+int ll_gemm_fold_plan(int M, int C, int K, int frame_len, char* out, int cap);
+int ll_gemm_bf16_gate_res_stats(const ll_bf16* x, const ll_bf16* w, const ll_bf16* bias, ll_bf16* out, float* sum, float* ssq, int M, int N, int K,
+                                int ldx, int ldo, const ll_bf16* res, const ll_bf16* e, int nmod, int gate_idx, int rows_per_batch,
+                                int frame_len, ll_stream stream);
+int ll_gemm_bf16_fold_ssq(const ll_bf16* x, const ll_bf16* w, const float* csum, const float* bfold, const float* psum, const float* pssq,
+                          float eps, ll_bf16* out, float* ssq, int M, int N, int K, int ldx, int ldo, ll_stream stream);
 int ll_flash_attn_qnorm(const ll_bf16* q, const float* ssq, const ll_bf16* norm_w, float eps, const ll_bf16* k, const ll_bf16* v,
                         ll_bf16* out, int B, int Lq, int H, int ldq, int ldo, int ldk, long long k_batch_stride, int key_start,
                         int nkeys, float scale, ll_stream stream);
diff --git a/longlive_amd/_lib.py b/longlive_amd/_lib.py
--- a/longlive_amd/_lib.py
+++ b/longlive_amd/_lib.py
@@ -46,6 +46,10 @@
     "ll_synth_hash": [_p, _ll, _ll, C.c_ulonglong, _i, _p],
     "ll_gemm_ssq_planes": [_i, _i, _i],
     "ll_gemm_bf16_ssq": [_p, _p, _p, _p, _p, _i, _i, _i, _i, _i, _p],
+    "ll_gemm_fold_planes": [_i, _i, _i, _i],
+    "ll_gemm_fold_plan": [_i, _i, _i, _i, C.c_char_p, _i],
+    "ll_gemm_bf16_gate_res_stats": [_p, _p, _p, _p, _p, _p, _i, _i, _i, _i, _i, _p, _p, _i, _i, _i, _i, _p],
+    "ll_gemm_bf16_fold_ssq": [_p, _p, _p, _p, _p, _p, _f, _p, _p, _i, _i, _i, _i, _i, _p],
     "ll_flash_attn_qnorm_ok": [_i, _i],
     "ll_flash_attn_qnorm": [_p, _p, _p, _f, _p, _p, _p, _i, _i, _i, _i, _i, _i, _ll, _i, _i, _f, _p],
     "ll_flash_attn_q_ok": [_i] * 6,
diff --git a/longlive_amd/csrc/gemm.hip b/longlive_amd/csrc/gemm.hip
--- a/longlive_amd/csrc/gemm.hip
+++ b/longlive_amd/csrc/gemm.hip
@@ -522,6 +522,50 @@
   return ll_check_launch("ll_gemm_bf16_ssq");
 }
 
+extern "C" int ll_gemm_fold_planes(int M, int C, int K, int frame_len) {
+  if (!gemm_asm_wanted(LL_EPI_BIAS) || M <= 0) return 0;
+  return gemm_asm_fold_planes(M, C, K, frame_len);
+}
+extern "C" int ll_gemm_fold_plan(int M, int C, int K, int frame_len, char* out, int cap) {
+  LL_REQUIRE(out != nullptr && cap > 0, "ll_gemm_fold_plan: needs an output buffer");
+  LL_REQUIRE(gemm_asm_wanted(LL_EPI_BIAS) && M > 0 && gemm_asm_fold_plan(M, C, K, frame_len, out, cap) != nullptr,
+             "ll_gemm_fold_plan: %d x %d x %d is not covered (ll_gemm_fold_planes)", M, C, K);
+  ll_plan_append_knobs(out, cap);
+  return LL_OK;
+}
+extern "C" int ll_gemm_bf16_gate_res_stats(const ll_bf16* x, const ll_bf16* w, const ll_bf16* bias, ll_bf16* out, float* sum, float* ssq, int M,
+                                           int N, int K, int ldx, int ldo, const ll_bf16* res, const ll_bf16* e, int nmod, int gate_idx,
+                                           int rows_per_batch, int frame_len, ll_stream stream) {
+  const char* fn = "ll_gemm_bf16_gate_res_stats";
+  if (int rc = FamBF16::check(fn, x, nullptr, w, nullptr, out, M, K, ldx, ldo)) return rc;
+  if (int rc = check_epilogue(fn, M, N, ldo, LL_EPI_BIAS_GATE_RES, bias, res, e, nullptr, nmod, gate_idx, rows_per_batch, frame_len)) return rc;
+  LL_REQUIRE(sum != nullptr && ssq != nullptr && (((size_t)sum | (size_t)ssq) & 3) == 0, "%s: sum and ssq are required", fn);
+  LL_REQUIRE(ll_gemm_fold_planes(M, N, K, frame_len) > 0 && ldx == K, "%s: %d x %d x %d is not covered by the generated kernel under the current "
+             "tuning (ask ll_gemm_fold_planes first and run ll_gemm_bf16 + ll_layernorm_affine instead)", fn, M, N, K);
+  EpiArgs ea{(const bf16*)bias, (const bf16*)res, (const bf16*)e, nullptr, nullptr, nullptr, nmod, gate_idx, rows_per_batch, frame_len,
+             frame_len > 0 && rows_per_batch > 0 ? rows_per_batch / frame_len : 0};
+  const int r = gemm_asm_stats_launch((const bf16*)x, (const bf16*)w, (bf16*)out, sum, ssq, M, N, K, ldx, ldo, ea, g_gemm_group_m, (hipStream_t)stream);
+  if (r < 0) return r;
+  LL_REQUIRE(r == 1, "%s: the generated kernel refused a shape its plan accepted", fn);
+  return ll_check_launch(fn);
+}
+extern "C" int ll_gemm_bf16_fold_ssq(const ll_bf16* x, const ll_bf16* w, const float* csum, const float* bfold, const float* psum, const float* pssq,
+                                     float eps, ll_bf16* out, float* ssq, int M, int N, int K, int ldx, int ldo, ll_stream stream) {
+  const char* fn = "ll_gemm_bf16_fold_ssq";
+  if (int rc = FamBF16::check(fn, x, nullptr, w, nullptr, out, M, K, ldx, ldo)) return rc;
+  LL_REQUIRE(x && w && out && N > 0 && ldo >= N && ldo % 8 == 0, "%s: x, w, out are required, ldo=%d must be >= N=%d and a multiple of 8", fn, ldo, N);
+  LL_REQUIRE(csum && bfold && psum && pssq && ssq && (((size_t)csum | (size_t)bfold) & 15) == 0 && (((size_t)psum | (size_t)pssq | (size_t)ssq) & 3) == 0,
+             "%s: csum and bfold (16-byte aligned), psum, pssq and ssq are required", fn);
+  LL_REQUIRE(N == K && ll_gemm_fold_planes(M, N, K, 1) > 0 && ll_gemm_ssq_planes(M, N, K) > 0 && ldx == K,
+             "%s: %d x %d x %d is not covered by the generated kernel under the current tuning (ask ll_gemm_fold_planes and "
+             "ll_gemm_ssq_planes first and run ll_layernorm_affine + ll_gemm_bf16_ssq instead)", fn, M, N, K);
+  const int r = gemm_asm_fold_launch((const bf16*)x, (const bf16*)w, csum, bfold, psum, pssq, eps, (bf16*)out, ssq, M, N, K, ldx, ldo,
+                                     g_gemm_group_m, (hipStream_t)stream);
+  if (r < 0) return r;
+  LL_REQUIRE(r == 1, "%s: the generated kernel refused a shape its plan accepted", fn);
+  return ll_check_launch(fn);
+}
+
 extern "C" int ll_gemm_ksplit_plan(int M, int N, int K) {
   if (!gemm_asm_wanted(LL_EPI_BIAS)) return 0;
   return gemm_ksplit_splits(M, N, K, device_cus());
diff --git a/longlive_amd/csrc/gemm_asm.h b/longlive_amd/csrc/gemm_asm.h
--- a/longlive_amd/csrc/gemm_asm.h
+++ b/longlive_amd/csrc/gemm_asm.h
@@ -26,6 +26,12 @@
                        int gm, hipStream_t s);
 int gemm_asm_ssq_launch(const bf16* x, const bf16* w, const bf16* bias, bf16* out, float* ssq, int M, int N, int K, int ldx, int ldo, int gm,
                         hipStream_t s);
+int gemm_asm_fold_planes(int M, int C, int K, int frame_len);
+const char* gemm_asm_fold_plan(int M, int C, int K, int frame_len, char* out, int cap);
+int gemm_asm_stats_launch(const bf16* x, const bf16* w, bf16* out, float* sum, float* ssq, int M, int N, int K, int ldx, int ldo, const EpiArgs& ea,
+                          int gm, hipStream_t s);
+int gemm_asm_fold_launch(const bf16* x, const bf16* w, const float* csum, const float* bfold, const float* psum, const float* pssq, float eps,
+                         bf16* out, float* ssq, int M, int N, int K, int ldx, int ldo, int gm, hipStream_t s);
 int gemm_ksplit_splits(int M, int N, int K, int cus);
 int gemm_asm_ksplit_launch(const bf16* x, const bf16* w, const bf16* bias, bf16* out, int M, int N, int K, int ldx, int ldo,
                            int epilogue, const bf16* res, float* workspace, int splits, int gm, hipStream_t s, const bf16* norm_w,
diff --git a/longlive_amd/csrc/gemm_asm.hip b/longlive_amd/csrc/gemm_asm.hip
--- a/longlive_amd/csrc/gemm_asm.hip
+++ b/longlive_amd/csrc/gemm_asm.hip
@@ -1,4 +1,6 @@
 #include "gemm_asm.h"
+
+#include <cstring>
 
 #define GA_EACH "gemm_asm_each.inl"
 #include "gemm_asm_kernels.def"
@@ -7,7 +9,7 @@
 #include "gemm_asm_kernels.def"
 #undef GA_TABLE
 };
-enum { GA_EPI_PARTIAL = 4, GA_EPI_SSQ = 5 };
+enum { GA_EPI_PARTIAL = 4, GA_EPI_SSQ = 5, GA_EPI_GATE_RES_STATS = 6, GA_EPI_FOLD_SSQ = 7 };
 
 int g_gemm_asm_persistent = 1;
 extern const int g_gemm_asm_mfma16_default = 511;
@@ -77,13 +79,16 @@
   int v_col0, v_C, v_shift, v_lo, v_hi;
   const float *sx, *sw;
   float* ssq;
+  const float *sum = nullptr, *pssq = nullptr, *csum = nullptr, *bfold = nullptr;
+  float invk = 0.f, eps = 0.f;
 };
 
 static int ga_launch(const GemmAsmKernel& k, int grid, hipStream_t s, GemmAsmArgs& a, const char* what) {
   const int lds = ga_lds(k.wn);
   if (int rc = ll_lds_attr(k.fn, lds)) return rc;
   void* args[] = {&a.x, &a.w, &a.bias, &a.out, &a.res, &a.gate, &a.M, &a.N, &a.K, &a.ldx, &a.ldo, &a.frame_len, &a.gate_stride, &a.ntm, &a.ntn,
-                  &a.gm, &a.v_out, &a.v_col0, &a.v_C, &a.v_shift, &a.v_lo, &a.v_hi, k.i8 ? (void*)&a.sx : (void*)&a.ssq, &a.sw};
+                  &a.gm, &a.v_out, &a.v_col0, &a.v_C, &a.v_shift, &a.v_lo, &a.v_hi, k.i8 ? (void*)&a.sx : (void*)&a.ssq, k.i8 ? (void*)&a.sw : (void*)&a.sum,
+                  &a.pssq, &a.csum, &a.bfold, &a.invk, &a.eps};
   if (hipLaunchKernel(k.fn, dim3(grid), dim3(256), args, (size_t)lds, s) != hipSuccess) return ll_check_launch(what);
   return 1;
 }
@@ -115,6 +120,47 @@
   if (!p.k || p.k->wn != 128) return 0;
   const GemmAsmKernel* k = ga_kernel(false, 128, GA_EPI_SSQ, false);
   GemmAsmArgs a{x, w, bias, out, nullptr, nullptr, M, N, K, ldx, ldo, 0, 0, p.ntm, p.ntn, gm, nullptr, 0, 0, 0, 0, 0, nullptr, nullptr, ssq};
+  return ga_launch(*k, p.grid, s, a, k->name);
+}
+
+int gemm_asm_fold_planes(int M, int C, int K, int frame_len) {
+  if (C % 128 != 0 || C / 128 > 12 || (long long)M * 4 * 12 >= 0x7fffffffLL) return 0;
+  const GemmAsmPick o = gemm_asm_pick(GQ_BF16, M, C, K, K, LL_EPI_BIAS_GATE_RES, true, false, false, frame_len, 0);
+  const GemmAsmPick q = gemm_asm_pick(GQ_BF16, M, C, C, C, LL_EPI_BIAS, true, false, false, 0, 0);
+  if (!o.k || !q.k || o.k->wn != 128 || q.k->wn != 128) return 0;
+  return C / 128;
+}
+const char* gemm_asm_fold_plan(int M, int C, int K, int frame_len, char* out, int cap) {
+  if (!gemm_asm_fold_planes(M, C, K, frame_len)) return nullptr;
+  GemmAsmPick o = gemm_asm_pick(GQ_BF16, M, C, K, K, LL_EPI_BIAS_GATE_RES, true, false, false, frame_len, 0);
+  GemmAsmPick q = gemm_asm_pick(GQ_BF16, M, C, C, C, LL_EPI_BIAS, true, false, false, 0, 0);
+  o.k = ga_kernel(false, 128, GA_EPI_GATE_RES_STATS, false), q.k = ga_kernel(false, 128, GA_EPI_FOLD_SSQ, false);
+  gemm_asm_plan(o, out, cap);
+  const size_t n = strlen(out);
+  if ((size_t)cap > n + 3) {
+    snprintf(out + n, (size_t)cap - n, "; ");
+    gemm_asm_plan(q, out + n + 2, cap - (int)n - 2);
+  }
+  return out;
+}
+int gemm_asm_stats_launch(const bf16* x, const bf16* w, bf16* out, float* sum, float* ssq, int M, int N, int K, int ldx, int ldo, const EpiArgs& ea,
+                          int gm, hipStream_t s) {
+  if (ea.mod != nullptr || ea.sx != nullptr || ea.v_out != nullptr || !gemm_asm_fold_planes(M, N, K, ea.frame_len)) return 0;
+  const GemmAsmPick p = gemm_asm_pick(GQ_BF16, M, N, K, ldx, LL_EPI_BIAS_GATE_RES, true, false, false, ea.frame_len, 0);
+  const GemmAsmKernel* k = ga_kernel(false, 128, GA_EPI_GATE_RES_STATS, false);
+  if (!p.k || !k) return 0;
+  GemmAsmArgs a{x, w, ea.bias, out, ea.res, ea.e + (size_t)ea.gate_idx * N, M, N, K, ldx, ldo, ea.frame_len, ea.nmod * N * 2, p.ntm, p.ntn, gm,
+                nullptr, 0, 0, 0, 0, 0, nullptr, nullptr, ssq};
+  a.sum = sum;
+  return ga_launch(*k, p.grid, s, a, k->name);
+}
+int gemm_asm_fold_launch(const bf16* x, const bf16* w, const float* csum, const float* bfold, const float* psum, const float* pssq, float eps,
+                         bf16* out, float* ssq, int M, int N, int K, int ldx, int ldo, int gm, hipStream_t s) {
+  const GemmAsmPick p = gemm_asm_pick(GQ_BF16, M, N, K, ldx, LL_EPI_BIAS, true, false, false, 0, 0);
+  const GemmAsmKernel* k = ga_kernel(false, 128, GA_EPI_FOLD_SSQ, false);
+  if (!p.k || p.k->wn != 128 || !k || K % 128 != 0 || K / 128 > 12 || (long long)M * 4 * 12 >= 0x7fffffffLL) return 0;
+  GemmAsmArgs a{x, w, nullptr, out, nullptr, nullptr, M, N, K, ldx, ldo, 0, 0, p.ntm, p.ntn, gm, nullptr, 0, 0, 0, 0, 0, nullptr, nullptr, ssq};
+  a.sum = psum, a.pssq = pssq, a.csum = csum, a.bfold = bfold, a.invk = 1.0f / (float)K, a.eps = eps;
   return ga_launch(*k, p.grid, s, a, k->name);
 }
 
diff --git a/longlive_amd/csrc/gen/gemm_asm_gen.py b/longlive_amd/csrc/gen/gemm_asm_gen.py
--- a/longlive_amd/csrc/gen/gemm_asm_gen.py
+++ b/longlive_amd/csrc/gen/gemm_asm_gen.py
@@ -11,6 +11,8 @@
 EPI_BIAS, EPI_GELU, EPI_GATE_RES, EPI_RES = 0, 1, 2, 3
 EPI_PARTIAL = 4
 EPI_BIAS_SSQ = 5
+EPI_GATE_RES_STATS = 6
+EPI_FOLD_SSQ = 7
 
 S_X, S_W, S_Y, S_BIAS, S_RES, S_GATE = 8, 10, 12, 14, 16, 18
 S_LDX, S_LDW, S_LDO = 20, 21, 22
@@ -19,6 +21,9 @@
 S_ROWLO = 29
 S_SX, S_SW = 64, 66
 S_SSQ = 64
+S_SUM = 66
+S_PSUM, S_PSSQ, S_CSUM, S_BF, S_PSTRIDE, S_NPL, S_INVC, S_EPS, S_PW = 66, 68, 70, 72, 74, 75, 76, 77, 78
+FOLD_MAXPL = 12
 S_XRS, S_WRS = 32, 36
 S_WAVE, S_I, S_T0, S_T1, S_T2 = 40, 41, 44, 45, 46
 S_WM0, S_XK, S_WK, S_XKMAX, S_WKMAX = 47, 48, 49, 43, 62
@@ -43,7 +48,10 @@
 class Cfg:
     def __init__(self, WN, epi, i8=False, mfma=32):
         assert WN % 32 == 0 and 64 <= WN <= 256
-        assert not (i8 and epi in (EPI_PARTIAL, EPI_BIAS_SSQ))
+        assert not (i8 and epi in (EPI_PARTIAL, EPI_BIAS_SSQ, EPI_GATE_RES_STATS, EPI_FOLD_SSQ))
+        assert WN == 128 or epi not in (EPI_GATE_RES_STATS, EPI_FOLD_SSQ)
+        self.gate, self.stats = epi in (EPI_GATE_RES, EPI_GATE_RES_STATS), epi == EPI_GATE_RES_STATS
+        self.ssq, self.fold = epi in (EPI_BIAS_SSQ, EPI_FOLD_SSQ), epi == EPI_FOLD_SSQ
         assert mfma in (32, 16) and not (mfma == 16 and (i8 or epi == EPI_PARTIAL))
         self.WN, self.NB, self.MB, self.epi, self.i8 = WN, WN // 32, 2, epi, i8
         self.mfma = mfma
@@ -73,13 +81,20 @@
             self.V_SX = top + 2
             top += 6
         assert top % 2 == 0, top
-        self.nl = {EPI_GATE_RES: 6, EPI_RES: 2}.get(epi, 0)
+        self.nl = {EPI_GATE_RES: 6, EPI_GATE_RES_STATS: 6, EPI_RES: 2}.get(epi, 0)
         self.V_E0 = top
         top += 16 if self.nl else 0
         self.V_SS = top
-        top += (8 if self.m16 else 4) if epi == EPI_BIAS_SSQ else 0
+        top += (8 if self.m16 else 4) if self.ssq else 0
+        self.V_RS = top
+        top += 4 * self.MB if self.stats else 0
+        self.nrb = 4 if self.m16 else 2
+        self.V_ST = top
+        top += 4 * self.nrb if self.fold else 0
+        self.nbv = 8 if self.m16 else 16
         self.V_EB = top
-        self.early_nb = 0 if epi == EPI_PARTIAL else max(0, min(self.NB, (256 - top) // 8))
+        assert not self.fold or top + 2 * self.nbv <= 256, top
+        self.early_nb = 0 if epi == EPI_PARTIAL or self.fold else max(0, min(self.NB, (256 - top) // 8))
 
     def acc(self, mb, nb):
         return (mb * self.NB + nb) * 16
@@ -283,7 +298,7 @@
 
 def generate(WN: int, epi: int, prefix: str, i8: bool = False, persistent: bool = False, mfma: int = 32) -> str:
     c = Cfg(WN, epi, i8, mfma)
-    assert not (persistent and (i8 or epi in (EPI_PARTIAL, EPI_BIAS_SSQ)))
+    assert not (persistent and (i8 or epi in (EPI_PARTIAL, EPI_BIAS_SSQ, EPI_GATE_RES_STATS, EPI_FOLD_SSQ)))
     g = Gen()
     I = g.I
     T = 128
@@ -362,7 +377,7 @@
             I(f"v_add_u32 {vreg(c.V_XROFF + 2 * hs + ks)}, {sreg(S_XM0)}, {vreg(c.V_WOFF + 2 * hs + ks)}")
     I(f"s_cmp_ge_u32 {sreg(S_T0)}, {sreg(S_ROWS)}")
     I(f"s_cbranch_scc1 {prefix}_IDLE")
-    n_early = gen_epilogue_setup(g, c)
+    n_early = gen_epilogue_setup(g, c, prefix)
     if persistent:
         I(f"s_cmp_eq_u32 {sreg(S_PF)}, 1")
         I(f"s_cbranch_scc1 {prefix}_STAGED")
@@ -375,6 +390,8 @@
     for r in range(c.nacc):
         I(f"v_accvgpr_write_b32 {areg(r)}, 0")
     I(f"s_waitcnt vmcnt({2 * npw + 8})")
+    if c.fold:
+        gen_fold_stats(g, c)
     if persistent:
         I(f"s_branch {prefix}_READY")
         g.L(f"{prefix}_STAGED")
@@ -512,7 +529,7 @@
 
 
 
-def gen_epilogue_setup(g: Gen, c: Cfg):
+def gen_epilogue_setup(g: Gen, c: Cfg, prefix: str = "GA"):
     I = g.I
     T = c.V_T
     epi = c.epi
@@ -527,7 +544,7 @@
         I(f"v_lshlrev_b32 {vreg(EA + 2)}, 3, {vreg(Q16)}")
     else:
         I(f"v_lshlrev_b32 {vreg(EA + 2)}, 3, {vreg(c.V_H)}")
-    if epi == EPI_GATE_RES:
+    if c.gate:
         I(f"s_sub_u32 {sreg(S_T1)}, {sreg(S_ROWS)}, 1")
         for mb in range(4 if c.m16 else c.MB):
             m, q, t = T + 66, EA + 3 + mb, T + 48
@@ -571,6 +588,10 @@
             I(f"global_load_dwordx2 {vreg(c.V_EB + 8 * nb + 2 * g4, 2)}, {vreg(EA + 2)}, {sreg(S_BIAS, 2)} offset:{64 * nb + (64 // c.bl) * g4}")
     if c.nl:
         epi_block_loads(g, c, 0, c.V_E0)
+    if c.fold:
+        I(f"v_lshlrev_b32 {vreg(EA + 3)}, 1, {vreg(EA + 2)}")
+        fold_vec_loads(g, c, 0, c.V_EB)
+        fold_plane_loads(g, c, prefix)
     return sum(1 for l in g.out if l.startswith("global_load")) - n0 + (c.MB if c.i8 else 0)
 
 
@@ -578,17 +599,75 @@
     I = g.I
     nb, mb = j // c.MB, j % c.MB
     EA = c.V_EA
-    if c.epi == EPI_GATE_RES:
+    if c.gate:
         for g4 in range(4):
             if c.m16:
                 I(f"global_load_dwordx2 {vreg(P + 2 * g4, 2)}, {vreg(EA + 3 + 2 * mb + (g4 & 1))}, {sreg(S_GATE, 2)} offset:{64 * nb + 32 * (g4 >> 1)}")
                 continue
             I(f"global_load_dwordx2 {vreg(P + 2 * g4, 2)}, {vreg(EA + 3 + mb)}, {sreg(S_GATE, 2)} offset:{64 * nb + 16 * g4}")
-    if c.epi in (EPI_GATE_RES, EPI_RES):
+    if c.nl:
         I(f"s_mov_b64 exec, {sreg(S_MSK + 2 * mb, 2)}")
         for k in (0, 2):
             I(f"global_load_dwordx4 {vreg(P + 8 + 2 * k, 4)}, {vreg(EA + mb)}, {sreg(S_RES, 2)} offset:{64 * nb + 16 * k}")
         I("s_mov_b64 exec, -1")
+
+
+def fold_vec_loads(g: Gen, c: Cfg, nb: int, base: int):
+    for k in range(c.nbv // 4):
+        off = 4 * (32 * nb + (16 if c.m16 else 8) * k)
+        g.I(f"global_load_dwordx4 {vreg(base + 4 * k, 4)}, {vreg(c.V_EA + 3)}, {sreg(S_BF, 2)} offset:{off}")
+        g.I(f"global_load_dwordx4 {vreg(base + c.nbv + 4 * k, 4)}, {vreg(c.V_EA + 3)}, {sreg(S_CSUM, 2)} offset:{off}")
+
+
+FOLD_PL, FOLD_ROW = 2, 100
+
+
+def fold_plane_loads(g: Gen, c: Cfg, prefix: str):
+    I = g.I
+    I(f"s_sub_u32 {sreg(S_T1)}, {sreg(S_ROWS)}, 1")
+    if c.m16:
+        I(f"v_and_b32 {vreg(FOLD_ROW + 4)}, 0xffffffef, {vreg(c.V_ROW)}")
+    for rb in range(c.nrb):
+        if c.m16:
+            I(f"v_add_u32 {vreg(FOLD_ROW + rb)}, {16 * rb}, {vreg(FOLD_ROW + 4)}")
+            I(f"v_min_u32 {vreg(FOLD_ROW + rb)}, {sreg(S_T1)}, {vreg(FOLD_ROW + rb)}")
+        else:
+            I(f"v_min_u32 {vreg(FOLD_ROW + rb)}, {sreg(S_T1)}, {vreg(c.V_ROW + rb)}")
+        I(f"v_lshlrev_b32 {vreg(FOLD_ROW + rb)}, 2, {vreg(FOLD_ROW + rb)}")
+    for k in range(2 * c.nrb * FOLD_MAXPL):
+        I(f"v_mov_b32 {vreg(FOLD_PL + k)}, 0")
+    for k in range(2):
+        I(f"s_mov_b32 {sreg(S_PW + k)}, {sreg(S_PSUM + k)}")
+        I(f"s_mov_b32 {sreg(S_PW + 2 + k)}, {sreg(S_PSSQ + k)}")
+    for p in range(FOLD_MAXPL):
+        if p:
+            I(f"s_cmp_le_u32 {sreg(S_NPL)}, {p}")
+            I(f"s_cbranch_scc1 {prefix}_PLANES")
+        for rb in range(c.nrb):
+            for k in range(2):
+                I(f"global_load_dword {vreg(FOLD_PL + 2 * (p * c.nrb + rb) + k)}, {vreg(FOLD_ROW + rb)}, {sreg(S_PW + 2 * k, 2)}")
+        for k in range(2):
+            add64(g, S_PW + 2 * k, S_PW + 2 * k, S_PSTRIDE)
+    g.L(f"{prefix}_PLANES")
+
+
+def gen_fold_stats(g: Gen, c: Cfg):
+    I = g.I
+    for rb in range(c.nrb):
+        s, qq, st = FOLD_PL + 2 * rb, FOLD_PL + 2 * rb + 1, c.V_ST + 4 * rb
+        for p in range(1, FOLD_MAXPL):
+            I(f"v_add_f32 {vreg(s)}, {vreg(s)}, {vreg(FOLD_PL + 2 * (p * c.nrb + rb))}")
+            I(f"v_add_f32 {vreg(qq)}, {vreg(qq)}, {vreg(FOLD_PL + 2 * (p * c.nrb + rb) + 1)}")
+        I(f"v_mul_f32 {vreg(s)}, {sreg(S_INVC)}, {vreg(s)}")
+        I(f"v_mul_f32 {vreg(qq)}, {sreg(S_INVC)}, {vreg(qq)}")
+        I(f"v_xor_b32 {vreg(st)}, 0x80000000, {vreg(s)}")
+        I(f"v_fma_f32 {vreg(qq)}, {vreg(st)}, {vreg(s)}, {vreg(qq)}")
+        I(f"v_max_f32 {vreg(qq)}, 0, {vreg(qq)}")
+        I(f"v_add_f32 {vreg(qq)}, {sreg(S_EPS)}, {vreg(qq)}")
+        I(f"v_rsq_f32 {vreg(st + 2)}, {vreg(qq)}")
+        I("s_nop 0")
+        I(f"v_mov_b32 {vreg(st + 1)}, {vreg(st)}")
+        I(f"v_mov_b32 {vreg(st + 3)}, {vreg(st + 2)}")
 
 
 def gen_epilogue(g: Gen, c: Cfg):
@@ -604,9 +683,12 @@
         cons[name] = s0
     if epi == EPI_GELU:
         const_pair("k1", K1, 54); const_pair("k0", K0, 56); const_pair("ce", CEXP, 58); const_pair("one", 1.0, 60)
-    if epi == EPI_BIAS_SSQ:
+    if c.ssq:
         for k in range((4 if c.m16 else 2) * c.MB):
             I(f"v_mov_b32 {vreg(c.V_SS + k)}, 0")
+    if c.stats:
+        for k in range(4 * c.MB):
+            I(f"v_mov_b32 {vreg(c.V_RS + k)}, 0")
     if epi == EPI_PARTIAL:
         for nb in range(c.NB):
             for mb in range(c.MB):
@@ -634,7 +716,7 @@
             I(f"global_load_dwordx4 {vreg(SWB + 16 * (nb & 1) + 4 * g4, 4)}, {vreg(EA + 5)}, {sreg(S_SW, 2)} offset:{128 * nb + 32 * g4}")
         q.extend([("sw", nb)] * 4)
 
-    for nb in range(c.early_nb, c.NB):
+    for nb in range(c.NB if c.fold else c.early_nb, c.NB):
         for g4 in range(c.bl):
             I(f"global_load_dwordx2 {vreg(BB + 8 * nb + 2 * g4, 2)}, {vreg(EA + 2)}, {sreg(S_BIAS, 2)} offset:{64 * nb + (64 // c.bl) * g4}")
         q.extend([("bias", nb)] * c.bl)
@@ -645,10 +727,21 @@
     blocks = [(nb, mb) for nb in range(c.NB) for mb in range(c.MB)]
     nl = c.nl
 
+    def fv(nb):
+        return c.V_EB if nb == 0 else BB + 2 * c.nbv * (nb & 1)
+    assert not c.fold or BB + 4 * c.nbv <= c.V_WOFF
+
     for j, (nb, mb) in enumerate(blocks):
         P = c.V_E0 if j == 0 else PB + 16 * (j & 1)
         if c.i8 and mb == 0 and nb + 1 < c.NB:
             sw_loads(nb + 1)
+        if c.fold and mb == 0:
+            if nb + 1 < c.NB:
+                fold_vec_loads(g, c, nb + 1, fv(nb + 1))
+                q.extend([("fv", nb + 1)] * (c.nbv // 2))
+            n = wait_for([("fv", nb)])
+            if n is not None:
+                I(f"s_waitcnt vmcnt({n})")
         if nl and j + 1 < len(blocks):
             epi_block_loads(g, c, j + 1, PB + 16 * ((j + 1) & 1))
             q.extend([("blk", j + 1)] * nl)
@@ -662,11 +755,11 @@
             I(f"s_waitcnt vmcnt({(n_late if c.early_nb else 0) + nxt_loads})")
         elif nl:
             I(f"s_waitcnt vmcnt({2 + nxt_loads})")
-        elif c.early_nb == 0 and j == 0:
+        elif c.early_nb == 0 and j == 0 and not c.fold:
             I("s_waitcnt vmcnt(0)")
         if not nl and mb == 0 and nb == c.early_nb and 0 < c.early_nb < c.NB:
             I(f"s_waitcnt vmcnt({min(63, 2 * j)})")
-        if mb == 0:
+        if mb == 0 and not c.fold:
             for g4 in range(4):
                 for d in range(2):
                     src = (c.V_EB if nb < c.early_nb else BB) + 8 * nb + 2 * (g4 >> 1 if c.m16 else g4) + d
@@ -683,18 +776,24 @@
                 I(f"v_pk_mul_f32 {vreg(T + 56, 2)}, {vreg(SWB + 16 * (nb & 1) + r, 2)}, {vreg(c.V_SX + 2 * mb, 2)}")
                 I(f"v_pk_mul_f32 {vreg(T + r, 2)}, {vreg(T + r, 2)}, {vreg(T + 56, 2)}")
         for r in range(0, 16, 2):
+            if c.fold:
+                st = c.V_ST + 4 * (2 * mb + ((r >> 2) & 1) if c.m16 else mb)
+                vi = 4 * (r >> 3) + (r & 3) if c.m16 else r
+                I(f"v_pk_fma_f32 {vreg(T + r, 2)}, {vreg(st, 2)}, {vreg(fv(nb) + c.nbv + vi, 2)}, {vreg(T + r, 2)}")
+                I(f"v_pk_fma_f32 {vreg(T + r, 2)}, {vreg(st + 2, 2)}, {vreg(T + r, 2)}, {vreg(fv(nb) + vi, 2)}")
+                continue
             I(f"v_pk_add_f32 {vreg(T + r, 2)}, {vreg(T + r, 2)}, {vreg(T + 24 + r, 2)}")
         for r in range(0, 16, 2):
             I(f"v_cvt_pk_bf16_f32 {vreg(T + 16 + r // 2)}, {vreg(T + r)}, {vreg(T + r + 1)}")
-        if epi in (EPI_GELU, EPI_GATE_RES, EPI_BIAS_SSQ):
+        if epi in (EPI_GELU, EPI_GATE_RES, EPI_BIAS_SSQ, EPI_GATE_RES_STATS, EPI_FOLD_SSQ):
             for r in range(0, 16, 2):
                 I(f"v_lshlrev_b32 {vreg(T + r)}, 16, {vreg(T + 16 + r // 2)}")
                 I(f"v_and_b32 {vreg(T + r + 1)}, 0xffff0000, {vreg(T + 16 + r // 2)}")
-        if epi == EPI_BIAS_SSQ:
+        if c.ssq:
             for r in range(0, 16, 2):
                 ss = c.V_SS + 2 * (2 * mb + ((r >> 2) & 1) if c.m16 else mb)
                 I(f"v_pk_fma_f32 {vreg(ss, 2)}, {vreg(T + r, 2)}, {vreg(T + r, 2)}, {vreg(ss, 2)}")
-        if epi == EPI_GATE_RES:
+        if c.gate:
             for r in range(0, 16, 2):
                 src = P + r // 2
                 I(f"v_lshlrev_b32 {vreg(T + 56)}, 16, {vreg(src)}")
@@ -728,7 +827,7 @@
             I(f"{swap} {vreg(ax)}, {vreg(bx)}")
             I(f"{swap} {vreg(ay)}, {vreg(by)}")
         off_y = 64 * nb
-        if epi in (EPI_GATE_RES, EPI_RES):
+        if c.nl:
             for k in (0, 2):
                 for d in range(4):
                     vsrc, rsrc = T + 16 + 2 * k + d, P + 8 + 2 * k + d
@@ -738,12 +837,17 @@
                     I(f"v_and_b32 {vreg(T + 3)}, 0xffff0000, {vreg(rsrc)}")
                     I(f"v_pk_add_f32 {vreg(T, 2)}, {vreg(T + 2, 2)}, {vreg(T, 2)}")
                     I(f"v_cvt_pk_bf16_f32 {vreg(vsrc)}, {vreg(T)}, {vreg(T + 1)}")
+                    if c.stats:
+                        I(f"v_lshlrev_b32 {vreg(T)}, 16, {vreg(vsrc)}")
+                        I(f"v_and_b32 {vreg(T + 1)}, 0xffff0000, {vreg(vsrc)}")
+                        I(f"v_pk_add_f32 {vreg(c.V_RS + 2 * mb, 2)}, {vreg(c.V_RS + 2 * mb, 2)}, {vreg(T, 2)}")
+                        I(f"v_pk_fma_f32 {vreg(c.V_RS + 2 * (c.MB + mb), 2)}, {vreg(T, 2)}, {vreg(T, 2)}, {vreg(c.V_RS + 2 * (c.MB + mb), 2)}")
         I(f"s_mov_b64 exec, {sreg(S_MSK + 2 * mb, 2)}")
         for k in (0, 2):
             I(f"global_store_dwordx4 {vreg(EA + mb)}, {vreg(T + 16 + 2 * k, 4)}, {sreg(S_Y, 2)} offset:{off_y + 16 * k}")
         I("s_mov_b64 exec, -1")
         q.extend([("st", j)] * 2)
-    if epi == EPI_BIAS_SSQ and c.m16:
+    if c.ssq and c.m16:
         R16, Q16 = T + 8, T + 9
         I(f"v_and_b32 {vreg(R16)}, 0xffffffef, {vreg(c.V_ROW)}")
         I(f"v_lshrrev_b32 {vreg(Q16)}, 4, {vreg(c.V_LANE)}")
@@ -768,7 +872,7 @@
             I(f"global_store_dword {vreg(T + mb)}, {vreg(ss)}, {sreg(S_SSQ, 2)}")
             I("s_mov_b64 exec, -1")
             q.append(("st", "ssq"))
-    elif epi == EPI_BIAS_SSQ:
+    elif c.ssq:
         for mb in range(c.MB):
             ss = c.V_SS + 2 * mb
             I(f"v_add_f32 {vreg(ss)}, {vreg(ss)}, {vreg(ss + 1)}")
@@ -787,6 +891,25 @@
             I(f"global_store_dword {vreg(T + mb)}, {vreg(ss)}, {sreg(S_SSQ, 2)}")
             I("s_mov_b64 exec, -1")
             q.append(("st", "ssq"))
+    if c.stats:
+        for k in range(2 * c.MB):
+            ss = c.V_RS + 2 * k
+            I(f"v_add_f32 {vreg(ss)}, {vreg(ss)}, {vreg(ss + 1)}")
+            I(f"v_mov_b32 {vreg(ss + 1)}, {vreg(ss)}")
+        I("s_nop 1")
+        for k in range(2 * c.MB):
+            ss = c.V_RS + 2 * k
+            I(f"v_permlane32_swap_b32 {vreg(ss)}, {vreg(ss + 1)}")
+        for k in range(2 * c.MB):
+            ss, mb = c.V_RS + 2 * k, k % c.MB
+            I(f"v_add_f32 {vreg(ss)}, {vreg(ss)}, {vreg(ss + 1)}")
+            I(f"v_lshlrev_b32 {vreg(T + mb)}, 2, {vreg(c.V_ROW + mb)}")
+            I(f"v_cmp_eq_u32_e64 vcc, {vreg(c.V_H)}, 0")
+            I(f"s_and_b64 vcc, vcc, {sreg(S_MSK + 2 * mb, 2)}")
+            I("s_mov_b64 exec, vcc")
+            I(f"global_store_dword {vreg(T + mb)}, {vreg(ss)}, {sreg(S_SUM if k < c.MB else S_SSQ, 2)}")
+            I("s_mov_b64 exec, -1")
+            q.append(("st", "stats"))
     n = 0
     while n < len(q) and q[len(q) - 1 - n][0] == "st":
         n += 1
diff --git a/longlive_amd/model.py b/longlive_amd/model.py
--- a/longlive_amd/model.py
+++ b/longlive_amd/model.py
@@ -168,6 +168,7 @@
         self.use_modulation_f32 = True
         self.fuse_attn_quant = False
         self.fuse_cross_qnorm = True
+        self.fold_norm3 = True
         self._packed = None
         self._rope_f = None
         self._rope_hw: Dict[Tuple[int, int], torch.Tensor] = {}
@@ -206,6 +207,8 @@
             ts = [sa.q.weight, sa.k.weight, sa.v.weight, sa.q.bias, sa.k.bias, sa.v.bias, blk.modulation]
             if self.quant is not None:
                 ts += [sa.o.weight, blk.cross_attn.q.weight, blk.cross_attn.o.weight, blk.ffn[0].weight, blk.ffn[2].weight]
+            elif self.fold_norm3:
+                ts += [blk.norm3.weight, blk.norm3.bias, blk.cross_attn.q.weight, blk.cross_attn.q.bias]
             key.extend((t.data_ptr(), t._version) for t in ts)
         return tuple(key)
 
@@ -227,6 +230,8 @@
                 for name, w in (("qkv", d["wqkv"]), ("o", sa.o.weight), ("cq", ca.q.weight), ("co", ca.o.weight),
                                 ("f1", blk.ffn[0].weight), ("f2", blk.ffn[2].weight)):
                     d["q_" + name], d["s_" + name] = quantize(w.detach().contiguous())
+            elif self.fold_norm3 and self.cfg.dim % 128 == 0:
+                d["cq_fold"] = ops.fold_norm_weights(ca.q.weight, ca.q.bias, blk.norm3.weight, blk.norm3.bias)
             P.append(d)
         self._packed = P
         self._mods = torch.stack([d["mod"] for d in P], 0).contiguous()
@@ -383,14 +388,21 @@
                                  out_fmt=ofmt)
         if cache_done_event is not None:
             cache_done_event.record(torch.cuda.current_stream())
-        self._lin(att if ofmt is not None else att.view(B, L, C), pk, "o", sa.o.weight, sa.o.bias, ops.EPI_BIAS_GATE_RES, out=xs, res=xs, e=e0,
-                  mod=mod, gate_idx=2, rows_per_batch=L, frame_len=fs)
-        xn = m.layernorm_affine(xs, blk.norm3.weight, blk.norm3.bias, c.eps)
         fuse_qn = (self.fuse_cross_qnorm and self.quant is None and ops.gemm_ssq_planes(B * L, C, C) == Hh and ops.flash_attn_qnorm_ok(Hh, c.text_len))
-        if fuse_qn:
-            qraw, ssq = ops.gemm_ssq(xn, ca.q.weight, ca.q.bias, tag="gemm_cq_ssq")
-        else:
-            qc = ops.rmsnorm(self._lin(xn, pk, "cq", ca.q.weight, ca.q.bias), ca.norm_q.weight, c.eps)
+        fold = (fuse_qn and self.fold_norm3 and mod is None and "cq_fold" in pk and ops.gemm_fold_planes(B * L, C, C, fs) == C // 128)
+        if fold:
+            _, stats = ops.gemm_gate_res_stats(att.view(B, L, C), sa.o.weight, sa.o.bias, xs, xs, e0, 2, L, fs, tag="gemm_o")
+        else:
+            self._lin(att if ofmt is not None else att.view(B, L, C), pk, "o", sa.o.weight, sa.o.bias, ops.EPI_BIAS_GATE_RES, out=xs, res=xs, e=e0,
+                      mod=mod, gate_idx=2, rows_per_batch=L, frame_len=fs)
+        if fold:
+            qraw, ssq = ops.gemm_fold_ssq(xs, pk["cq_fold"], stats, c.eps, tag="gemm_cq_ssq")
+        else:
+            xn = m.layernorm_affine(xs, blk.norm3.weight, blk.norm3.bias, c.eps)
+            if fuse_qn:
+                qraw, ssq = ops.gemm_ssq(xn, ca.q.weight, ca.q.bias, tag="gemm_cq_ssq")
+            else:
+                qc = ops.rmsnorm(self._lin(xn, pk, "cq", ca.q.weight, ca.q.bias), ca.norm_q.weight, c.eps)
         if not cac["is_init"]:
             kc = ops.gemm(ctx, ca.k.weight, ca.k.bias)
             if cac["k"].shape != (B, c.text_len, Hh, D) or not cac["k"].is_contiguous():
diff --git a/longlive_amd/ops.py b/longlive_amd/ops.py
--- a/longlive_amd/ops.py
+++ b/longlive_amd/ops.py
@@ -281,6 +281,62 @@
     t0 = _t0(tag)
     _lib.check(lib.ll_gemm_bf16_ssq(x.data_ptr(), w.data_ptr(), bias.data_ptr(), out.data_ptr(), ssq.data_ptr(), M, N, K, K, N, _stream()),
                "ll_gemm_bf16_ssq")
+    _t1(tag, t0, 2.0 * M * N * K)
+    return out, ssq
+
+
+def gemm_fold_planes(M: int, C: int, K: int, frame_len: int) -> int:
+    return int(_lib.load().ll_gemm_fold_planes(M, C, K, frame_len))
+
+
+def fold_norm_weights(w, b, gamma, beta):
+    w64 = w.detach().double()
+    wf = (w64 * gamma.detach().double()[None, :]).to(bf16).contiguous()
+    csum = wf.double().sum(1).float().contiguous()
+    bfold = (b.detach().double() + w64 @ beta.detach().double()).float().contiguous()
+    return wf, csum, bfold
+
+
+def gemm_gate_res_stats(x, w, bias, out, res, e, gate_idx: int, rows_per_batch: int, frame_len: int, tag: str = "gemm"):
+    _chk(x, "x"); _chk(w, "w"); _chk(bias, "bias"); _chk(out, "out"); _chk(res, "res"); _chk(e, "e")
+    K = x.shape[-1]
+    M = x.numel() // K
+    N = w.shape[0]
+    nmod = e.shape[-2]
+    assert w.shape == (N, K) and bias.numel() == N and out.numel() == M * N and res.numel() == M * N
+    assert e.shape[-1] == N and e.numel() == (M // frame_len) * nmod * N, (e.shape, M, frame_len)
+    planes = gemm_fold_planes(M, N, K, frame_len)
+    if planes == 0:
+        raise RuntimeError(f"gemm_gate_res_stats: {M} x {N} x {K} is not covered by the generated kernel (use gemm + layernorm_affine)")
+    stats = torch.empty(2, planes, M, dtype=torch.float32, device=x.device)
+    lib = _lib.load()
+    t0 = _t0(tag)
+    _lib.check(lib.ll_gemm_bf16_gate_res_stats(x.data_ptr(), w.data_ptr(), bias.data_ptr(), out.data_ptr(), stats[0].data_ptr(),
+                                               stats[1].data_ptr(), M, N, K, K, N, res.data_ptr(), e.data_ptr(), nmod, gate_idx,
+                                               rows_per_batch, frame_len, _stream()), "ll_gemm_bf16_gate_res_stats")
+    _t1(tag, t0, 2.0 * M * N * K)
+    return out, stats
+
+
+def gemm_fold_ssq(x, folded, stats, eps: float, out=None, tag: str = "gemm"):
+    wf, csum, bfold = folded
+    _chk(x, "x"); _chk(wf, "wf"); _chk(csum, "csum", torch.float32); _chk(bfold, "bfold", torch.float32); _chk(stats, "stats", torch.float32)
+    K = x.shape[-1]
+    M = x.numel() // K
+    N = wf.shape[0]
+    assert wf.shape == (N, K) and N == K and csum.numel() == N and bfold.numel() == N and stats.shape == (2, K // 128, M), (wf.shape, stats.shape)
+    if out is None:
+        out = torch.empty(*x.shape[:-1], N, dtype=bf16, device=x.device)
+    _chk(out, "out")
+    planes = gemm_ssq_planes(M, N, K)
+    if planes == 0 or gemm_fold_planes(M, N, K, 1) == 0:
+        raise RuntimeError(f"gemm_fold_ssq: {M} x {N} x {K} is not covered by the generated kernel (use layernorm_affine + gemm_ssq)")
+    ssq = torch.empty(planes, M, dtype=torch.float32, device=x.device)
+    lib = _lib.load()
+    t0 = _t0(tag)
+    _lib.check(lib.ll_gemm_bf16_fold_ssq(x.data_ptr(), wf.data_ptr(), csum.data_ptr(), bfold.data_ptr(), stats[0].data_ptr(),
+                                         stats[1].data_ptr(), eps, out.data_ptr(), ssq.data_ptr(), M, N, K, K, N, _stream()),
+               "ll_gemm_bf16_fold_ssq")
     _t1(tag, t0, 2.0 * M * N * K)
     return out, ssq
 
```

Result: no change. 93.81, median of 6 (+0.9%).
